# ChenKaiXuSan/Skiing_Analysis_PyTorch

Measured on AMD Instinct MI355X. Metric: 3D-pose frames/sec, 8-view 518px clips, higher is better.
Workload: dtype f16

## Files before the change

### include/skimi.h

```cpp
#ifndef SKIMI_H
#define SKIMI_H

#include <stddef.h>
#include <stdint.h>

#ifdef __cplusplus
extern "C" {
#endif

#define SKIMI_OK 0
#define SKIMI_ERR_ARG (-1)
#define SKIMI_ERR_HIP (-2)
#define SKIMI_ERR_STATE (-3)
#define SKIMI_ERR_WORKSPACE (-4)

#define SKIMI_F32 0
#define SKIMI_BF16 1
#define SKIMI_BF16X3_REC 2
#define SKIMI_FP8MX 3
#define SKIMI_F16 4

#define SKIMI_PREC_BF16 0
#define SKIMI_PREC_BF16X3 1
#define SKIMI_PREC_FP8 2
#define SKIMI_PREC_F16 3

#define SKIMI_ACT_NONE 0
#define SKIMI_ACT_RELU 1
#define SKIMI_ACT_GELU 2
#define SKIMI_ACT_SILU 3
#define SKIMI_ACT_SIGMOID 4

const char* skimi_last_error(void);
int skimi_version(void);
int skimi_sizeof_gemm_desc(void);
int skimi_device_count(void);

int skimi_profile_start(int32_t kind, int64_t min_size);
int skimi_profile_stop(double* total_ms, int64_t* launches, double* flops, double* bytes);

typedef struct skimi_gemm_desc {
    int32_t M, N, K;
    const void* A;
    const void* W;
    int32_t a_dtype, w_dtype;
    int64_t lda, ldw;
    int32_t prec;
    int32_t a_mode;
    int32_t cN, cH, cW, cC, KH, KW, stride, pad, dil, OH, OW;
    const float* bias;
    const float* gamma;
    const void* resid;
    int32_t resid_dtype;
    int64_t ldr;
    int32_t resid_rows_per_batch;
    int64_t resid_batch_stride;
    int64_t resid_row_off;
    int32_t act;
    const void* resid2;
    int64_t ldr2;
    int32_t post_act;
    int32_t out_rows_per_batch;
    int64_t out_batch_stride;
    int64_t out_row_off;
    void* out;
    void* out2;
    int32_t out_dtype;
    int64_t ldo, ldo2;
    int32_t store_mode, ps_s, ps_C;
    void* splitk_scratch;
    uint64_t splitk_scratch_bytes;
    int32_t force_splitk;
    int32_t splitk_scratch_zeroed;
    const void* W_split;
    void* x3_scratch;
    uint64_t x3_scratch_bytes;
    void* out_records;
} skimi_gemm_desc;

int skimi_split_planes(const float* x, int64_t ld, int64_t rows, int32_t C, void* hi, void* lo, void* stream);

int skimi_split_records(const float* x, int64_t ld, int64_t rows, int32_t C, void* records, void* stream);

int skimi_dpt_fold_pack(const float* w_T, const float* b_T, const float* w_rn, int32_t C_in, int32_t C_mid, int32_t C_out,
                        int32_t s, void* w_records, float* beta, void* stream);

int skimi_gemm(const skimi_gemm_desc* d, void* stream);

#define SKIMI_GEMM_PATH_GENERIC 1
#define SKIMI_GEMM_PATH_SPLITK_ORDERED 2
#define SKIMI_GEMM_PATH_SPLITK_ATOMIC 3
#define SKIMI_GEMM_PATH_X3DMA_WIDE 4
#define SKIMI_GEMM_PATH_X3DMA_NARROW 5
#define SKIMI_GEMM_PATH_GEMM256 6
#define SKIMI_GEMM_PATH_CONV_WIN 7
int32_t skimi_gemm_last_path(void);

int skimi_quant_mx(const void* x, int32_t dtype, int64_t ldx, int64_t rows, int32_t K, void* payload, void* scales,
                   void* stream);
int skimi_layernorm_mx(const float* x, int64_t ldx, int64_t rows, int32_t C, const float* gamma, const float* beta,
                       float eps, void* payload, void* scales, void* stream);
int skimi_gemm_fp8(const void* A, const void* A_scales, const void* W, const void* W_scales, int32_t M, int32_t N,
                   int32_t K, const float* bias, int32_t act, const float* gamma, const float* resid, int64_t ldr,
                   void* out, int32_t out_dtype, int64_t ldo, void* out_scales, void* stream);

int skimi_conv3x3_n32_pack(const float* w, void* packed, int32_t C, void* stream);
int skimi_conv3x3_n32(const void* in_hi, const void* in_lo, const void* packed_w, const float* bias, float* out,
                      int32_t F, int32_t H, int32_t W, int32_t C, int32_t relu, void* stream);

int skimi_resample_u8(const uint8_t* in, uint8_t* out, int64_t outer, int32_t n_in, int32_t n_out, int64_t inner,
                      const int32_t* kk, const int32_t* bounds, int32_t ksize, void* stream);
int skimi_u8_hwc_to_f32_chw(const uint8_t* in, int32_t H, int32_t W, float* out, int32_t OH, int32_t OW, int32_t y_off,
                            int32_t x_off, float fill, void* stream);

int skimi_layernorm(const float* x, const float* x2, int64_t ldx, int64_t rows, int32_t C,
                    const float* gamma, const float* beta, float eps,
                    void* out, int32_t out_dtype, int64_t ldo, void* stream);

int skimi_qknorm_rope(void* qkv, int32_t dtype, int64_t tokens, int32_t heads,
                      const float* qn_w, const float* qn_b, const float* kn_w, const float* kn_b,
                      float eps, const int32_t* pos, const float* rope_cos, const float* rope_sin,
                      int32_t rope_npos, void* stream);

int skimi_attention(const void* qkv, void* out, int32_t dtype, int32_t batch, int32_t seq,
                    int32_t heads, int32_t head_dim, void* stream);
int skimi_attention_out(const void* qkv, void* out, int32_t dtype, int32_t out_dtype, int32_t batch, int32_t seq,
                        int32_t heads, int32_t head_dim, void* stream);

int skimi_qknorm_rope_scaled(void* qkv, int32_t dtype, int64_t tokens, int32_t heads,
                             const float* qn_w, const float* qn_b, const float* kn_w, const float* kn_b,
                             float eps, const int32_t* pos, const float* rope_cos, const float* rope_sin,
                             int32_t rope_npos, float q_scale, int32_t* q_scaled, void* stream);
int skimi_attention_ex(const void* qkv, void* out, int32_t dtype, int32_t out_dtype, int32_t batch, int32_t seq,
                       int32_t heads, int32_t head_dim, int32_t q_prescaled, void* x3_scratch,
                       uint64_t x3_scratch_bytes, int32_t* out_records, void* stream);
uint64_t skimi_attention_x3_scratch_bytes(int64_t tokens, int64_t row_elems);

typedef struct skimi_vp3d skimi_vp3d;

skimi_vp3d* skimi_vp3d_create(int32_t joints_in, int32_t in_features, int32_t joints_out,
                              const int32_t* filter_widths, int32_t n_widths,
                              int32_t channels, int32_t causal);
skimi_vp3d* skimi_vp3d_create_ex(int32_t joints_in, int32_t in_features, int32_t joints_out,
                                 const int32_t* filter_widths, int32_t n_widths,
                                 int32_t channels, int32_t causal, int32_t dense);
void skimi_vp3d_destroy(skimi_vp3d*);
int skimi_vp3d_set_weight(skimi_vp3d*, const char* key, const float* host_data, int64_t n);
int skimi_vp3d_finalize(skimi_vp3d*, int32_t prec);
int32_t skimi_vp3d_receptive_field(const skimi_vp3d*);
size_t skimi_vp3d_workspace_bytes(const skimi_vp3d*, int32_t batch, int32_t frames_in);
int skimi_vp3d_forward(skimi_vp3d*, const float* x, float* out, int32_t batch, int32_t frames_in,
                       void* workspace, size_t workspace_bytes, void* stream);

typedef struct skimi_vggt skimi_vggt;

typedef struct skimi_vggt_config {
    int32_t patch_size, embed_dim, depth, num_heads, num_register_tokens;
    int32_t use_dino;
    int32_t dino_depth, dino_heads, dino_img_size;
    int32_t cam_trunk_depth, cam_heads, cam_iters;
    int32_t dpt_features, dpt_out_channels[4], dpt_layers[4];
    int32_t track_features, track_hidden, track_corr_levels, track_corr_radius, track_iters, track_depth,
        track_heads, track_virtual;
    int32_t enable_camera, enable_depth, enable_point, enable_track;
    int32_t prec;
    int32_t head_prec;
} skimi_vggt_config;

skimi_vggt* skimi_vggt_create(const skimi_vggt_config* cfg);
void skimi_vggt_destroy(skimi_vggt*);
int skimi_vggt_set_weight(skimi_vggt*, const char* key, const float* data, int64_t n, int32_t on_device);
int skimi_vggt_finalize(skimi_vggt*);
int skimi_vggt_set_pos_embed(skimi_vggt*, int32_t H, int32_t W, const float* pos_embed, int32_t on_device);
size_t skimi_vggt_workspace_bytes(skimi_vggt*, int32_t B, int32_t S, int32_t H, int32_t W, int32_t n_query);
int skimi_vggt_rope_positions(skimi_vggt*, int32_t frames, int32_t H, int32_t W, int32_t* positions);

typedef struct skimi_vggt_outputs {
    float* pose_enc;
    float* pose_enc_list;
    float* depth;
    float* depth_conf;
    float* world_points;
    float* world_points_conf;
    float* track;
    float* vis;
    float* conf;
    float* tokens_last;
} skimi_vggt_outputs;

int skimi_vggt_forward(skimi_vggt*, const float* images, const float* query_points, int32_t B, int32_t S,
                       int32_t H, int32_t W, int32_t n_query, const skimi_vggt_outputs* out,
                       void* workspace, size_t workspace_bytes, void* stream);

int skimi_pose_to_cameras(const float* pose_enc, int64_t rows, int32_t H, int32_t W, float* extrinsic,
                          float* intrinsic, void* stream);
int skimi_unproject_depth(const float* depth, const float* extrinsic, const float* intrinsic,
                          float* world_points, int32_t frames, int32_t H, int32_t W, void* stream);
int skimi_triangulate_dlt(const float* K, const float* R, const float* t, const float* keypoints,
                          float* joints3d, int64_t steps, int32_t views, int32_t joints, void* stream);

int skimi_triangulate_triage(const float* K, const float* R, const float* t, const float* keypoints, const float* conf,
                             double conf_thr, double err_thresh_px, int64_t steps, int32_t views, int32_t joints,
                             float* joints3d, float* joints3d_clean, double* err, double* depth, uint8_t* keep,
                             double* view_stats, double* report, void* stream);

int skimi_triangulate_robust(const float* K, const float* R, const float* t, const float* keypoints, const float* conf,
                             double conf_thr, double inlier_px, int32_t min_inliers, int32_t refine_iters, int32_t weighted,
                             int64_t steps, int32_t views, int32_t joints, float* joints3d, double* err,
                             uint8_t* inlier_views, double* rms_px, uint8_t* ok, float* joints3d_ok,
                             double* view_inlier_ratio, double* report, void* stream);

size_t skimi_person_workspace_bytes(int64_t maps, int32_t H, int32_t W);
int skimi_person_origin(const float* points, const float* boxes, int64_t maps, int32_t H, int32_t W, int32_t src_h,
                        int32_t src_w, void* workspace, double* stats, void* stream);
int skimi_recenter_cameras(const double* stats, const float* extrinsic, int64_t steps, int32_t views, double* origin_out,
                           float* R_out, float* t_out, void* stream);

size_t skimi_icp_workspace_bytes(int64_t n_src, int64_t n_tgt);
int skimi_estimate_normals(const float* points, int64_t n, double radius, double* normals_out,
                           int32_t* neighbour_count_out, void* ws, size_t ws_bytes, void* stream);
int skimi_icp_correspondences(const float* src, int64_t n_src, const float* tgt, int64_t n_tgt, const double* T4x4,
                              double max_dist, int32_t* tgt_index_out, void* ws, size_t ws_bytes, void* stream);
int skimi_icp_point_to_plane(const float* src, int64_t n_src, const float* tgt, int64_t n_tgt, double max_corr_dist,
                             double normal_radius, int32_t max_iteration, double rel_fitness, double rel_rmse,
                             const double* init4x4, double* T_out, double* fitness_out, double* rmse_out,
                             int32_t* iterations_out, void* ws, size_t ws_bytes, void* stream);

#define SKIMI_BA_POSE_ONLY 0
#define SKIMI_BA_POSE_CAM_T 1
#define SKIMI_BA_FULL 2
#define SKIMI_BA_AUTO 0
#define SKIMI_BA_LDS 1
#define SKIMI_BA_WORKSPACE 2
size_t skimi_ba_workspace_bytes(int64_t T, int32_t C, int32_t J, int32_t modes);
int skimi_bundle_adjust(const double* K, const double* R0, const double* t0, const double* X0, const double* x2d,
                        const double* conf, int64_t T, int32_t C, int32_t J, const int32_t* modes, int32_t n_modes,
                        int32_t num_iters, double lr, double w_reproj, double w_smooth, double w_baseline,
                        double w_bone_length, double w_pose_temporal, int32_t placement, double* R_out, double* t_out,
                        double* X_out, double* history_out, void* ws, size_t ws_bytes, void* stream);

#define SKIMI_RESECT_LINEAR 0
#define SKIMI_RESECT_SOFT_L1 1
size_t skimi_resect_workspace_bytes(int64_t n_points, int32_t views, int64_t group_size);
int skimi_resect_cameras(const double* X, const double* x2d, const double* conf, const double* K, const double* R0,
                         const double* t0, int64_t n_points, int32_t views, int64_t group_size, int32_t loss, double f_scale,
                         double min_conf, int32_t max_evals, double* R, double* t, double* K_out, double* cost0, double* cost,
                         int32_t* n_evals, int32_t* n_used, int32_t* success, double* err, double* stats, void* ws,
                         size_t ws_bytes, void* stream);
int skimi_relative_pose(const double* R, const double* t, int64_t groups, int32_t views, double* R_rel, double* t_rel,
                        void* stream);

#ifdef __cplusplus
}
#endif
#endif
```

### skiing_analysis_pytorch_amd/_lib.py

```python
from __future__ import annotations

import ctypes as C
from pathlib import Path

LIB_PATH = Path(__file__).resolve().parent / "lib" / "libskimi.so"

F32, BF16 = 0, 1
F16 = 4
BF16X3_REC = 2
FP8MX = 3
PREC_BF16, PREC_BF16X3, PREC_FP8 = 0, 1, 2
PREC_F16 = 3
ACT_NONE, ACT_RELU, ACT_GELU, ACT_SILU, ACT_SIGMOID = 0, 1, 2, 3, 4
GEMM_PATH_GENERIC, GEMM_PATH_SPLITK_ORDERED, GEMM_PATH_SPLITK_ATOMIC = 1, 2, 3
GEMM_PATH_X3DMA_WIDE, GEMM_PATH_X3DMA_NARROW, GEMM_PATH_GEMM256, GEMM_PATH_CONV_WIN = 4, 5, 6, 7


class SkimiError(RuntimeError):
    pass


class GemmDesc(C.Structure):

    _fields_ = [
        ("M", C.c_int32), ("N", C.c_int32), ("K", C.c_int32),
        ("A", C.c_void_p), ("W", C.c_void_p),
        ("a_dtype", C.c_int32), ("w_dtype", C.c_int32),
        ("lda", C.c_int64), ("ldw", C.c_int64),
        ("prec", C.c_int32),
        ("a_mode", C.c_int32),
        ("cN", C.c_int32), ("cH", C.c_int32), ("cW", C.c_int32), ("cC", C.c_int32),
        ("KH", C.c_int32), ("KW", C.c_int32), ("stride", C.c_int32), ("pad", C.c_int32),
        ("dil", C.c_int32), ("OH", C.c_int32), ("OW", C.c_int32),
        ("bias", C.c_void_p), ("gamma", C.c_void_p), ("resid", C.c_void_p),
        ("resid_dtype", C.c_int32),
        ("ldr", C.c_int64),
        ("resid_rows_per_batch", C.c_int32),
        ("resid_batch_stride", C.c_int64),
        ("resid_row_off", C.c_int64),
        ("act", C.c_int32),
        ("resid2", C.c_void_p), ("ldr2", C.c_int64), ("post_act", C.c_int32),
        ("out_rows_per_batch", C.c_int32), ("out_batch_stride", C.c_int64), ("out_row_off", C.c_int64),
        ("out", C.c_void_p), ("out2", C.c_void_p),
        ("out_dtype", C.c_int32),
        ("ldo", C.c_int64), ("ldo2", C.c_int64),
        ("store_mode", C.c_int32), ("ps_s", C.c_int32), ("ps_C", C.c_int32),
        ("splitk_scratch", C.c_void_p),
        ("splitk_scratch_bytes", C.c_uint64),
        ("force_splitk", C.c_int32), ("splitk_scratch_zeroed", C.c_int32),
        ("W_split", C.c_void_p), ("x3_scratch", C.c_void_p), ("x3_scratch_bytes", C.c_uint64),
        ("out_records", C.c_void_p),
    ]


_vp = C.c_void_p
_SIGNATURES = {
    "skimi_last_error": (C.c_char_p, []),
    "skimi_version": (C.c_int, []),
    "skimi_sizeof_gemm_desc": (C.c_int, []),
    "skimi_device_count": (C.c_int, []),
    "skimi_profile_start": (C.c_int, [C.c_int32, C.c_int64]),
    "skimi_profile_stop": (C.c_int, [C.POINTER(C.c_double), C.POINTER(C.c_int64), C.POINTER(C.c_double),
                                    C.POINTER(C.c_double)]),
    "skimi_gemm": (C.c_int, [C.POINTER(GemmDesc), _vp]),
    "skimi_gemm_last_path": (C.c_int32, []),
    "skimi_dpt_fold_pack": (C.c_int, [_vp, _vp, _vp, C.c_int32, C.c_int32, C.c_int32, C.c_int32, _vp, _vp, _vp]),
    "skimi_quant_mx": (C.c_int, [_vp, C.c_int32, C.c_int64, C.c_int64, C.c_int32, _vp, _vp, _vp]),
    "skimi_layernorm_mx": (C.c_int, [_vp, C.c_int64, C.c_int64, C.c_int32, _vp, _vp, C.c_float, _vp, _vp, _vp]),
    "skimi_gemm_fp8": (C.c_int, [_vp, _vp, _vp, _vp, C.c_int32, C.c_int32, C.c_int32, _vp, C.c_int32, _vp, _vp, C.c_int64,
                                 _vp, C.c_int32, C.c_int64, _vp, _vp]),
    "skimi_split_planes": (C.c_int, [_vp, C.c_int64, C.c_int64, C.c_int32, _vp, _vp, _vp]),
    "skimi_split_records": (C.c_int, [_vp, C.c_int64, C.c_int64, C.c_int32, _vp, _vp]),
    "skimi_resample_u8": (C.c_int, [_vp, _vp, C.c_int64, C.c_int32, C.c_int32, C.c_int64, _vp, _vp, C.c_int32, _vp]),
    "skimi_u8_hwc_to_f32_chw": (C.c_int, [_vp, C.c_int32, C.c_int32, _vp, C.c_int32, C.c_int32, C.c_int32, C.c_int32,
                                          C.c_float, _vp]),
    "skimi_conv3x3_n32_pack": (C.c_int, [_vp, _vp, C.c_int32, _vp]),
    "skimi_conv3x3_n32": (C.c_int, [_vp, _vp, _vp, _vp, _vp, C.c_int32, C.c_int32, C.c_int32, C.c_int32, C.c_int32, _vp]),
    "skimi_layernorm": (C.c_int, [_vp, _vp, C.c_int64, C.c_int64, C.c_int32, _vp, _vp, C.c_float, _vp,
                                  C.c_int32, C.c_int64, _vp]),
    "skimi_qknorm_rope": (C.c_int, [_vp, C.c_int32, C.c_int64, C.c_int32, _vp, _vp, _vp, _vp, C.c_float,
                                    _vp, _vp, _vp, C.c_int32, _vp]),
    "skimi_attention": (C.c_int, [_vp, _vp, C.c_int32, C.c_int32, C.c_int32, C.c_int32, C.c_int32, _vp]),
    "skimi_attention_out": (C.c_int, [_vp, _vp, C.c_int32, C.c_int32, C.c_int32, C.c_int32, C.c_int32, C.c_int32, _vp]),
    "skimi_qknorm_rope_scaled": (C.c_int, [_vp, C.c_int32, C.c_int64, C.c_int32, _vp, _vp, _vp, _vp, C.c_float,
                                           _vp, _vp, _vp, C.c_int32, C.c_float, C.POINTER(C.c_int32), _vp]),
    "skimi_attention_ex": (C.c_int, [_vp, _vp, C.c_int32, C.c_int32, C.c_int32, C.c_int32, C.c_int32, C.c_int32, C.c_int32,
                                     _vp, C.c_uint64, C.POINTER(C.c_int32), _vp]),
    "skimi_attention_x3_scratch_bytes": (C.c_uint64, [C.c_int64, C.c_int64]),
    "skimi_vp3d_create": (_vp, [C.c_int32, C.c_int32, C.c_int32, C.POINTER(C.c_int32), C.c_int32,
                                C.c_int32, C.c_int32]),
    "skimi_vp3d_create_ex": (_vp, [C.c_int32, C.c_int32, C.c_int32, C.POINTER(C.c_int32), C.c_int32,
                                   C.c_int32, C.c_int32, C.c_int32]),
    "skimi_vp3d_destroy": (None, [_vp]),
    "skimi_vp3d_set_weight": (C.c_int, [_vp, C.c_char_p, _vp, C.c_int64]),
    "skimi_vp3d_finalize": (C.c_int, [_vp, C.c_int32]),
    "skimi_vp3d_receptive_field": (C.c_int32, [_vp]),
    "skimi_vp3d_workspace_bytes": (C.c_size_t, [_vp, C.c_int32, C.c_int32]),
    "skimi_vp3d_forward": (C.c_int, [_vp, _vp, _vp, C.c_int32, C.c_int32, _vp, C.c_size_t, _vp]),
    "skimi_pose_to_cameras": (C.c_int, [_vp, C.c_int64, C.c_int32, C.c_int32, _vp, _vp, _vp]),
    "skimi_unproject_depth": (C.c_int, [_vp, _vp, _vp, _vp, C.c_int32, C.c_int32, C.c_int32, _vp]),
    "skimi_triangulate_dlt": (C.c_int, [_vp, _vp, _vp, _vp, _vp, C.c_int64, C.c_int32, C.c_int32, _vp]),
    "skimi_triangulate_triage": (C.c_int, [_vp, _vp, _vp, _vp, _vp, C.c_double, C.c_double, C.c_int64, C.c_int32, C.c_int32,
                                           _vp, _vp, _vp, _vp, _vp, _vp, _vp, _vp]),
    "skimi_triangulate_robust": (C.c_int, [_vp, _vp, _vp, _vp, _vp, C.c_double, C.c_double, C.c_int32, C.c_int32, C.c_int32,
                                           C.c_int64, C.c_int32, C.c_int32, _vp, _vp, _vp, _vp, _vp, _vp, _vp, _vp, _vp]),
    "skimi_person_workspace_bytes": (C.c_size_t, [C.c_int64, C.c_int32, C.c_int32]),
    "skimi_person_origin": (C.c_int, [_vp, _vp, C.c_int64, C.c_int32, C.c_int32, C.c_int32, C.c_int32, _vp, _vp, _vp]),
    "skimi_recenter_cameras": (C.c_int, [_vp, _vp, C.c_int64, C.c_int32, _vp, _vp, _vp, _vp]),
    "skimi_icp_workspace_bytes": (C.c_size_t, [C.c_int64, C.c_int64]),
    "skimi_estimate_normals": (C.c_int, [_vp, C.c_int64, C.c_double, _vp, _vp, _vp, C.c_size_t, _vp]),
    "skimi_icp_correspondences": (C.c_int, [_vp, C.c_int64, _vp, C.c_int64, C.POINTER(C.c_double), C.c_double, _vp, _vp,
                                            C.c_size_t, _vp]),
    "skimi_icp_point_to_plane": (C.c_int, [_vp, C.c_int64, _vp, C.c_int64, C.c_double, C.c_double, C.c_int32, C.c_double,
                                           C.c_double, C.POINTER(C.c_double), C.POINTER(C.c_double), C.POINTER(C.c_double),
                                           C.POINTER(C.c_double), C.POINTER(C.c_int32), _vp, C.c_size_t, _vp]),
    "skimi_ba_workspace_bytes": (C.c_size_t, [C.c_int64, C.c_int32, C.c_int32, C.c_int32]),
    "skimi_bundle_adjust": (C.c_int, [_vp, _vp, _vp, _vp, _vp, _vp, C.c_int64, C.c_int32, C.c_int32, C.POINTER(C.c_int32),
                                      C.c_int32, C.c_int32, C.c_double, C.c_double, C.c_double, C.c_double, C.c_double,
                                      C.c_double, C.c_int32, _vp, _vp, _vp, _vp, _vp, C.c_size_t, _vp]),
    "skimi_resect_workspace_bytes": (C.c_size_t, [C.c_int64, C.c_int32, C.c_int64]),
    "skimi_resect_cameras": (C.c_int, [_vp, _vp, _vp, _vp, _vp, _vp, C.c_int64, C.c_int32, C.c_int64, C.c_int32, C.c_double,
                                       C.c_double, C.c_int32, _vp, _vp, _vp, _vp, _vp, _vp, _vp, _vp, _vp, _vp, _vp, C.c_size_t,
                                       _vp]),
    "skimi_relative_pose": (C.c_int, [_vp, _vp, C.c_int64, C.c_int32, _vp, _vp, _vp]),
    "skimi_vggt_create": (_vp, [_vp]),
    "skimi_vggt_destroy": (None, [_vp]),
    "skimi_vggt_set_weight": (C.c_int, [_vp, C.c_char_p, _vp, C.c_int64, C.c_int32]),
    "skimi_vggt_finalize": (C.c_int, [_vp]),
    "skimi_vggt_set_pos_embed": (C.c_int, [_vp, C.c_int32, C.c_int32, _vp, C.c_int32]),
    "skimi_vggt_rope_positions": (C.c_int, [_vp, C.c_int32, C.c_int32, C.c_int32, _vp]),
    "skimi_vggt_workspace_bytes": (C.c_size_t, [_vp, C.c_int32, C.c_int32, C.c_int32, C.c_int32, C.c_int32]),
    "skimi_vggt_forward": (C.c_int, [_vp, _vp, _vp, C.c_int32, C.c_int32, C.c_int32, C.c_int32, C.c_int32, _vp,
                                     _vp, C.c_size_t, _vp]),
}

_lib = None


def exported_symbols():
    return sorted(_SIGNATURES)


def lib() -> C.CDLL:
    global _lib
    if _lib is not None:
        return _lib
    if not LIB_PATH.exists():
        raise SkimiError(
            f"{LIB_PATH} not found: build it with `python -m skiing_analysis_pytorch_amd.build` "
            "(or __graft_entry__.build()). There is no fallback path."
        )
    import torch

    handle = C.CDLL(str(LIB_PATH))
    for name, (res, args) in _SIGNATURES.items():
        try:
            fn = getattr(handle, name)
        except AttributeError as e:
            raise SkimiError(f"libskimi.so does not export {name}") from e
        fn.restype = res
        fn.argtypes = args
    if handle.skimi_sizeof_gemm_desc() != C.sizeof(GemmDesc):
        raise SkimiError(f"skimi_gemm_desc is {handle.skimi_sizeof_gemm_desc()} bytes in libskimi.so but "
                         f"{C.sizeof(GemmDesc)} in _lib.py: rebuild the library (python -m skiing_analysis_pytorch_amd.build)")
    _lib = handle
    return _lib


def check(rc: int, what: str = "") -> None:
    if rc != 0:
        msg = lib().skimi_last_error()
        raise SkimiError(f"{what} failed ({rc}): {msg.decode() if msg else ''}")


def ptr(t) -> int | None:
    if t is None:
        return None
    return t.data_ptr()


def current_stream() -> int:
    import torch

    return torch.cuda.current_stream().cuda_stream
```

### skiing_analysis_pytorch_amd/csrc/api.hip

```cpp
#include <stdarg.h>

#include <mutex>
#include <vector>

#include "common.h"
#include "gemm_epilogue.h"
#include "kernels.h"
#include "vggt_kernels.h"

namespace skimi {

static thread_local char g_err[512] = "";

void set_error(const char* fmt, ...) {
    va_list ap;
    va_start(ap, fmt);
    vsnprintf(g_err, sizeof(g_err), fmt, ap);
    va_end(ap);
}

int lds_opt_in(std::atomic<unsigned>& done, const void* kernel, int bytes, const char* what) {
    int dev = 0;
    if (hipGetDevice(&dev) != hipSuccess) {
        set_error("hipGetDevice failed (%s)", what);
// ... 78 lines not shown
        SKIMI_HIP(hipEventSynchronize(e.second));
        float t = 0;
        SKIMI_HIP(hipEventElapsedTime(&t, e.first, e.second));
        ms += t;
    }
    if (total_ms) *total_ms = ms;
    if (launches) *launches = (int64_t)g_prof.ev.size();
    if (flops) *flops = g_prof.flops;
    if (bytes) *bytes = g_prof.bytes;
    for (auto& e : g_prof.ev) g_prof.pool.push_back(e);
    g_prof.ev.clear();
    g_prof.kind = PROF_NONE;
    return SKIMI_OK;
}

int32_t skimi_gemm_last_path(void) { return gemm_last_path(); }

int skimi_gemm(const skimi_gemm_desc* d, void* stream) {
    if (!d) {
        set_gemm_path(0, 0, 0, 0, 0);
        set_error("skimi_gemm: null descriptor");
        return SKIMI_ERR_ARG;
    }
    return gemm_dispatch(d, (hipStream_t)stream, d->splitk_scratch, (size_t)d->splitk_scratch_bytes,
                         d->force_splitk);
}

int skimi_resample_u8(const uint8_t* in, uint8_t* out, int64_t outer, int32_t n_in, int32_t n_out, int64_t inner,
                      const int32_t* kk, const int32_t* bounds, int32_t ksize, void* stream) {
    return resample_u8_launch(in, out, outer, n_in, n_out, inner, kk, bounds, ksize, (hipStream_t)stream);
}

int skimi_u8_hwc_to_f32_chw(const uint8_t* in, int32_t H, int32_t W, float* out, int32_t OH, int32_t OW, int32_t y_off,
                            int32_t x_off, float fill, void* stream) {
    return u8_hwc_to_f32_chw_launch(in, H, W, out, OH, OW, y_off, x_off, fill, (hipStream_t)stream);
}

int skimi_conv3x3_n32_pack(const float* w, void* packed, int32_t C, void* stream) {
    SKIMI_CHECK_ARG(w && packed && C > 0, "skimi_conv3x3_n32_pack: bad arguments");
    return conv_direct_pack_launch(w, (unsigned short*)packed, C, (hipStream_t)stream);
}

int skimi_conv3x3_n32(const void* in_hi, const void* in_lo, const void* packed_w, const float* bias, float* out,
                      int32_t F, int32_t H, int32_t W, int32_t C, int32_t relu, void* stream) {
    return conv_direct_n32_launch((const unsigned short*)in_hi, (const unsigned short*)in_lo,
                                  (const unsigned short*)packed_w, bias, out, F, H, W, C, relu, (hipStream_t)stream);
}

int skimi_split_planes(const float* x, int64_t ld, int64_t rows, int32_t C, void* hi, void* lo, void* stream) {
    SKIMI_CHECK_ARG(x && hi && lo && rows > 0 && C > 0, "skimi_split_planes: bad arguments");
    return split_planes_launch(x, (long)ld, (long)rows, C, hi, lo, (hipStream_t)stream);
}

int skimi_split_records(const float* x, int64_t ld, int64_t rows, int32_t C, void* records, void* stream) {
    SKIMI_CHECK_ARG(x && records && rows > 0 && C > 0, "skimi_split_records: bad arguments");
    return split_records_launch(x, (long)ld, (long)rows, C, records, (hipStream_t)stream);
}

int skimi_dpt_fold_pack(const float* w_T, const float* b_T, const float* w_rn, int32_t C_in, int32_t C_mid, int32_t C_out,
                        int32_t s, void* w_records, float* beta, void* stream) {
    SKIMI_CHECK_ARG(w_T && w_rn && w_records && beta, "skimi_dpt_fold_pack: null buffer");
    SKIMI_CHECK_ARG(s >= 2 && s <= 16 && C_in > 0 && C_in % 32 == 0 && C_mid > 0 && C_out > 0, "skimi_dpt_fold_pack: bad sizes");
    float* tmp = nullptr;
    SKIMI_HIP(hipMalloc((void**)&tmp, (size_t)(s + 2) * (s + 2) * C_out * C_in * 4));
    const int rc = dpt_fold_pack_launch(w_T, b_T, w_rn, C_in, C_mid, C_out, s, tmp, w_records, beta, (hipStream_t)stream);
    const hipError_t e = hipStreamSynchronize((hipStream_t)stream);
    (void)hipFree(tmp);
    if (rc) return rc;
    SKIMI_HIP(e);
    return SKIMI_OK;
}

int skimi_quant_mx(const void* x, int32_t dtype, int64_t ldx, int64_t rows, int32_t K, void* payload, void* scales,
                   void* stream) {
    return quant_mx_launch(x, dtype, (long)ldx, (long)rows, K, payload, scales, (hipStream_t)stream);
}

int skimi_layernorm_mx(const float* x, int64_t ldx, int64_t rows, int32_t C, const float* gamma, const float* beta,
                       float eps, void* payload, void* scales, void* stream) {
    return layernorm_mx_launch(x, ldx, rows, C, gamma, beta, eps, payload, scales, (hipStream_t)stream);
}

int skimi_gemm_fp8(const void* A, const void* A_scales, const void* W, const void* W_scales, int32_t M, int32_t N,
                   int32_t K, const float* bias, int32_t act, const float* gamma, const float* resid, int64_t ldr,
                   void* out, int32_t out_dtype, int64_t ldo, void* out_scales, void* stream) {
    return gemm_fp8_launch(A, A_scales, W, W_scales, M, N, K, bias, act, gamma, resid, (long)ldr, out, out_dtype, (long)ldo,
                           (hipStream_t)stream, out_scales);
}

int skimi_layernorm(const float* x, const float* x2, int64_t ldx, int64_t rows, int32_t C,
                    const float* gamma, const float* beta, float eps, void* out, int32_t out_dtype,
                    int64_t ldo, void* stream) {
    return layernorm_launch(x, x2, ldx, rows, C, gamma, beta, eps, out, out_dtype, ldo,
                            (hipStream_t)stream);
}

int skimi_qknorm_rope(void* qkv, int32_t dtype, int64_t tokens, int32_t heads, const float* qn_w,
                      const float* qn_b, const float* kn_w, const float* kn_b, float eps,
                      const int32_t* pos, const float* rope_cos, const float* rope_sin,
                      int32_t rope_npos, void* stream) {
    return qknorm_rope_launch(qkv, dtype, tokens, heads, qn_w, qn_b, kn_w, kn_b, eps, pos, rope_cos,
                              rope_sin, rope_npos, (hipStream_t)stream);
}

int skimi_attention(const void* qkv, void* out, int32_t dtype, int32_t batch, int32_t seq,
                    int32_t heads, int32_t head_dim, void* stream) {
    return attention_launch(qkv, out, dtype, batch, seq, heads, head_dim, (hipStream_t)stream);
}

int skimi_attention_out(const void* qkv, void* out, int32_t dtype, int32_t out_dtype, int32_t batch, int32_t seq,
                        int32_t heads, int32_t head_dim, void* stream) {
    if (out_dtype == SKIMI_FP8MX) {
        SKIMI_CHECK_ARG(out && batch > 0 && seq > 0 && attention_mx_output_ok(dtype, heads, head_dim),
                        "skimi_attention_out: MXFP8 rows need bf16 q / k / v, head_dim 64 and an even number of heads");
        const size_t Kp = align_up((size_t)heads * head_dim, 128);
        return attention_launch(qkv, nullptr, dtype, batch, seq, heads, head_dim, (hipStream_t)stream, 0, nullptr, 0, nullptr, 0,
                                out, (char*)out + (size_t)batch * seq * Kp);
    }
    SKIMI_CHECK_ARG(out_dtype == dtype || (dtype == SKIMI_BF16 && out_dtype == SKIMI_F16),
                    "skimi_attention_out: out_dtype is dtype, SKIMI_F16 or SKIMI_FP8MX for bf16 q / k / v (got %d -> %d)", dtype, out_dtype);
    return attention_launch(qkv, out, dtype, batch, seq, heads, head_dim, (hipStream_t)stream, 0, nullptr, 0, nullptr,
                            out_dtype == SKIMI_F16 && dtype == SKIMI_BF16);
}

int skimi_qknorm_rope_scaled(void* qkv, int32_t dtype, int64_t tokens, int32_t heads, const float* qn_w,
                             const float* qn_b, const float* kn_w, const float* kn_b, float eps,
                             const int32_t* pos, const float* rope_cos, const float* rope_sin,
                             int32_t rope_npos, float q_scale, int32_t* q_scaled, void* stream) {
    return qknorm_rope_launch(qkv, dtype, tokens, heads, qn_w, qn_b, kn_w, kn_b, eps, pos, rope_cos,
                              rope_sin, rope_npos, (hipStream_t)stream, q_scale, q_scaled);
}

int skimi_attention_ex(const void* qkv, void* out, int32_t dtype, int32_t out_dtype, int32_t batch, int32_t seq,
                       int32_t heads, int32_t head_dim, int32_t q_prescaled, void* x3_scratch,
                       uint64_t x3_scratch_bytes, int32_t* out_records, void* stream) {
    if (out_dtype == SKIMI_FP8MX) {
        if (out_records) *out_records = 0;
        SKIMI_CHECK_ARG(out && batch > 0 && seq > 0 && attention_mx_output_ok(dtype, heads, head_dim),
                        "skimi_attention_ex: MXFP8 rows need bf16 q / k / v, head_dim 64 and an even number of heads");
        const size_t Kp = align_up((size_t)heads * head_dim, 128);
        return attention_launch(qkv, nullptr, dtype, batch, seq, heads, head_dim, (hipStream_t)stream, q_prescaled, nullptr, 0,
                                nullptr, 0, out, (char*)out + (size_t)batch * seq * Kp);
    }
    SKIMI_CHECK_ARG(out_dtype == dtype || (dtype == SKIMI_BF16 && out_dtype == SKIMI_F16),
                    "skimi_attention_ex: out_dtype is dtype, SKIMI_F16 or SKIMI_FP8MX for bf16 q / k / v (got %d -> %d)", dtype, out_dtype);
    return attention_launch(qkv, out, dtype, batch, seq, heads, head_dim, (hipStream_t)stream, q_prescaled, x3_scratch,
                            (size_t)x3_scratch_bytes, out_records, out_dtype == SKIMI_F16 && dtype == SKIMI_BF16);
}

uint64_t skimi_attention_x3_scratch_bytes(int64_t tokens, int64_t row_elems) {
    return (uint64_t)attention_x3_scratch_bytes((long)tokens, (long)row_elems);
}

}
```

### skiing_analysis_pytorch_amd/csrc/attention_bf16.hip

```cpp
#include <stdlib.h>

#include "common.h"
#include "kernels.h"

namespace skimi {

typedef __attribute__((ext_vector_type(4))) short s16x4;
typedef __attribute__((address_space(3))) s16x4 lds_s16x4;
typedef __attribute__((address_space(3))) void lds_void;
typedef __attribute__((address_space(1))) const void gbl_void;

__device__ __forceinline__ bf16x8 pack8(const f32x16& p, int s) {
    bf16x8 r;
#pragma unroll
    for (int j = 0; j < 8; ++j) r[j] = (short)f2bf(p[8 * s + j]);
    return r;
}

template <int dbg>
__global__ __launch_bounds__(256, 4) void attn_bf16_kernel(const AttnArgs a, int nqb) {
    constexpr int KV = 64;
    constexpr int TILE = KV * 64 * 2;
    __shared__ __attribute__((aligned(16))) char smem[4 * TILE];

// ... 20 lines not shown

    bf16x8 qf[4];
    {
        const int q = min(q0 + l31, a.seq_q - 1);
        const unsigned short* qp = Q + (long)q * a.q_row + 8 * lh;
#pragma unroll
        for (int s = 0; s < 4; ++s) qf[s] = *reinterpret_cast<const bf16x8*>(qp + 16 * s);
    }

    const int nkt = (a.seq_k + KV - 1) / KV;
    const bool ragged = (a.seq_k & (KV - 1)) != 0;
    const int srow = lane >> 3, sch = lane & 7;
    auto issue = [&](int buf, int kt) {
        char* kb = smem + buf * 2 * TILE;
        char* vb = kb + TILE;
#pragma unroll
        for (int j = 0; j < 2; ++j) {
            const int row = 8 * (2 * wave + j) + srow;
            const int key = min(kt * KV + row, a.seq_k - 1);
            const int kc = sch ^ ((row >> 1) & 7);
            const int vc = sch ^ (((row >> 1) & 1) << 2);
            __builtin_amdgcn_global_load_lds((gbl_void*)(K + (long)key * a.k_row + kc * 8),
                                             (lds_void*)(kb + (2 * wave + j) * 8 * 128), 16, 0, 0);
            __builtin_amdgcn_global_load_lds((gbl_void*)(V + (long)key * a.v_row + vc * 8),
                                             (lds_void*)(vb + (2 * wave + j) * 8 * 128), 16, 0, 0);
        }
    };

    f32x16 o[2];
#pragma unroll
    for (int i = 0; i < 2; ++i)
#pragma unroll
        for (int r = 0; r < 16; ++r) o[i][r] = 0.f;
    f32x16 lacc = {0.f, 0.f, 0.f, 0.f, 0.f, 0.f, 0.f, 0.f, 0.f, 0.f, 0.f, 0.f, 0.f, 0.f, 0.f, 0.f};
    const bf16x8 ones = {0x3F80, 0x3F80, 0x3F80, 0x3F80, 0x3F80, 0x3F80, 0x3F80, 0x3F80};
    float m = -INFINITY;
    const float c2 = a.scale * 1.44269504088896340736f;

    issue(0, 0);
    __builtin_amdgcn_s_waitcnt(0x0F70);
    __syncthreads();

    for (int kt = 0; kt < nkt; ++kt) {
        const int cur = kt & 1;
        if (kt + 1 < nkt) issue(cur ^ 1, kt + 1);
        const char* kb = smem + cur * 2 * TILE;
        const char* vb = kb + TILE;

        f32x16 s[2];
        const f32x16 zero16 = {0.f, 0.f, 0.f, 0.f, 0.f, 0.f, 0.f, 0.f, 0.f, 0.f, 0.f, 0.f, 0.f, 0.f, 0.f, 0.f};
#pragma unroll
        for (int t = 0; t < 2; ++t) {
            const int row = t * 32 + l31;
#pragma unroll
            for (int ks = 0; ks < 4; ++ks) {
                const bf16x8 kf = (dbg & 1) ? qf[ks] :
                    *reinterpret_cast<const bf16x8*>(kb + row * 128 + (((2 * ks + lh) ^ ((row >> 1) & 7)) << 4));
                s[t] = __builtin_amdgcn_mfma_f32_32x32x16_bf16(kf, qf[ks], ks == 0 ? zero16 : s[t], 0, 0, 0);
            }
        }
        if (ragged && kt == nkt - 1) {
#pragma unroll
            for (int t = 0; t < 2; ++t)
#pragma unroll
                for (int r = 0; r < 16; ++r) {
                    const int key = kt * KV + t * 32 + (r & 3) + 8 * (r >> 2) + 4 * lh;
                    if (key >= a.seq_k) s[t][r] = -INFINITY;
                }
        }
        float mloc = -INFINITY;
#pragma unroll
        for (int t = 0; t < 2; ++t)
#pragma unroll
            for (int r = 0; r < 16; ++r) mloc = fmaxf(mloc, s[t][r]);
        mloc = fmaxf(mloc, __shfl_xor(mloc, 32, 64));
        const float mnew = fmaxf(m, mloc);
        const float nmb = -(mnew * c2);
        if (!__all(mnew == m)) {
            const float alpha = __builtin_amdgcn_exp2f((m - mnew) * c2);
#pragma unroll
            for (int r = 0; r < 16; ++r) {
                o[0][r] *= alpha;
                o[1][r] *= alpha;
                lacc[r] *= alpha;
            }
            m = mnew;
        }
#pragma unroll
        for (int r = 0; r < 16; ++r) {
            if (!(dbg & 4)) {
                s[0][r] = __builtin_amdgcn_exp2f(__builtin_fmaf(s[0][r], c2, nmb));
                s[1][r] = __builtin_amdgcn_exp2f(__builtin_fmaf(s[1][r], c2, nmb));
            }
        }

#pragma unroll
        for (int t = 0; t < 2; ++t) {
#pragma unroll
            for (int ks = 0; ks < 2; ++ks) {
                const bf16x8 pf = pack8(s[t], ks);
                if (!(dbg & 8)) lacc = __builtin_amdgcn_mfma_f32_32x32x16_bf16(ones, pf, lacc, 0, 0, 0);
#pragma unroll
                for (int dt = 0; dt < 2; ++dt) {
                    const int q4 = (lane & 15) >> 2, p4 = lane & 3;
                    const int dcol = dt * 32 + 16 * ((lane >> 4) & 1) + 4 * p4;
                    bf16x8 vf = qf[0];
                    if (!(dbg & 2))
#pragma unroll
                    for (int half = 0; half < 2; ++half) {
                        const int row = t * 32 + 16 * ks + 8 * half + 4 * lh + q4;
                        const int chunk = (dcol >> 3) ^ (((row >> 1) & 1) << 2);
                        const char* addr = vb + row * 128 + (chunk << 4) + ((dcol & 7) << 1);
                        const s16x4 v4 = __builtin_amdgcn_ds_read_tr16_b64_v4i16((lds_s16x4*)addr);
                        vf[4 * half + 0] = v4[0];
                        vf[4 * half + 1] = v4[1];
                        vf[4 * half + 2] = v4[2];
                        vf[4 * half + 3] = v4[3];
                    }
                    o[dt] = __builtin_amdgcn_mfma_f32_32x32x16_bf16(vf, pf, o[dt], 0, 0, 0);
                }
            }
        }

        __builtin_amdgcn_s_waitcnt(0x0F70);
        __syncthreads();
    }

    const float inv = 1.f / lacc[0];
    const int q = q0 + l31;
    if (q < a.seq_q) {
        unsigned short* op = O + (long)q * a.o_row;
#pragma unroll
        for (int dt = 0; dt < 2; ++dt)
#pragma unroll
            for (int g = 0; g < 4; ++g) {
                bf16x4 v;
#pragma unroll
                for (int j = 0; j < 4; ++j) v[j] = (short)f2x16(o[dt][4 * g + j] * inv, a.out_f16 != 0);
                *reinterpret_cast<bf16x4*>(op + dt * 32 + 8 * g + 4 * lh) = v;
            }
    }
}

static int q64_enabled() {
    static const int q64 = getenv("SKIMI_ATTN_Q64") ? atoi(getenv("SKIMI_ATTN_Q64")) : 1;
    return q64;
}

bool attention_mx_output_ok(int dtype, int heads, int head_dim) {
    static const bool dyn = getenv("SKIMI_ENV_DYNAMIC") && atoi(getenv("SKIMI_ENV_DYNAMIC"));
    static int use_mx = -1;
    if (use_mx < 0 || dyn) use_mx = getenv("SKIMI_ATTN_MX") ? atoi(getenv("SKIMI_ATTN_MX")) : 1;
    return use_mx && dtype == SKIMI_BF16 && head_dim == 64 && heads % 2 == 0 && q64_enabled() != 0;
}

int attention_bf16_launch(const AttnArgs& a, hipStream_t st) {
    SKIMI_CHECK_ARG(a.q && a.k && a.v && (a.out || a.out_mx), "skimi_attention: null buffer");
    SKIMI_CHECK_ARG(a.batch > 0 && a.heads > 0 && a.seq_q > 0 && a.seq_k > 0, "skimi_attention: empty shape");
    SKIMI_CHECK_ARG(a.head_dim == 64, "skimi_attention: the bf16 MFMA kernel is head_dim 64 only (got %d)", a.head_dim);
    SKIMI_CHECK_ARG(a.q_row % 8 == 0 && a.k_row % 8 == 0 && a.v_row % 8 == 0 && a.o_row % 4 == 0 &&
                    a.q_head % 8 == 0 && a.k_head % 8 == 0 && a.v_head % 8 == 0 && a.o_head % 4 == 0 &&
                    a.q_batch % 8 == 0 && a.k_batch % 8 == 0 && a.v_batch % 8 == 0 && a.o_batch % 4 == 0,
                    "skimi_attention: bf16 strides must keep 16-B alignment");
    SKIMI_CHECK_ARG((((uintptr_t)a.q | (uintptr_t)a.k | (uintptr_t)a.v) & 15) == 0,
                    "skimi_attention: bf16 q / k / v are loaded in 16-B pieces: the buffer must be 16-B aligned");
    const int nqb = (int)cdiv(a.seq_q, 128);
    const long nblk = (long)nqb * a.heads * a.batch;
    SKIMI_CHECK_ARG(nblk < (1l << 31), "skimi_attention: grid too large");
    const bool prof = prof_armed(PROF_ATTN_BF16, a.seq_k);
    if (prof) prof_before(st);
#ifdef SKIMI_ABLATIONS
    static const int dbg = getenv("SKIMI_ATTN_ABL") ? atoi(getenv("SKIMI_ATTN_ABL")) : 0;
#else
    const int dbg = 0;
#endif
    const int q64 = q64_enabled();
    SKIMI_CHECK_ARG(!a.out_mx || q64 != 0, "skimi_attention: MXFP8 output rows are written by the 64-query kernel only");
    if (q64 != 0) {
        attention_q64_dispatch(a, st);
    } else if (a.q_prescaled) {
        AttnArgs a1 = a;
        a1.scale = 0.69314718055994530942f;
        hipLaunchKernelGGL(attn_bf16_kernel<0>, dim3((unsigned)nblk), dim3(256), 0, st, a1, nqb);
    } else
    switch (dbg) {
#ifdef SKIMI_ABLATIONS
#define SKIMI_ABL_CASE(D) case D: hipLaunchKernelGGL(attn_bf16_kernel<D>, dim3((unsigned)nblk), dim3(256), 0, st, a, nqb); break;
        SKIMI_ABL_CASE(1) SKIMI_ABL_CASE(2) SKIMI_ABL_CASE(3) SKIMI_ABL_CASE(4) SKIMI_ABL_CASE(8) SKIMI_ABL_CASE(12)
        SKIMI_ABL_CASE(15)
#undef SKIMI_ABL_CASE
#endif
        default: hipLaunchKernelGGL(attn_bf16_kernel<0>, dim3((unsigned)nblk), dim3(256), 0, st, a, nqb);
    }
    if (prof) {
        const double bh = (double)a.batch * a.heads;
        prof_after(st, 4.0 * bh * a.seq_q * (double)a.seq_k * 64.0,
                   2.0 * bh * 64.0 * (2.0 * a.seq_q + 2.0 * a.seq_k));
    }
    SKIMI_LAUNCH_CHECK();
    return SKIMI_OK;
}

int attention_launch(const void* qkv, void* out, int dtype, int batch, int seq, int heads, int head_dim,
                     hipStream_t st, int q_prescaled, void* x3_scratch, size_t x3_scratch_bytes, int* out_records, int out_f16,
                     void* out_mx, void* out_mx_scales) {
    SKIMI_CHECK_ARG(qkv && (out || out_mx), "skimi_attention: null buffer");
    SKIMI_CHECK_ARG(!out_mx || (out_mx_scales && attention_mx_output_ok(dtype, heads, head_dim)),
                    "skimi_attention: MXFP8 output needs the 64-query bf16 kernel (head_dim 64, heads even) and a scale buffer");
    const bool want_rec = out_records != nullptr && *out_records != 0;
    if (out_records) *out_records = 0;
    AttnArgs a;
    const long C = (long)heads * head_dim;
    const size_t es = dtype == SKIMI_F32 ? 4 : 2;
    a.q = qkv;
    a.k = (const char*)qkv + C * es;
    a.v = (const char*)qkv + 2 * C * es;
    a.out = out;
    a.q_row = a.k_row = a.v_row = 3 * C;
    a.o_row = C;
    a.q_batch = a.k_batch = a.v_batch = (long)seq * 3 * C;
    a.o_batch = (long)seq * C;
    a.q_head = a.k_head = a.v_head = a.o_head = head_dim;
    a.batch = batch;
    a.heads = heads;
    a.seq_q = a.seq_k = seq;
    a.head_dim = head_dim;
    a.scale = 1.0f / sqrtf((float)head_dim);
    a.q_prescaled = dtype == SKIMI_F32 ? 0 : q_prescaled;
    a.out_f16 = dtype == SKIMI_F32 ? 0 : out_f16;
    if (out_mx) {
        a.out_mx = out_mx;
        a.out_mx_scales = out_mx_scales;
        a.mx_row = (long)align_up((size_t)C, 128);
        a.mx_srow = a.mx_row / 32;
    }
    if (dtype == SKIMI_F32) {
        static const bool dyn = getenv("SKIMI_ENV_DYNAMIC") && atoi(getenv("SKIMI_ENV_DYNAMIC"));
        static int use_x3 = -1;
        if (use_x3 < 0 || dyn) use_x3 = getenv("SKIMI_ATTN_X3") ? atoi(getenv("SKIMI_ATTN_X3")) : 1;
        const long tokens = (long)batch * seq;
        if (use_x3 && head_dim == 64 && x3_scratch && x3_scratch_bytes >= attention_x3_scratch_bytes(tokens, 3 * C)) {
            const bool rec = want_rec && ((uintptr_t)out & 127) == 0;
            if (rec) *out_records = 1;
            return attention_x3_launch(a, tokens, 3 * C, x3_scratch, x3_scratch_bytes, st, rec);
        }
        return attention_f32_launch(a, st);
    }
    return attention_bf16_launch(a, st);
}

}
```

### skiing_analysis_pytorch_amd/csrc/attention_q64.hip

```cpp
#include <stdlib.h>

#include "common.h"
#include "kernels.h"

namespace skimi {

typedef __attribute__((ext_vector_type(4))) short s16x4;
typedef __attribute__((address_space(3))) s16x4 lds_s16x4;
typedef __attribute__((address_space(3))) void lds_void;
typedef __attribute__((address_space(1))) const void gbl_void;
typedef __attribute__((ext_vector_type(2))) float f32x2;

__device__ __forceinline__ float xhalf_max(float x) {
    const auto r = __builtin_amdgcn_permlane32_swap(__float_as_uint(x), __float_as_uint(x), false, false);
    return __builtin_fmaxf(__uint_as_float(r[0]), __uint_as_float(r[1]));
}
__device__ __forceinline__ float xhalf_sum(float x) {
    const auto r = __builtin_amdgcn_permlane32_swap(__float_as_uint(x), __float_as_uint(x), false, false);
    return __uint_as_float(r[0]) + __uint_as_float(r[1]);
}

template <int dbg>
__global__ __launch_bounds__(256, 2) void attn_q64_kernel(const AttnArgs a, int nqb) {
    constexpr int KV = 64;
    constexpr int TILE = KV * 64 * 2;
    __shared__ __attribute__((aligned(16))) char smem[4 * TILE];

    const int tid = threadIdx.x, lane = tid & 63;
    const int wave = __builtin_amdgcn_readfirstlane(tid >> 6);
    const int l31 = lane & 31, lh = lane >> 5;

    int id;
    {
        const int nblk = gridDim.x;
        const int bid = blockIdx.x;
        const int xcd = bid & 7;
        const int q = nblk >> 3, r = nblk & 7;
        id = (xcd < r ? xcd * (q + 1) : r * (q + 1) + (xcd - r) * q) + (bid >> 3);
    }
    const int qb = id % nqb;
    const int bh = id / nqb;
    const int head = bh % a.heads, b = bh / a.heads;
    const int q0 = qb * 256 + wave * 64;

    const unsigned short* Q = (const unsigned short*)a.q + (long)b * a.q_batch + (long)head * a.q_head;
    const unsigned short* K = (const unsigned short*)a.k + (long)b * a.k_batch + (long)head * a.k_head;
    const unsigned short* V = (const unsigned short*)a.v + (long)b * a.v_batch + (long)head * a.v_head;
    unsigned short* O = (unsigned short*)a.out + (long)b * a.o_batch + (long)head * a.o_head;

    bf16x8 qf[2][4];
#pragma unroll
    for (int qi = 0; qi < 2; ++qi) {
        const int q = min(q0 + qi * 32 + l31, a.seq_q - 1);
        const unsigned short* qp = Q + (long)q * a.q_row + 8 * lh;
#pragma unroll
        for (int s = 0; s < 4; ++s) qf[qi][s] = *reinterpret_cast<const bf16x8*>(qp + 16 * s);
    }
    if (!a.q_prescaled) {
        const float c2q = a.scale * 1.44269504088896340736f;
#pragma unroll
        for (int qi = 0; qi < 2; ++qi)
#pragma unroll
            for (int s = 0; s < 4; ++s)
#pragma unroll
                for (int j = 0; j < 8; ++j) qf[qi][s][j] = (short)f2bf(bf2f((unsigned short)qf[qi][s][j]) * c2q);
    }

    const int nkt = (a.seq_k + KV - 1) / KV;
    const bool ragged = (a.seq_k & (KV - 1)) != 0;
    const int srow = lane >> 3, sch = lane & 7;
    auto issue = [&](int buf, int kt) {
        char* kb = smem + buf * 2 * TILE;
        char* vb = kb + TILE;
#pragma unroll
        for (int j = 0; j < 2; ++j) {
            const int row = 8 * (2 * wave + j) + srow;
            const int key = min(kt * KV + row, a.seq_k - 1);
            const int kc = sch ^ ((row >> 1) & 7);
            const int vc = sch ^ (((row >> 1) & 1) << 2);
            __builtin_amdgcn_global_load_lds((gbl_void*)(K + (long)key * a.k_row + kc * 8),
                                             (lds_void*)(kb + (2 * wave + j) * 8 * 128), 16, 0, 0);
            __builtin_amdgcn_global_load_lds((gbl_void*)(V + (long)key * a.v_row + vc * 8),
                                             (lds_void*)(vb + (2 * wave + j) * 8 * 128), 16, 0, 0);
        }
    };

    f32x16 o[2][2];
#pragma unroll
    for (int qi = 0; qi < 2; ++qi)
#pragma unroll
        for (int dt = 0; dt < 2; ++dt)
#pragma unroll
            for (int r = 0; r < 16; ++r) o[qi][dt][r] = 0.f;
    float lsum[2] = {0.f, 0.f};
    float mr[2] = {0.f, 0.f};
    const f32x16 zero16 = {0.f, 0.f, 0.f, 0.f, 0.f, 0.f, 0.f, 0.f, 0.f, 0.f, 0.f, 0.f, 0.f, 0.f, 0.f, 0.f};
    bf16x8 kone = {0, 0, 0, 0, 0, 0, 0, 0};
    if (lh == 0) kone[0] = (short)0x3F80;
    bf16x8 qneg[2] = {{0, 0, 0, 0, 0, 0, 0, 0}, {0, 0, 0, 0, 0, 0, 0, 0}};

    issue(0, 0);
    __builtin_amdgcn_s_waitcnt(0x0F70);
    __syncthreads();

    for (int kt = 0; kt < nkt; ++kt) {
        const int cur = kt & 1;
        const char* kb = smem + cur * 2 * TILE;
        const char* vb = kb + TILE;

        f32x16 s[2][2];
        bf16x8 kf[2][4];
#pragma unroll
        for (int t = 0; t < 2; ++t) {
            const int row = t * 32 + l31;
#pragma unroll
            for (int ks = 0; ks < 4; ++ks)
                kf[t][ks] = *reinterpret_cast<const bf16x8*>(kb + row * 128 + (((2 * ks + lh) ^ ((row >> 1) & 7)) << 4));
        }
        __builtin_amdgcn_sched_barrier(0);
#pragma unroll
        for (int t = 0; t < 2; ++t) {
#pragma unroll
            for (int qi = 0; qi < 2; ++qi)
                s[qi][t] = __builtin_amdgcn_mfma_f32_32x32x16_bf16(kone, qneg[qi], zero16, 0, 0, 0);
#pragma unroll
            for (int ks = 0; ks < 4; ++ks)
#pragma unroll
                for (int qi = 0; qi < 2; ++qi)
                    s[qi][t] = __builtin_amdgcn_mfma_f32_32x32x16_bf16(kf[t][ks], qf[qi][ks], s[qi][t], 0, 0, 0);
        }

        bf16x8 vf[2][2][2];
#pragma unroll
        for (int t = 0; t < 2; ++t)
#pragma unroll
            for (int ks = 0; ks < 2; ++ks)
#pragma unroll
                for (int dt = 0; dt < 2; ++dt) {
                    const int q4 = (lane & 15) >> 2, p4 = lane & 3;
                    const int dcol = dt * 32 + 16 * ((lane >> 4) & 1) + 4 * p4;
#pragma unroll
                    for (int half = 0; half < 2; ++half) {
                        const int row = t * 32 + 16 * ks + 8 * half + 4 * lh + q4;
                        const int chunk = (dcol >> 3) ^ (((row >> 1) & 1) << 2);
                        const char* addr = vb + row * 128 + (chunk << 4) + ((dcol & 7) << 1);
                        const s16x4 v4 = __builtin_amdgcn_ds_read_tr16_b64_v4i16((lds_s16x4*)addr);
                        vf[t][ks][dt][4 * half + 0] = v4[0];
                        vf[t][ks][dt][4 * half + 1] = v4[1];
                        vf[t][ks][dt][4 * half + 2] = v4[2];
                        vf[t][ks][dt][4 * half + 3] = v4[3];
                    }
                }

        __builtin_amdgcn_sched_barrier(0);
        if (kt + 1 < nkt) issue(cur ^ 1, kt + 1);

        if (ragged && kt == nkt - 1) {
#pragma unroll
            for (int qi = 0; qi < 2; ++qi)
#pragma unroll
                for (int t = 0; t < 2; ++t)
#pragma unroll
                    for (int r = 0; r < 16; ++r) {
                        const int key = kt * KV + t * 32 + (r & 3) + 8 * (r >> 2) + 4 * lh;
                        if (key >= a.seq_k) s[qi][t][r] = -INFINITY;
                    }
        }

#pragma unroll
        for (int qi = 0; qi < 2; ++qi) {
            bool redo = kt == 0;
            if (kt != 0) {
                float l0 = 0.f, l1 = 0.f;
#pragma unroll
                for (int t = 0; t < 2; ++t)
#pragma unroll
                    for (int r = 0; r < 16; r += 2) {
                        float v0 = s[qi][t][r], v1 = s[qi][t][r + 1];
                        if (!(dbg & 2)) {
                            v0 = __builtin_amdgcn_exp2f(v0);
                            v1 = __builtin_amdgcn_exp2f(v1);
                        }
                        l0 += v0;
                        l1 += v1;
                        s[qi][t][r] = v0;
                        s[qi][t][r + 1] = v1;
                    }
                const float ts = l0 + l1;
                redo = __any(!(ts < 1.099511627776e12f));
                if (!redo) lsum[qi] += ts;
            }
            if (redo) {
                if (kt != 0) {
#pragma unroll
                    for (int t = 0; t < 2; ++t) {
                        const int row = t * 32 + l31;
                        s[qi][t] = __builtin_amdgcn_mfma_f32_32x32x16_bf16(kone, qneg[qi], zero16, 0, 0, 0);
#pragma unroll
                        for (int ks = 0; ks < 4; ++ks) {
                            const bf16x8 kr = *reinterpret_cast<const bf16x8*>(kb + row * 128 + (((2 * ks + lh) ^ ((row >> 1) & 7)) << 4));
                            s[qi][t] = __builtin_amdgcn_mfma_f32_32x32x16_bf16(kr, qf[qi][ks], s[qi][t], 0, 0, 0);
                        }
                        if (ragged && kt == nkt - 1) {
#pragma unroll
                            for (int r = 0; r < 16; ++r) {
                                const int key = kt * KV + t * 32 + (r & 3) + 8 * (r >> 2) + 4 * lh;
                                if (key >= a.seq_k) s[qi][t][r] = -INFINITY;
                            }
                        }
                    }
                }
                float mloc = -INFINITY;
#pragma unroll
                for (int t = 0; t < 2; ++t)
#pragma unroll
                    for (int r = 0; r < 16; ++r) mloc = __builtin_fmaxf(mloc, s[qi][t][r]);
                mloc = xhalf_max(mloc);
                const float want = mr[qi] + (kt == 0 ? mloc : __builtin_fmaxf(mloc, 0.f));
                const float mnew = bf2f(f2bf(want));
                const float dlt = mnew - mr[qi];
                if (kt != 0) {
                    const float alpha = __builtin_amdgcn_exp2f(-dlt);
#pragma unroll
                    for (int r = 0; r < 16; ++r) {
                        o[qi][0][r] *= alpha;
                        o[qi][1][r] *= alpha;
                    }
                    lsum[qi] *= alpha;
                }
                mr[qi] = mnew;
                qneg[qi][0] = lh == 0 ? (short)f2bf(-mnew) : (short)0;
                float l0 = 0.f, l1 = 0.f;
#pragma unroll
                for (int t = 0; t < 2; ++t)
#pragma unroll
                    for (int r = 0; r < 16; r += 2) {
                        float v0 = s[qi][t][r] - dlt, v1 = s[qi][t][r + 1] - dlt;
                        if (!(dbg & 2)) {
                            v0 = __builtin_amdgcn_exp2f(v0);
                            v1 = __builtin_amdgcn_exp2f(v1);
                        }
                        l0 += v0;
                        l1 += v1;
                        s[qi][t][r] = v0;
                        s[qi][t][r + 1] = v1;
                    }
                lsum[qi] += l0 + l1;
            }

#pragma unroll
            for (int t = 0; t < 2; ++t)
#pragma unroll
                for (int ks = 0; ks < 2; ++ks) {
                    bf16x8 pf;
#pragma unroll
                    for (int j = 0; j < 8; ++j) pf[j] = (short)f2bf(s[qi][t][8 * ks + j]);
#pragma unroll
                    for (int dt = 0; dt < 2; ++dt)
                        o[qi][dt] = __builtin_amdgcn_mfma_f32_32x32x16_bf16(vf[t][ks][dt], pf, o[qi][dt], 0, 0, 0);
                }
        }

        __builtin_amdgcn_s_waitcnt(0x0F70);
        if (!(dbg & 1)) __syncthreads();
    }

#pragma unroll
    for (int qi = 0; qi < 2; ++qi) {
        const float inv = 1.f / xhalf_sum(lsum[qi]);
        const int q = q0 + qi * 32 + l31;
        if (a.out_mx) {
            const long tok = (long)b * a.seq_q + q;
            unsigned char* pq = (unsigned char*)a.out_mx + tok * a.mx_row + head * 64;
            unsigned char* ps = (unsigned char*)a.out_mx_scales + tok * a.mx_srow + head * 2;
            unsigned sb2 = 0;
#pragma unroll
            for (int dt = 0; dt < 2; ++dt) {
                float amax = 0.f;
#pragma unroll
                for (int j = 0; j < 16; ++j) amax = __builtin_fmaxf(amax, __builtin_fabsf(o[qi][dt][j] * inv));
                amax = xhalf_max(amax);
                const unsigned sb = mx_scale_byte(amax);
                const float si = mx_inv_scale(sb);
                sb2 |= sb << (8 * dt);
                if (q < a.seq_q) {
#pragma unroll
                    for (int g = 0; g < 4; ++g)
                        *reinterpret_cast<int*>(pq + dt * 32 + 8 * g + 4 * lh) =
                            mx_pack4(o[qi][dt][4 * g] * inv, o[qi][dt][4 * g + 1] * inv, o[qi][dt][4 * g + 2] * inv,
                                     o[qi][dt][4 * g + 3] * inv, si);
                }
            }
            if (q < a.seq_q && lh == 0) *reinterpret_cast<unsigned short*>(ps) = (unsigned short)sb2;
            continue;
        }
        if (q < a.seq_q) {
            unsigned short* op = O + (long)q * a.o_row;
#pragma unroll
            for (int dt = 0; dt < 2; ++dt)
#pragma unroll
                for (int g = 0; g < 4; ++g) {
                    bf16x4 v;
#pragma unroll
                    for (int j = 0; j < 4; ++j) v[j] = (short)f2x16(o[qi][dt][4 * g + j] * inv, a.out_f16 != 0);
                    *reinterpret_cast<bf16x4*>(op + dt * 32 + 8 * g + 4 * lh) = v;
                }
        }
    }
}

void attention_q64_dispatch(const AttnArgs& a, hipStream_t st) {
    const int nqb = (int)cdiv(a.seq_q, 256);
    const long nblk = (long)nqb * a.heads * a.batch;
#ifdef SKIMI_ABLATIONS
    static const int dbg = getenv("SKIMI_ATTN_ABL") ? atoi(getenv("SKIMI_ATTN_ABL")) : 0;
#else
    const int dbg = 0;
#endif
    static const size_t pad = getenv("SKIMI_ATTN_LDSPAD") ? (size_t)atol(getenv("SKIMI_ATTN_LDSPAD")) : 0;
    if (pad) {
        static bool once = false;
        if (!once) {
            (void)hipFuncSetAttribute(reinterpret_cast<const void*>(attn_q64_kernel<0>), hipFuncAttributeMaxDynamicSharedMemorySize, (int)pad);
            once = true;
        }
        hipLaunchKernelGGL(attn_q64_kernel<0>, dim3((unsigned)nblk), dim3(256), pad, st, a, nqb);
        return;
    }
    switch (dbg) {
#ifdef SKIMI_ABLATIONS
        case 1: hipLaunchKernelGGL(attn_q64_kernel<1>, dim3((unsigned)nblk), dim3(256), 0, st, a, nqb); break;
        case 2: hipLaunchKernelGGL(attn_q64_kernel<2>, dim3((unsigned)nblk), dim3(256), 0, st, a, nqb); break;
        case 3: hipLaunchKernelGGL(attn_q64_kernel<3>, dim3((unsigned)nblk), dim3(256), 0, st, a, nqb); break;
#endif
        default: hipLaunchKernelGGL(attn_q64_kernel<0>, dim3((unsigned)nblk), dim3(256), 0, st, a, nqb);
    }
}

}
```

### skiing_analysis_pytorch_amd/csrc/kernels.h

```cpp
#pragma once
#include "common.h"

namespace skimi {

int gemm_dispatch(const skimi_gemm_desc* d, hipStream_t st, void* scratch, size_t scratch_bytes,
                  int force_splitk);

int layernorm_launch(const float* x, const float* x2, int64_t ldx, int64_t rows, int C,
                     const float* gamma, const float* beta, float eps, void* out, int out_dtype,
                     int64_t ldo, hipStream_t st, int64_t grp_rows = 0, int64_t grp_stride = 0,
                     int64_t grp_off = 0);

int qknorm_rope_launch(void* qkv, int dtype, int64_t tokens, int heads, const float* qn_w,
                       const float* qn_b, const float* kn_w, const float* kn_b, float eps,
                       const int32_t* pos, const float* rope_cos, const float* rope_sin, int rope_npos,
                       hipStream_t st, float q_scale = 1.f, int* q_scaled = nullptr);

struct AttnArgs {
    const void* q;
    const void* k;
    const void* v;
    void* out;
    long q_row, k_row, v_row, o_row;
    long q_batch, k_batch, v_batch, o_batch;
    long q_head, k_head, v_head, o_head;
    int batch, heads, seq_q, seq_k, head_dim;
    float scale;
    int batch_inner = 0;
    long q_batch2 = 0, k_batch2 = 0, v_batch2 = 0, o_batch2 = 0;
    int q_prescaled = 0;
    int out_f16 = 0;
    void* out_mx = nullptr;
    void* out_mx_scales = nullptr;
    long mx_row = 0, mx_srow = 0;
};
bool attention_mx_output_ok(int dtype, int heads, int head_dim);
int attention_f32_launch(const AttnArgs& a, hipStream_t st);
int attention_bf16_launch(const AttnArgs& a, hipStream_t st);
int resample_u8_launch(const unsigned char* in, unsigned char* out, long outer, int n_in, int n_out, long inner,
                       const int* kk, const int* bounds, int ksize, hipStream_t st);
int u8_hwc_to_f32_chw_launch(const unsigned char* in, int H, int W, float* out, int OH, int OW, int y_off, int x_off,
                             float fill, hipStream_t st);
int conv_direct_pack_launch(const float* w, unsigned short* out, int Cin, hipStream_t st);
int conv_direct_n32_launch(const unsigned short* in_hi, const unsigned short* in_lo, const unsigned short* w_packed,
                           const float* bias, float* out, int F, int H, int W, int C, int relu, hipStream_t st,
                           long px_stride = 0);
void attention_q64_dispatch(const AttnArgs& a, hipStream_t st);
int attention_launch(const void* qkv, void* out, int dtype, int batch, int seq, int heads, int head_dim,
                     hipStream_t st, int q_prescaled = 0, void* x3_scratch = nullptr, size_t x3_scratch_bytes = 0,
                     int* out_records = nullptr,
                     int out_f16 = 0,
                     void* out_mx = nullptr, void* out_mx_scales = nullptr);
size_t attention_x3_scratch_bytes(long tokens, long row_elems);
int attention_x3_launch(const AttnArgs& a, long tokens, long row_elems, void* scratch, size_t scratch_bytes, hipStream_t st,
                        bool out_records = false);

int vp3d_im2col_launch(const float* x, float* a0, int B, int L, int Cin, int k, int Kpad, hipStream_t st);

int quant_mx_launch(const void* x, int dtype, long ldx, long rows, int K, void* q, void* scales, hipStream_t st);
int gemm_fp8_launch(const void* A, const void* As, const void* W, const void* Ws, int M, int N, int K, const float* bias, int act,
                    const float* gamma, const float* resid, long ldr, void* out, int out_dtype, long ldo, hipStream_t st,
                    void* out_scales = nullptr);
bool gemm_fp8_mx_output_ok(int M, int N);
int layernorm_mx_launch(const float* x, int64_t ldx, int64_t rows, int C, const float* gamma, const float* beta, float eps,
                        void* payload, void* scales, hipStream_t st);

int vp3d_expand_launch(const float* x, const float* w, int ldw, const float* bias, float* out_f32, void* out_rec, int B, int Lin,
                       int Cin, int taps, int C, hipStream_t st);
int vp3d_expand_mfma_launch(const float* x, const void* wfrag, int Kpad, const float* bias, float* out_f32, void* out_rec, int B,
                            int Lin, int Cin, int taps, int C, hipStream_t st);
int vp3d_mm_launch(const void* wrec, int Npad, const void* xrec, const float* bias, const float* resid, int resid_L,
                   int resid_off, float* out_f32, int ldo, void* out_rec, int B, int Lin, int C, int taps, int dil, int N,
                   int relu, hipStream_t st);
bool vp3d_window_enabled();
int vp3d_win_launch(const void* wrec, int Npad, const void* xrec, const float* bias, float* out_f32, int ldo, void* out_rec,
                    int B, int Lin, int C, int taps, int N, hipStream_t st);

}
```

### skiing_analysis_pytorch_amd/csrc/rowops.hip

```cpp
#include <algorithm>

#include "common.h"
#include "kernels.h"

namespace skimi {

template <int MAXV>
__global__ __launch_bounds__(256) void layernorm_kernel(const float* __restrict__ x,
                                                        const float* __restrict__ x2, long ldx, long rows,
                                                        int C, const float* __restrict__ gamma,
                                                        const float* __restrict__ beta, float eps, void* out,
                                                        int out_dtype, long ldo, long grp_rows,
                                                        long grp_stride, long grp_off) {
    const int lane = threadIdx.x & 63;
    const long orow = (long)blockIdx.x * 4 + (threadIdx.x >> 6);
    if (orow >= rows) return;
    const long row = grp_rows > 0 ? (orow / grp_rows) * grp_stride + grp_off + orow % grp_rows : orow;
    const int half = C >> 1;
    float v[MAXV];
    float s = 0.f;
#pragma unroll
    for (int i = 0; i < MAXV; ++i) {
        const int c = lane + 64 * i;
        float t = 0.f;
// ... 142 lines not shown
int layernorm_mx_launch(const float* x, int64_t ldx, int64_t rows, int C, const float* gamma, const float* beta, float eps,
                        void* payload, void* scales, hipStream_t st) {
    SKIMI_CHECK_ARG(x && payload && scales && rows > 0, "layernorm_mx: bad arguments");
    SKIMI_CHECK_ARG(C % 256 == 0 && ldx % 4 == 0 && ((uintptr_t)x & 15) == 0 && ((uintptr_t)payload & 3) == 0,
                    "layernorm_mx: C must be a multiple of 256 and the rows 16-byte aligned");
    dim3 grid((unsigned)cdiv(rows, 4)), block(256);
#define LNM_GO(V) hipLaunchKernelGGL(layernorm_vec_kernel<V>, grid, block, 0, st, x, (const float*)nullptr, (long)ldx, (long)rows, gamma, beta, eps, payload, (int)SKIMI_FP8MX, (long)C, 0L, 0L, 0L, (unsigned char*)scales)
    switch (C / 256) {
        case 1: LNM_GO(1); break;
        case 2: LNM_GO(2); break;
        case 3: LNM_GO(3); break;
        case 4: LNM_GO(4); break;
        case 6: LNM_GO(6); break;
        case 8: LNM_GO(8); break;
        default: set_error("layernorm_mx: C = %d not supported", C); return SKIMI_ERR_ARG;
    }
#undef LNM_GO
    SKIMI_LAUNCH_CHECK();
    return SKIMI_OK;
}

template <typename T>
__global__ __launch_bounds__(256) void qknorm_rope_kernel(T* __restrict__ qkv, long tokens, int heads,
                                                          const float* __restrict__ qn_w,
                                                          const float* __restrict__ qn_b,
                                                          const float* __restrict__ kn_w,
                                                          const float* __restrict__ kn_b, float eps,
                                                          const int* __restrict__ pos,
                                                          const float* __restrict__ rcos,
                                                          const float* __restrict__ rsin, int npos) {
    const int lane = threadIdx.x & 63;
    const long vec = (long)blockIdx.x * 4 + (threadIdx.x >> 6);
    const long total = tokens * 2 * heads;
    if (vec >= total) return;
    const long tok = vec / (2 * heads);
    const int rem = (int)(vec - tok * 2 * heads);
    const int which = rem / heads;
    const int h = rem - which * heads;
    T* p = qkv + ((tok * 3 + which) * heads + h) * 64;
    float t;
    if (sizeof(T) == 4) t = ((const float*)p)[lane];
    else t = bf2f(((const unsigned short*)p)[lane]);
    const float* w = which ? kn_w : qn_w;
    const float* b = which ? kn_b : qn_b;
    if (w != nullptr) {
        const float mean = wave_sum(t) * (1.f / 64.f);
        const float d = t - mean;
        const float var = wave_sum(d * d) * (1.f / 64.f);
        t = d * rsqrtf(var + eps) * w[lane] + (b ? b[lane] : 0.f);
    }
    if (pos != nullptr) {
        const int sect = lane >> 5;
        const int d = lane & 31;
        int pp = pos[tok * 2 + sect];
        pp = min(max(pp, 0), npos - 1);
        const float c = rcos[pp * 16 + (d & 15)];
        const float s = rsin[pp * 16 + (d & 15)];
        const float other = __shfl_xor(t, 16, 64);
        const float rot = (d < 16) ? -other : other;
        t = t * c + rot * s;
    }
    if (sizeof(T) == 4) ((float*)p)[lane] = t;
    else ((unsigned short*)p)[lane] = f2bf(t);
}

template <typename T>
__global__ __launch_bounds__(256) void qknorm_rope_vec_kernel(T* __restrict__ qkv, long tokens, int heads,
                                                              const float* __restrict__ qn_w,
                                                              const float* __restrict__ qn_b,
                                                              const float* __restrict__ kn_w,
                                                              const float* __restrict__ kn_b, float eps,
                                                              const int* __restrict__ pos,
                                                              const float* __restrict__ rcos,
                                                              const float* __restrict__ rsin, int npos) {
    const long gid = (long)blockIdx.x * 256 + threadIdx.x;
    const long vec = gid >> 3;
    const int sub = (int)(gid & 7);
    const long total = tokens * 2 * heads;
    const bool live = vec < total;
    const long vv = live ? vec : total - 1;
    const long tok = vv / (2 * heads);
    const int rem = (int)(vv - tok * 2 * heads);
    const int which = rem / heads;
    const int h = rem - which * heads;
    T* p = qkv + ((tok * 3 + which) * heads + h) * 64 + 8 * sub;
    float t[8];
    if (sizeof(T) == 4) {
        const float4 a = *reinterpret_cast<const float4*>(p), b = *reinterpret_cast<const float4*>((const float*)p + 4);
        t[0] = a.x; t[1] = a.y; t[2] = a.z; t[3] = a.w; t[4] = b.x; t[5] = b.y; t[6] = b.z; t[7] = b.w;
    } else {
        const bf16x8 a = *reinterpret_cast<const bf16x8*>(p);
#pragma unroll
        for (int j = 0; j < 8; ++j) t[j] = bf2f((unsigned short)a[j]);
    }
    const float* w = which ? kn_w : qn_w;
    const float* b = which ? kn_b : qn_b;
    if (w != nullptr) {
        float s = 0.f;
#pragma unroll
        for (int j = 0; j < 8; ++j) s += t[j];
        s += __shfl_xor(s, 1, 64); s += __shfl_xor(s, 2, 64); s += __shfl_xor(s, 4, 64);
        const float mean = s * (1.f / 64.f);
        float q = 0.f;
#pragma unroll
        for (int j = 0; j < 8; ++j) { t[j] -= mean; q += t[j] * t[j]; }
        q += __shfl_xor(q, 1, 64); q += __shfl_xor(q, 2, 64); q += __shfl_xor(q, 4, 64);
        const float rstd = rsqrtf(q * (1.f / 64.f) + eps);
#pragma unroll
        for (int j = 0; j < 8; ++j) t[j] = t[j] * rstd * w[8 * sub + j] + (b ? b[8 * sub + j] : 0.f);
    }
    if (pos != nullptr) {
        const int sect = sub >> 2;
        const int d0 = (8 * sub) & 31;
        int pp = pos[tok * 2 + sect];
        pp = min(max(pp, 0), npos - 1);
        const float* ct = rcos + pp * 16 + (d0 & 15);
        const float* st = rsin + pp * 16 + (d0 & 15);
        const bool lower = d0 < 16;
#pragma unroll
        for (int j = 0; j < 8; ++j) {
            const float other = __shfl_xor(t[j], 2, 64);
            const float rot = lower ? -other : other;
            t[j] = t[j] * ct[j] + rot * st[j];
        }
    }
    if (!live) return;
    if (sizeof(T) == 4) {
        *reinterpret_cast<float4*>(p) = make_float4(t[0], t[1], t[2], t[3]);
        *reinterpret_cast<float4*>((float*)p + 4) = make_float4(t[4], t[5], t[6], t[7]);
    } else {
        bf16x8 o;
#pragma unroll
        for (int j = 0; j < 8; ++j) o[j] = (short)f2bf(t[j]);
        *reinterpret_cast<bf16x8*>(p) = o;
    }
}

__device__ __forceinline__ float dpp_xor1(float v) {
    return __int_as_float(__builtin_amdgcn_update_dpp(0, __float_as_int(v), 0xB1, 0xF, 0xF, true));
}
__device__ __forceinline__ float dpp_xor2(float v) {
    return __int_as_float(__builtin_amdgcn_update_dpp(0, __float_as_int(v), 0x4E, 0xF, 0xF, true));
}
__device__ __forceinline__ float dpp_mirror8(float v) {
    return __int_as_float(__builtin_amdgcn_update_dpp(0, __float_as_int(v), 0x141, 0xF, 0xF, true));
}
__device__ __forceinline__ float sum8(float s) {
    s += dpp_xor1(s);
    s += dpp_xor2(s);
    s += dpp_mirror8(s);
    return s;
}

__global__ __launch_bounds__(256) void qknorm_rope_bf16_kernel(unsigned short* __restrict__ qkv, long tokens, int heads,
                                                               const float* __restrict__ qn_w,
                                                               const float* __restrict__ qn_b,
                                                               const float* __restrict__ kn_w,
                                                               const float* __restrict__ kn_b, float eps,
                                                               const int* __restrict__ pos,
                                                               const float* __restrict__ rcos,
                                                               const float* __restrict__ rsin, int npos, float q_scale) {
    extern __shared__ __attribute__((aligned(16))) float tab[];
    for (int i = threadIdx.x; i < npos * 16; i += 256) {
        tab[i] = rcos[i];
        tab[npos * 16 + i] = rsin[i];
    }
    __syncthreads();
    const int sub = threadIdx.x & 7;
    float w[2][8], b[2][8];
#pragma unroll
    for (int j = 0; j < 8; ++j) {
        w[0][j] = qn_w[8 * sub + j]; b[0][j] = qn_b ? qn_b[8 * sub + j] : 0.f;
        w[1][j] = kn_w[8 * sub + j]; b[1][j] = kn_b ? kn_b[8 * sub + j] : 0.f;
    }
    const int sect = sub >> 2;
    const int d0 = (8 * sub) & 15;
    const bool lower = ((8 * sub) & 31) < 16;
    const long total = tokens * heads;
    const long step = (long)gridDim.x * 32;
    const long trips = (total + step - 1) / step;
    long idx = (long)blockIdx.x * 32 + (threadIdx.x >> 3);
    for (long it = 0; it < trips; ++it, idx += step) {
        const bool live = idx < total;
        const long ii = live ? idx : total - 1;
        const long tok = ii / heads;
        const int h = (int)(ii - tok * heads);
        unsigned short* pq = qkv + ((tok * 3) * heads + h) * 64 + 8 * sub;
        unsigned short* pk = pq + (long)heads * 64;
        const bf16x8 raw[2] = {*reinterpret_cast<const bf16x8*>(pq), *reinterpret_cast<const bf16x8*>(pk)};
        int pp = pos[tok * 2 + sect];
        pp = min(max(pp, 0), npos - 1);
        const float4 c0 = *reinterpret_cast<const float4*>(&tab[pp * 16 + d0]);
        const float4 c1 = *reinterpret_cast<const float4*>(&tab[pp * 16 + d0 + 4]);
        const float4 s0 = *reinterpret_cast<const float4*>(&tab[npos * 16 + pp * 16 + d0]);
        const float4 s1 = *reinterpret_cast<const float4*>(&tab[npos * 16 + pp * 16 + d0 + 4]);
        const float ct[8] = {c0.x, c0.y, c0.z, c0.w, c1.x, c1.y, c1.z, c1.w};
        const float st[8] = {s0.x, s0.y, s0.z, s0.w, s1.x, s1.y, s1.z, s1.w};
        bf16x8 outv[2];
#pragma unroll
        for (int z = 0; z < 2; ++z) {
            float t[8];
#pragma unroll
            for (int j = 0; j < 8; ++j) t[j] = bf2f((unsigned short)raw[z][j]);
            float s = 0.f;
#pragma unroll
            for (int j = 0; j < 8; ++j) s += t[j];
            const float mean = sum8(s) * (1.f / 64.f);
            float q = 0.f;
#pragma unroll
            for (int j = 0; j < 8; ++j) { t[j] -= mean; q += t[j] * t[j]; }
            const float rstd = rsqrtf(sum8(q) * (1.f / 64.f) + eps);
#pragma unroll
            for (int j = 0; j < 8; ++j) t[j] = t[j] * rstd * w[z][j] + b[z][j];
#pragma unroll
            for (int j = 0; j < 8; ++j) {
                const float other = dpp_xor2(t[j]);
                const float rot = lower ? -other : other;
                const float r = t[j] * ct[j] + rot * st[j];
                outv[z][j] = (short)f2bf(z == 0 ? r * q_scale : r);
            }
        }
        if (live) {
            *reinterpret_cast<bf16x8*>(pq) = outv[0];
            *reinterpret_cast<bf16x8*>(pk) = outv[1];
        }
    }
}

int qknorm_rope_launch(void* qkv, int dtype, int64_t tokens, int heads, const float* qn_w, const float* qn_b,
                       const float* kn_w, const float* kn_b, float eps, const int32_t* pos,
                       const float* rope_cos, const float* rope_sin, int rope_npos, hipStream_t st, float q_scale,
                       int* q_scaled) {
    SKIMI_CHECK_ARG(qkv && tokens > 0 && heads > 0, "skimi_qknorm_rope: bad arguments");
    if (q_scaled) *q_scaled = 0;
    SKIMI_CHECK_ARG(pos == nullptr || (rope_cos && rope_sin && rope_npos > 0), "skimi_qknorm_rope: pos without tables");
    if (((uintptr_t)qkv & 15) == 0 && dtype == SKIMI_BF16 && qn_w && kn_w && pos && rope_npos * 128 <= 48 * 1024) {
        const long total = tokens * heads;
        const unsigned blocks = (unsigned)std::min<long>(cdiv(total, 32), 256 * 8);
        hipLaunchKernelGGL(qknorm_rope_bf16_kernel, dim3(blocks), dim3(256), (size_t)rope_npos * 128, st,
                           (unsigned short*)qkv, (long)tokens, heads, qn_w, qn_b, kn_w, kn_b, eps, pos, rope_cos, rope_sin,
                           rope_npos, q_scaled ? q_scale : 1.f);
        if (q_scaled) *q_scaled = 1;
        SKIMI_LAUNCH_CHECK();
        return SKIMI_OK;
    }
    if (((uintptr_t)qkv & 15) == 0) {
        const long threads = tokens * 2 * heads * 8;
        dim3 g((unsigned)cdiv(threads, 256)), blk(256);
        if (dtype == SKIMI_F32)
            hipLaunchKernelGGL(qknorm_rope_vec_kernel<float>, g, blk, 0, st, (float*)qkv, (long)tokens, heads, qn_w, qn_b,
                               kn_w, kn_b, eps, pos, rope_cos, rope_sin, rope_npos);
        else
            hipLaunchKernelGGL(qknorm_rope_vec_kernel<unsigned short>, g, blk, 0, st, (unsigned short*)qkv, (long)tokens,
                               heads, qn_w, qn_b, kn_w, kn_b, eps, pos, rope_cos, rope_sin, rope_npos);
        SKIMI_LAUNCH_CHECK();
        return SKIMI_OK;
    }
    const long total = tokens * 2 * heads;
    dim3 grid((unsigned)cdiv(total, 4)), block(256);
    if (dtype == SKIMI_F32)
        hipLaunchKernelGGL(qknorm_rope_kernel<float>, grid, block, 0, st, (float*)qkv, (long)tokens, heads, qn_w,
                           qn_b, kn_w, kn_b, eps, pos, rope_cos, rope_sin, rope_npos);
    else
        hipLaunchKernelGGL(qknorm_rope_kernel<unsigned short>, grid, block, 0, st, (unsigned short*)qkv,
                           (long)tokens, heads, qn_w, qn_b, kn_w, kn_b, eps, pos, rope_cos, rope_sin, rope_npos);
    SKIMI_LAUNCH_CHECK();
    return SKIMI_OK;
}

__global__ __launch_bounds__(256) void vp3d_im2col_kernel(const float* __restrict__ x, float* __restrict__ a0,
                                                          int B, int L, int Cin, int k, int Kpad) {
    const int Lout = L - k + 1;
    const long total = (long)B * Lout * Kpad;
    for (long i = (long)blockIdx.x * 256 + threadIdx.x; i < total; i += (long)gridDim.x * 256) {
        const int c = (int)(i % Kpad);
        const long r = i / Kpad;
        const int b = (int)(r / Lout);
        const int t = (int)(r - (long)b * Lout);
        a0[i] = (c < k * Cin) ? x[((long)b * L + t) * Cin + c] : 0.f;
    }
}

int vp3d_im2col_launch(const float* x, float* a0, int B, int L, int Cin, int k, int Kpad, hipStream_t st) {
    const long total = (long)B * (L - k + 1) * Kpad;
    int blocks = (int)std::min<long>(cdiv(total, 256), 1024);
    hipLaunchKernelGGL(vp3d_im2col_kernel, dim3(blocks), dim3(256), 0, st, x, a0, B, L, Cin, k, Kpad);
    SKIMI_LAUNCH_CHECK();
    return SKIMI_OK;
}

}
```

### skiing_analysis_pytorch_amd/csrc/vggt.hip

```cpp
#include <math.h>
#include <string.h>

#include <map>
#include <memory>
#include <string>
#include <tuple>
#include <atomic>
#include <mutex>
#include <vector>

#include <stdlib.h>

#include "common.h"
#include "gemm_epilogue.h"
#include "kernels.h"
#include "track_kernels.h"
#include "vggt_kernels.h"

using namespace skimi;

namespace {

struct Lin {
    void* w = nullptr;
    int wdt = SKIMI_F32;
    float* b = nullptr;
    int N = 0, K = 0;
    int prec = SKIMI_PREC_BF16X3;
    void* w_split = nullptr;
    void* wq = nullptr;
    void* wq_scales = nullptr;
};
struct LNw { float* g = nullptr; float* b = nullptr; };
struct BlockW {
    LNw n1, n2;
    Lin qkv, proj, fc1, fc2;
    float *ls1 = nullptr, *ls2 = nullptr;
    float *qn_w = nullptr, *qn_b = nullptr, *kn_w = nullptr, *kn_b = nullptr;
};
struct ConvW { Lin lin; int k = 1, stride = 1, pad = 0, cin = 0; int kmode = 1; };
struct FusionW { Lin out_conv; ConvW r1c1, r1c2, r2c1, r2c2; bool has_r1 = false; };
struct DptW {
    LNw norm;
    Lin proj[4];
    Lin rs0, rs1;
    Lin fold[2];
    ConvW rs3;
    ConvW rn[4];
    FusionW ref[4];
    ConvW oc1, oc2a;
    float *oc2b_w = nullptr, *oc2b_b = nullptr;
    unsigned short* oc2a_direct = nullptr;
    int n_out = 0, features = 0, oc[4] = {0, 0, 0, 0};
    bool feature_only = false, pos_embed = true;
    bool out_f32 = false;
    const LNw* out_ln = nullptr;
    int down_ratio = 1;
};
struct CamW {
    std::vector<BlockW> trunk;
    LNw token_norm, trunk_norm;
    float* empty16 = nullptr;
    Lin embed_pose, poseLN, fc1, fc2;
};

struct Arena {
    char* base = nullptr;
    size_t off = 0, peak = 0, cap = 0;
    bool dry = false, overflow = false;
    void* alloc(size_t bytes) {
        off = align_up(off, 256);
        void* p = dry ? (void*)(uintptr_t)(0x1000 + off) : (void*)(base + off);
        off += bytes;
        if (off > peak) peak = off;
        if (!dry && off > cap) overflow = true;
        return p;
    }
    size_t mark() const { return off; }
    void release(size_t m) { off = m; }
};

struct UvTab { int w, h, C; float* tx; float* ty; };

struct ShapeTabs {
    int frames = 0;
    int* pos = nullptr;
    float *rope_cos = nullptr, *rope_sin = nullptr;
    int rope_npos = 0;
    const float* dino_pos = nullptr;
    std::vector<UvTab> uv;
    std::vector<void*> owned;
    ~ShapeTabs() {
        for (void* p : owned) (void)hipFree(p);
    }
};

#define TRACK_PART 1
#include "track_impl.inc"
#undef TRACK_PART

}

struct skimi_vggt {
    skimi_vggt_config cfg;
    std::map<std::string, std::pair<float*, int64_t>> raw;
    std::vector<void*> owned;
    bool finalized = false;
    bool dpt_fold = true;
    Lin patch_proj;
    int patch_kp = 0;
    float* dino_pos = nullptr;
    std::map<std::pair<int, int>, float*> dino_pos_alt;
    float* dino_special = nullptr;
    float* agg_special = nullptr;
    std::vector<BlockW> dino, frame, global;
    LNw dino_norm;
    CamW cam;
    DptW depth, point, trackf;
    TrackW track;
    std::mutex prep_mu;
    std::map<std::pair<int, int>, std::vector<std::unique_ptr<ShapeTabs>>> tabs;
};

namespace {

struct Packer {
    skimi_vggt* h;
    int rc = SKIMI_OK;
    hipStream_t st = nullptr;

    float* raw(const std::string& key, int64_t n) {
        if (rc) return nullptr;
        auto it = h->raw.find(key);
        if (it == h->raw.end()) {
            set_error("skimi_vggt_finalize: missing weight '%s'", key.c_str());
            rc = SKIMI_ERR_STATE;
            return nullptr;
        }
        if (it->second.second != n) {
            set_error("skimi_vggt_finalize: weight '%s' has %ld elements, expected %ld", key.c_str(),
                      (long)it->second.second, (long)n);
            rc = SKIMI_ERR_STATE;
            return nullptr;
        }
        return it->second.first;
    }
    void* dmalloc(size_t bytes) {
        if (rc) return nullptr;
        void* p = nullptr;
        if (hipMalloc(&p, bytes) != hipSuccess) {
            set_error("skimi_vggt_finalize: hipMalloc(%zu) failed", bytes);
            rc = SKIMI_ERR_HIP;
            return nullptr;
        }
        h->owned.push_back(p);
        return p;
    }
    float* keep(const std::string& key, int64_t n) {
        float* src = raw(key, n);
        if (!src) return nullptr;
        float* dst = (float*)dmalloc(n * 4);
        if (dst && hipMemcpyAsync(dst, src, n * 4, hipMemcpyDeviceToDevice, st) != hipSuccess) rc = SKIMI_ERR_HIP;
        return dst;
    }
    LNw ln(const std::string& p, int C) { return LNw{keep(p + ".weight", C), keep(p + ".bias", C)}; }

    Lin pack_matrix(float* src, int N, int K, int prec) {
        Lin L;
        L.N = N;
        L.K = (int)align_up((size_t)K, 8);
        L.prec = prec;
        if (rc) return L;
        float* m = src;
        if (L.K != K) {
            m = (float*)dmalloc((size_t)N * L.K * 4);
            if (m && (rc = pad_cols_launch(src, m, N, K, L.K, st))) return L;
        }
        if (prec == SKIMI_PREC_BF16 || prec == SKIMI_PREC_F16) {
            void* b = dmalloc((size_t)N * L.K * 2);
            if (b) rc = prec == SKIMI_PREC_F16 ? f32_to_f16_launch(m, b, (long)N * L.K, st) : f32_to_bf16_launch(m, b, (long)N * L.K, st);
            L.w = b;
            L.wdt = prec == SKIMI_PREC_F16 ? SKIMI_F16 : SKIMI_BF16;
        } else {
            if (m == src) {
                m = (float*)dmalloc((size_t)N * L.K * 4);
                if (m && hipMemcpyAsync(m, src, (size_t)N * L.K * 4, hipMemcpyDeviceToDevice, st) != hipSuccess)
                    rc = SKIMI_ERR_HIP;
            }
            L.w = m;
            L.wdt = SKIMI_F32;
        }
        return L;
    }
    Lin linear(const std::string& p, int N, int K, int prec, bool bias = true) {
        Lin L = pack_matrix(raw(p + ".weight", (int64_t)N * K), N, K, prec);
        if (bias) L.b = keep(p + ".bias", N);
        return L;
    }
    Lin linear_named(const std::string& wkey, const std::string& bkey, int N, int K, int prec) {
        Lin L = pack_matrix(raw(wkey, (int64_t)N * K), N, K, prec);
        L.b = keep(bkey, N);
        return L;
    }
    void add_records(Lin& L) {
        const size_t n = (size_t)L.N * ((L.K + 31) / 32 * 32);
        L.w_split = dmalloc(n * 4);
        if (L.w_split) rc = split_records_launch((const float*)L.w, L.K, L.N, L.K, L.w_split, st);
    }
    ConvW conv(const std::string& p, int Co, int Ci, int k, int stride, int pad, int prec, bool bias) {
        ConvW c;
        c.k = k; c.stride = stride; c.pad = pad; c.cin = Ci;
        float* src = raw(p + ".weight", (int64_t)Co * Ci * k * k);
        if (rc) return c;
        float* perm = src;
        float* tmp = nullptr;
        if (k > 1) {
            static const int force_tap_major = getenv("SKIMI_CONV_TAP_MAJOR") ? atoi(getenv("SKIMI_CONV_TAP_MAJOR")) : 0;
            c.kmode = (prec == SKIMI_PREC_BF16X3 && Ci % 32 == 0 && !force_tap_major) ? 2 : 1;
            if (hipMalloc((void**)&tmp, (size_t)Co * Ci * k * k * 4) != hipSuccess) { rc = SKIMI_ERR_HIP; return c; }
            if ((rc = permute_conv_launch(src, tmp, Co, Ci, k, k, st, c.kmode == 2))) return c;
            perm = tmp;
        }
        c.lin = pack_matrix(perm, Co, Ci * k * k, prec);
        if (!rc && prec == SKIMI_PREC_BF16X3 && Ci % 32 == 0 && ((k == 3 && Co >= 96) || (k == 1 && Co >= 512)))
            add_records(c.lin);
        if (tmp) { (void)hipStreamSynchronize(st); (void)hipFree(tmp); }
        if (bias) c.lin.b = keep(p + ".bias", Co);
        return c;
    }
    Lin convT(const std::string& p, int C, int s, int prec) {
        Lin L;
        float* src = raw(p + ".weight", (int64_t)C * C * s * s);
        float* bsrc = raw(p + ".bias", C);
        if (rc) return L;
        float* tmp = nullptr;
        if (hipMalloc((void**)&tmp, (size_t)C * C * s * s * 4) != hipSuccess) { rc = SKIMI_ERR_HIP; return L; }
        if ((rc = permute_convT_launch(src, tmp, C, C, s, st))) return L;
        L = pack_matrix(tmp, s * s * C, C, prec);
        if (!rc && prec == SKIMI_PREC_BF16X3 && C % 32 == 0) add_records(L);
        (void)hipStreamSynchronize(st);
        (void)hipFree(tmp);
        L.b = (float*)dmalloc((size_t)s * s * C * 4);
// ... 17 lines not shown
        (void)hipStreamSynchronize(st);
        (void)hipFree(tmp);
        return L;
    }
    void add_fp8(Lin& L, const std::string& p, int N, int K) {
        if (rc) return;
        const size_t Kp = align_up((size_t)K, 128);
        L.wq = dmalloc((size_t)N * Kp);
        L.wq_scales = dmalloc((size_t)N * (Kp / 32));
        if (L.wq && L.wq_scales) rc = quant_mx_launch(raw(p + ".weight", (int64_t)N * K), SKIMI_F32, K, N, K, L.wq, L.wq_scales, st);
    }
    BlockW block(const std::string& p, int C, int hidden, bool qk_norm, int hd, int prec_in) {
        BlockW b;
        const bool fp8 = prec_in == SKIMI_PREC_FP8 && C % 32 == 0 && hidden % 32 == 0;
        const int prec = prec_in == SKIMI_PREC_FP8 ? SKIMI_PREC_BF16 : prec_in;
        b.n1 = ln(p + ".norm1", C);
        b.n2 = ln(p + ".norm2", C);
        b.qkv = linear(p + ".attn.qkv", 3 * C, C, prec);
        b.proj = linear(p + ".attn.proj", C, C, prec);
        b.fc1 = linear(p + ".mlp.fc1", hidden, C, prec);
        b.fc2 = linear(p + ".mlp.fc2", C, hidden, prec);
        if (!rc && prec == SKIMI_PREC_BF16X3 && C % 32 == 0 && hidden % 32 == 0) {
            add_records(b.qkv);
            add_records(b.proj);
            add_records(b.fc1);
            add_records(b.fc2);
        }
        if (fp8) {
            add_fp8(b.qkv, p + ".attn.qkv", 3 * C, C);
            if (!(getenv("SKIMI_FP8_PROJ") && atoi(getenv("SKIMI_FP8_PROJ")) == 0)) add_fp8(b.proj, p + ".attn.proj", C, C);
            add_fp8(b.fc1, p + ".mlp.fc1", hidden, C);
            add_fp8(b.fc2, p + ".mlp.fc2", C, hidden);
        }
        b.ls1 = keep(p + ".ls1.gamma", C);
        b.ls2 = keep(p + ".ls2.gamma", C);
        if (qk_norm) {
            b.qn_w = keep(p + ".attn.q_norm.weight", hd);
            b.qn_b = keep(p + ".attn.q_norm.bias", hd);
            b.kn_w = keep(p + ".attn.k_norm.weight", hd);
            b.kn_b = keep(p + ".attn.k_norm.bias", hd);
        }
        return b;
    }
    DptW dpt(const std::string& p, int D, int features, const int* oc, int n_out, bool feature_only, int prec) {
        DptW d;
        d.features = features;
        d.n_out = n_out;
        d.feature_only = feature_only;
        for (int i = 0; i < 4; ++i) d.oc[i] = oc[i];
        d.norm = ln(p + ".norm", D);
        for (int i = 0; i < 4; ++i) {
            d.proj[i] = linear(p + ".projects." + std::to_string(i), oc[i], D, prec);
            if (!rc && prec == SKIMI_PREC_BF16X3 && oc[i] >= 512 && D % 32 == 0) add_records(d.proj[i]);
        }
        d.rs0 = convT(p + ".resize_layers.0", oc[0], 4, prec);
        d.rs1 = convT(p + ".resize_layers.1", oc[1], 2, prec);
        d.rs3 = conv(p + ".resize_layers.3", oc[3], oc[3], 3, 2, 1, prec, true);
        for (int i = 0; i < 4; ++i)
            d.rn[i] = conv(p + ".scratch.layer" + std::to_string(i + 1) + "_rn", features, oc[i], 3, 1, 1, prec, false);
        if (h->dpt_fold && prec == SKIMI_PREC_BF16X3 && features % 32 == 0 && features > 128)
            for (int i = 0; i < 2; ++i)
                if (oc[i] % 32 == 0)
                    d.fold[i] = conv_fold(p + ".resize_layers." + std::to_string(i), p + ".scratch.layer" + std::to_string(i + 1) + "_rn",
                                          oc[i], features, i == 0 ? 4 : 2);
        for (int r = 0; r < 4; ++r) {
            const std::string rp = p + ".scratch.refinenet" + std::to_string(r + 1);
            FusionW& f = d.ref[r];
            f.out_conv = linear(rp + ".out_conv", features, features, prec);
            if (!rc && prec == SKIMI_PREC_BF16X3 && features % 32 == 0) add_records(f.out_conv);
            f.has_r1 = r != 3;
            if (f.has_r1) {
                f.r1c1 = conv(rp + ".resConfUnit1.conv1", features, features, 3, 1, 1, prec, true);
                f.r1c2 = conv(rp + ".resConfUnit1.conv2", features, features, 3, 1, 1, prec, true);
            }
            f.r2c1 = conv(rp + ".resConfUnit2.conv1", features, features, 3, 1, 1, prec, true);
            f.r2c2 = conv(rp + ".resConfUnit2.conv2", features, features, 3, 1, 1, prec, true);
        }
        if (feature_only) {
            d.oc1 = conv(p + ".scratch.output_conv1", features, features, 3, 1, 1, prec, true);
        } else {
            d.oc1 = conv(p + ".scratch.output_conv1", features / 2, features, 3, 1, 1, prec, true);
            d.oc2a = conv(p + ".scratch.output_conv2.0", 32, features / 2, 3, 1, 1, prec, true);
            if (!rc && prec == SKIMI_PREC_BF16X3 && (features / 2) % 32 == 0) {
                const int Ci = features / 2;
                float* src = raw(p + ".scratch.output_conv2.0.weight", (int64_t)32 * Ci * 9);
                d.oc2a_direct = (unsigned short*)dmalloc((size_t)32 * Ci * 9 * 2 * 2);
                if (!rc && d.oc2a_direct) rc = conv_direct_pack_launch(src, d.oc2a_direct, Ci, st);
                if (!rc && hipStreamSynchronize(st) != hipSuccess) rc = SKIMI_ERR_HIP;
            }
            d.oc2b_w = keep(p + ".scratch.output_conv2.2.weight", (int64_t)n_out * 32);
            d.oc2b_b = keep(p + ".scratch.output_conv2.2.bias", n_out);
        }
        return d;
    }
};

struct Ctx {
    skimi_vggt* h;
    hipStream_t st;
    const ShapeTabs* tabs = nullptr;
    Arena ar;
    int rc = SKIMI_OK;
    void* slab = nullptr;
    size_t slab_bytes = 0;

    bool dry() const { return ar.dry; }
    static int act_dt(int prec) { return prec == SKIMI_PREC_BF16X3 ? SKIMI_F32 : prec == SKIMI_PREC_F16 ? SKIMI_F16 : SKIMI_BF16; }
    static size_t esz(int dt) { return dt == SKIMI_F32 ? 4 : 2; }

    void gemm(skimi_gemm_desc& d) {
        const size_t mk = ar.mark();
        if (d.W_split != nullptr && d.a_dtype != SKIMI_BF16X3_REC) {
            d.x3_scratch_bytes = gemm_x3dma_scratch_bytes(&d);
            d.x3_scratch = ar.alloc(d.x3_scratch_bytes);
        }
        if (!rc && !dry()) rc = gemm_dispatch(&d, st, slab, slab_bytes, 0);
        ar.release(mk);
    }
    skimi_gemm_desc desc(const Lin& L, const void* A, int a_dt, long lda, int M, void* out, int out_dt, long ldo) {
        skimi_gemm_desc d;
        memset(&d, 0, sizeof d);
        d.M = M; d.N = L.N; d.K = L.K;
        d.A = A; d.a_dtype = a_dt; d.lda = lda;
        d.W = L.w; d.w_dtype = L.wdt; d.ldw = L.K;
        d.prec = L.prec;
        d.splitk_scratch_zeroed = 1;
        d.W_split = L.w_split;
        d.bias = L.b;
        d.out = out; d.out_dtype = out_dt; d.ldo = ldo;
        return d;
    }
    void conv_geom(skimi_gemm_desc& d, const ConvW& c, int N, int H, int W, int OH, int OW) {
        if (c.k == 1 && c.stride == 1) return;
        d.a_mode = c.kmode;
        d.cN = N; d.cH = H; d.cW = W; d.cC = c.cin; d.KH = c.k; d.KW = c.k;
        d.stride = c.stride; d.pad = c.pad; d.dil = 1; d.OH = OH; d.OW = OW;
    }
    void ln(const float* x, const float* x2, long ldx, long rows, int C, const LNw& w, float eps, void* out, int odt,
            long grp_rows = 0, long grp_stride = 0, long grp_off = 0) {
        if (rc || dry()) return;
        rc = layernorm_launch(x, x2, ldx, rows, C, w.g, w.b, eps, out, odt, C, st, grp_rows, grp_stride, grp_off);
    }
    void copy(void* dst, const void* src, size_t bytes) {
        if (rc || dry()) return;
        if (hipMemcpyAsync(dst, src, bytes, hipMemcpyDeviceToDevice, st) != hipSuccess) {
            set_error("hipMemcpyAsync failed");
            rc = SKIMI_ERR_HIP;
        }
    }
};

struct BlockBufs { void* xn; void* qkv; void* ao; void* hid; void* q8 = nullptr; void* q8s = nullptr; };

void run_block(Ctx& c, const BlockW& w, float* x, int batch, int seq, int C, int heads, float eps, bool rope,
               const BlockBufs& b) {
    const int M = batch * seq;
    const int prec = w.qkv.prec;
    const int adt = Ctx::act_dt(prec);
    const int qdt = adt == SKIMI_F16 ? SKIMI_BF16 : adt;
    const int hidden = w.fc1.N;
    const bool fp8 = w.qkv.wq != nullptr && b.q8 != nullptr;
    const bool ln_mx = fp8 && C % 256 == 0;
    const bool hid_mx = fp8 && gemm_fp8_mx_output_ok(M, hidden);
    const bool ao_mx = fp8 && w.proj.wq != nullptr && attention_mx_output_ok(qdt, heads, C / heads);
    auto as_records = [&](skimi_gemm_desc d, void* rec, size_t rec_bytes) {
        d.A = rec; d.a_dtype = SKIMI_BF16X3_REC;
        d.x3_scratch = (char*)rec + rec_bytes; d.x3_scratch_bytes = 256;
        return d;
    };
    const bool x3 = adt == SKIMI_F32 && C % 256 == 0;
    auto d_qkv = c.desc(w.qkv, b.xn, adt, C, M, b.qkv, qdt, 3 * C);
    bool rec_qkv = false;
    if (x3) {
        const auto q = as_records(d_qkv, b.xn, (size_t)M * C * 4);
        if ((rec_qkv = gemm_x3dma_eligible(&q))) d_qkv = q;
    }
    if (ln_mx) {
        if (!c.rc && !c.dry()) c.rc = layernorm_mx_launch(x, C, M, C, w.n1.g, w.n1.b, eps, b.q8, b.q8s, c.st);
    } else {
        c.ln(x, nullptr, C, M, C, w.n1, eps, b.xn, rec_qkv ? SKIMI_BF16X3_REC : adt);
    }
    if (fp8) {
        if (!ln_mx && !c.rc && !c.dry()) c.rc = quant_mx_launch(b.xn, SKIMI_BF16, C, M, C, b.q8, b.q8s, c.st);
        if (!c.rc && !c.dry())
            c.rc = gemm_fp8_launch(b.q8, b.q8s, w.qkv.wq, w.qkv.wq_scales, M, 3 * C, C, w.qkv.b, SKIMI_ACT_NONE, nullptr, nullptr, 0,
                                   b.qkv, SKIMI_BF16, 3 * C, c.st);
    } else {
        c.gemm(d_qkv);
    }
    int q_scaled = 0;
    if (!c.rc && !c.dry() && (w.qn_w || rope)) {
        const float q_scale = (1.0f / sqrtf((float)(C / heads))) * 1.44269504088896340736f;
        c.rc = qknorm_rope_launch(b.qkv, qdt, M, heads, w.qn_w, w.qn_b, w.kn_w, w.kn_b, 1e-5f, rope ? c.tabs->pos : nullptr,
                                  c.tabs->rope_cos, c.tabs->rope_sin, c.tabs->rope_npos, c.st, q_scale,
                                  qdt == SKIMI_BF16 && C / heads == 64 ? &q_scaled : nullptr);
    }
    auto d_proj = c.desc(w.proj, b.ao, adt, C, M, x, SKIMI_F32, C);
    d_proj.gamma = w.ls1; d_proj.resid = x; d_proj.ldr = C;
    int ao_rec = 0;
    if (x3 && C / heads == 64) {
        const auto q = as_records(d_proj, b.ao, (size_t)M * C * 4);
        ao_rec = gemm_x3dma_eligible(&q) ? 1 : 0;
    }
    if (!c.rc && !c.dry())
        c.rc = attention_launch(b.qkv, b.ao, qdt, batch, seq, heads, C / heads, c.st, q_scaled, adt == SKIMI_F32 ? b.hid : nullptr,
                                adt == SKIMI_F32 ? (size_t)M * hidden * 4 : 0, &ao_rec, adt == SKIMI_F16,
                                ao_mx ? b.q8 : nullptr, ao_mx ? b.q8s : nullptr);
    if (ao_rec && !c.dry()) d_proj = as_records(d_proj, b.ao, (size_t)M * C * 4);
    if (fp8 && w.proj.wq) {
        if (!ao_mx && !c.rc && !c.dry()) c.rc = quant_mx_launch(b.ao, SKIMI_BF16, C, M, C, b.q8, b.q8s, c.st);
        if (!c.rc && !c.dry())
            c.rc = gemm_fp8_launch(b.q8, b.q8s, w.proj.wq, w.proj.wq_scales, M, C, C, w.proj.b, SKIMI_ACT_NONE, w.ls1, x, C, x,
                                   SKIMI_F32, C, c.st);
    } else {
        c.gemm(d_proj);
    }
    auto d_fc1 = c.desc(w.fc1, b.xn, adt, C, M, b.hid, adt, hidden);
    d_fc1.act = SKIMI_ACT_GELU;
    auto d_fc2 = c.desc(w.fc2, b.hid, adt, hidden, M, x, SKIMI_F32, C);
    d_fc2.gamma = w.ls2; d_fc2.resid = x; d_fc2.ldr = C;
    bool rec_fc1 = false;
    if (x3) {
        const auto q1 = as_records(d_fc1, b.xn, (size_t)M * C * 4);
        if ((rec_fc1 = gemm_x3dma_eligible(&q1))) d_fc1 = q1;
        const auto q2 = as_records(d_fc2, b.hid, (size_t)M * hidden * 4);
        if (hidden % 32 == 0 && gemm_x3dma_eligible(&q2)) {
            d_fc2 = q2;
            d_fc1.out = nullptr;
            d_fc1.out_records = b.hid;
        }
    }
    if (ln_mx) {
        if (!c.rc && !c.dry()) c.rc = layernorm_mx_launch(x, C, M, C, w.n2.g, w.n2.b, eps, b.q8, b.q8s, c.st);
    } else {
        c.ln(x, nullptr, C, M, C, w.n2, eps, b.xn, rec_fc1 ? SKIMI_BF16X3_REC : adt);
    }
    if (fp8) {
        if (!ln_mx && !c.rc && !c.dry()) c.rc = quant_mx_launch(b.xn, SKIMI_BF16, C, M, C, b.q8, b.q8s, c.st);
        unsigned char* hq = (unsigned char*)b.hid;
        unsigned char* hs = hq + (size_t)M * hidden;
        if (hid_mx) {
            if (!c.rc && !c.dry())
                c.rc = gemm_fp8_launch(b.q8, b.q8s, w.fc1.wq, w.fc1.wq_scales, M, hidden, C, w.fc1.b, SKIMI_ACT_GELU, nullptr, nullptr, 0,
                                       hq, SKIMI_FP8MX, hidden, c.st, hs);
        } else {
            if (!c.rc && !c.dry())
                c.rc = gemm_fp8_launch(b.q8, b.q8s, w.fc1.wq, w.fc1.wq_scales, M, hidden, C, w.fc1.b, SKIMI_ACT_GELU, nullptr, nullptr, 0,
                                       b.hid, SKIMI_BF16, hidden, c.st);
            if (!c.rc && !c.dry()) c.rc = quant_mx_launch(b.hid, SKIMI_BF16, hidden, M, hidden, b.q8, b.q8s, c.st);
            hq = (unsigned char*)b.q8;
            hs = (unsigned char*)b.q8s;
        }
        if (!c.rc && !c.dry())
            c.rc = gemm_fp8_launch(hq, hs, w.fc2.wq, w.fc2.wq_scales, M, C, hidden, w.fc2.b, SKIMI_ACT_NONE, w.ls2, x, C, x,
                                   SKIMI_F32, C, c.st);
        return;
    }
    c.gemm(d_fc1);
    c.gemm(d_fc2);
}

const UvTab* find_uv(const ShapeTabs* h, int w, int hh, int C) {
    if (!h) return nullptr;
    for (const auto& t : h->uv)
        if (t.w == w && t.h == hh && t.C == C) return &t;
    return nullptr;
}

bool dpt_fused_ln(const DptW& w, int f2, int udt) {
    static const bool off = getenv("SKIMI_TRACK_LN_FUSED") && !atoi(getenv("SKIMI_TRACK_LN_FUSED"));
    return !off && w.feature_only && w.out_ln != nullptr && w.out_ln->g != nullptr && w.out_ln->b != nullptr && f2 == 128 && udt == SKIMI_F32;
}

void* run_dpt(Ctx& c, const DptW& w, float* const* sf, float* const* sg, int F, int P, int nsp, int ph, int pw, int C,
              int H, int W, float* pts, float* conf, int act_mode) {
    const int prec = w.proj[0].prec;
    const int adt = Ctx::act_dt(prec);
    const size_t es = Ctx::esz(adt);
    const int D = 2 * C, np = ph * pw, feat = w.features;
    const size_t mk = c.ar.mark();
    int hh[4] = {ph * 4, ph * 2, ph, (ph - 1) / 2 + 1};
    int ww[4] = {pw * 4, pw * 2, pw, (pw - 1) / 2 + 1};
    void* rn[4];
    for (int i = 0; i < 4; ++i) rn[i] = c.ar.alloc((size_t)F * hh[i] * ww[i] * feat * es);
    auto rec_bytes = [&](int lvl) { return (size_t)F * hh[lvl] * ww[lvl] * feat * 4 + 256; };
    auto takes_records = [&](const Lin& L, const ConvW* cw, int lvl) {
        if (adt != SKIMI_F32 || feat % 32 != 0 || L.w_split == nullptr) return false;
        char* fake = (char*)(uintptr_t)0x10000000;
        auto d = c.desc(L, fake, SKIMI_BF16X3_REC, feat, F * hh[lvl] * ww[lvl], fake, adt, L.N);
        if (cw) c.conv_geom(d, *cw, F, hh[lvl], ww[lvl], hh[lvl], ww[lvl]);
        d.x3_scratch = fake + rec_bytes(lvl) - 256;
        d.x3_scratch_bytes = 256;
        return gemm_x3dma_eligible(&d);
    };
    bool use_rec[4];
    char* rn_rec[4] = {nullptr, nullptr, nullptr, nullptr};
    for (int i = 0; i < 4; ++i) {
        use_rec[i] = takes_records(w.ref[i].r2c1.lin, &w.ref[i].r2c1, i);
        if (use_rec[i]) rn_rec[i] = (char*)c.ar.alloc(rec_bytes(i));
    }
    {
        const size_t mk2 = c.ar.mark();
        void* lnb = c.ar.alloc((size_t)F * np * D * es);
        void* lnb_rec = adt == SKIMI_F32 ? c.ar.alloc((size_t)F * np * D * 4 + 256) : nullptr;
        for (int i = 0; i < 4; ++i) {
            const size_t mk3 = c.ar.mark();
            void* t0 = c.ar.alloc((size_t)F * np * w.oc[i] * es);
            {
                auto d = c.desc(w.proj[i], lnb, adt, D, F * np, t0, adt, w.oc[i]);
                bool rec_in = false;
                if (adt == SKIMI_F32 && D % 256 == 0 && w.proj[i].w_split != nullptr) {
                    auto q = d;
                    q.a_dtype = SKIMI_BF16X3_REC;
                    q.x3_scratch = (char*)lnb_rec + (size_t)F * np * D * 4;
                    q.x3_scratch_bytes = 256;
                    q.A = lnb_rec;
                    rec_in = gemm_x3dma_eligible(&q);
                    if (rec_in) d = q;
                }
                c.ln(sf[i], sg[i], C, (long)F * np, D, w.norm, 1e-5f, rec_in ? lnb_rec : lnb, rec_in ? SKIMI_BF16X3_REC : adt, np, P, nsp);
                c.gemm(d);
            }
            if (i < 2 && adt == SKIMI_F32 && w.fold[i].w_split != nullptr) {
                const size_t t0_bytes = (size_t)F * np * w.oc[i] * 4;
                char* fake = (char*)(uintptr_t)0x10000000;
                auto d = c.desc(w.fold[i], fake, SKIMI_BF16X3_REC, w.oc[i], F * np, fake, adt, feat);
                d.a_mode = 3; d.store_mode = 2; d.ps_s = i == 0 ? 4 : 2; d.ps_C = feat;
                d.cN = F; d.cH = ph; d.cW = pw; d.cC = w.oc[i];
                d.x3_scratch = fake + t0_bytes; d.x3_scratch_bytes = 256;
                d.act = SKIMI_ACT_RELU;
                if (gemm_x3dma_eligible(&d)) {
                    char* t0_rec = (char*)c.ar.alloc(t0_bytes + 256);
                    const UvTab* t = w.pos_embed ? find_uv(c.tabs, pw, ph, w.oc[i]) : nullptr;
                    if (w.pos_embed && !t && !c.rc && !c.dry()) { set_error("uv table missing"); c.rc = SKIMI_ERR_STATE; }
                    if (!c.rc && !c.dry())
                        c.rc = add_uv_pos_records_launch((const float*)t0, t ? t->tx : nullptr, t ? t->ty : nullptr, F, ph, pw, w.oc[i],
                                                         t0_rec, c.st);
                    d.A = t0_rec;
                    d.x3_scratch = t0_rec + t0_bytes;
                    d.out = rn[i];
                    d.out_records = rn_rec[i];
                    c.gemm(d);
                    c.ar.release(mk3);
                    continue;
                }
            }
            if (w.pos_embed && !c.rc && !c.dry()) {
                const UvTab* t = find_uv(c.tabs, pw, ph, w.oc[i]);
                if (!t) { set_error("uv table missing"); c.rc = SKIMI_ERR_STATE; }
                else c.rc = add_uv_pos_launch(t0, adt, t->tx, t->ty, F, ph, pw, w.oc[i], c.st);
            }
            void* t1 = t0;
            if (i == 0 || i == 1) {
                const int s = i == 0 ? 4 : 2;
                const Lin& L = i == 0 ? w.rs0 : w.rs1;
                t1 = c.ar.alloc((size_t)F * hh[i] * ww[i] * w.oc[i] * es);
                auto d = c.desc(L, t0, adt, w.oc[i], F * np, t1, adt, w.oc[i]);
                d.store_mode = 1; d.ps_s = s; d.ps_C = w.oc[i];
                d.cN = F; d.cH = ph; d.cW = pw;
                c.gemm(d);
            } else if (i == 3) {
                t1 = c.ar.alloc((size_t)F * hh[i] * ww[i] * w.oc[i] * es);
                auto d = c.desc(w.rs3.lin, t0, adt, w.oc[i], F * hh[i] * ww[i], t1, adt, w.oc[i]);
                c.conv_geom(d, w.rs3, F, ph, pw, hh[i], ww[i]);
                c.gemm(d);
            }
            {
                auto d = c.desc(w.rn[i].lin, t1, adt, w.oc[i], F * hh[i] * ww[i], rn[i], adt, feat);
                c.conv_geom(d, w.rn[i], F, hh[i], ww[i], hh[i], ww[i]);
                d.act = SKIMI_ACT_RELU;
                d.out_records = rn_rec[i];
                c.gemm(d);
            }
            c.ar.release(mk3);
        }
        c.ar.release(mk2);
    }
    void* prev = nullptr;
    char* prev_rec = nullptr;
    for (int r = 3; r >= 0; --r) {
        const FusionW& f = w.ref[r];
        const int h0 = hh[r], w0 = ww[r];
        const int M = F * h0 * w0;
        const size_t bytes = (size_t)M * feat * es;
        const bool recs = use_rec[r];
        auto conv_in = [&](const ConvW& cw, const void* in_f32, char* in_rec, void* out_f32, char* out_rec) {
            auto d = c.desc(cw.lin, recs ? (const void*)in_rec : in_f32, recs ? SKIMI_BF16X3_REC : adt, feat, M, out_f32, adt, feat);
            c.conv_geom(d, cw, F, h0, w0, h0, w0);
            if (recs) {
                d.x3_scratch = in_rec + rec_bytes(r) - 256;
                d.x3_scratch_bytes = 256;
            }
            d.out_records = out_rec;
            return d;
        };
        void* cur;
        char* cur_rec = nullptr;
        void* tmp = recs ? nullptr : c.ar.alloc(bytes);
        char* tmp_rec = recs ? (char*)c.ar.alloc(rec_bytes(r)) : nullptr;
        if (f.has_r1) {
            cur = c.ar.alloc(bytes);
            if (recs) cur_rec = (char*)c.ar.alloc(rec_bytes(r));
            auto d1 = conv_in(f.r1c1, rn[r], rn_rec[r], tmp, tmp_rec);
            d1.act = SKIMI_ACT_RELU;
            c.gemm(d1);
            auto d2 = conv_in(f.r1c2, tmp, tmp_rec, cur, cur_rec);
            d2.resid = rn[r]; d2.ldr = feat; d2.resid_dtype = adt;
            d2.resid2 = prev; d2.ldr2 = feat;
            d2.post_act = SKIMI_ACT_RELU;
            c.gemm(d2);
        } else {
            cur = rn[r];
            cur_rec = rn_rec[r];
        }
        const bool u_recs = recs && takes_records(f.out_conv, nullptr, r);
        void* u = u_recs ? nullptr : c.ar.alloc(bytes);
        char* u_rec = u_recs ? (char*)c.ar.alloc(rec_bytes(r)) : nullptr;
        {
            auto d1 = conv_in(f.r2c1, cur, cur_rec, tmp, tmp_rec);
            d1.act = SKIMI_ACT_RELU;
            c.gemm(d1);
            auto d2 = conv_in(f.r2c2, tmp, tmp_rec, u, u_rec);
            d2.resid = cur; d2.ldr = feat; d2.resid_dtype = adt;
            c.gemm(d2);
        }
        const int h1 = r > 0 ? hh[r - 1] : 2 * h0, w1 = r > 0 ? ww[r - 1] : 2 * w0;
        void* olow = c.ar.alloc(bytes);
        {
            auto d = c.desc(f.out_conv, u_recs ? (const void*)u_rec : u, u_recs ? SKIMI_BF16X3_REC : adt, feat, M, olow, adt, feat);
            if (u_recs) {
                d.x3_scratch = u_rec + rec_bytes(r) - 256;
                d.x3_scratch_bytes = 256;
            }
            c.gemm(d);
        }
        if (r == 0 && adt == SKIMI_F32 && w.oc1.lin.w_split != nullptr && feat % 32 == 0) {
            const size_t rec_bytes = (size_t)F * h1 * w1 * feat * 4;
            const size_t mk_rec = c.ar.mark();
            char* rec = (char*)c.ar.alloc(rec_bytes + 256);
            auto d = c.desc(w.oc1.lin, rec, SKIMI_BF16X3_REC, feat, F * h1 * w1, nullptr, adt, w.feature_only ? feat : feat / 2);
            c.conv_geom(d, w.oc1, F, h1, w1, h1, w1);
            d.x3_scratch = rec + rec_bytes;
            d.x3_scratch_bytes = 256;
            d.out = rec;
            if (gemm_x3dma_eligible(&d)) {
                prev_rec = rec;
                if (!c.rc && !c.dry())
                    c.rc = bilinear_ac_planes_launch((const float*)olow, (unsigned short*)rec, F, h0, w0, h1, w1, feat, c.st,
                                                     nullptr, nullptr, 1, rec + rec_bytes);
                prev = nullptr;
                hh[r] = h1; ww[r] = w1;
                continue;
            }
            c.ar.release(mk_rec);
        }
        void* o = c.ar.alloc((size_t)F * h1 * w1 * feat * es);
        if (!c.rc && !c.dry()) c.rc = bilinear_ac_launch(olow, o, adt, F, h0, w0, h1, w1, feat, c.st);
        prev = o;
        hh[r] = h1; ww[r] = w1;
    }
    const int h1 = hh[0], w1 = ww[0];
    const int f2 = w.feature_only ? feat : feat / 2;
    void* c1 = c.ar.alloc((size_t)F * h1 * w1 * f2 * es);
    if (prev_rec != nullptr) {
        auto d = c.desc(w.oc1.lin, prev_rec, SKIMI_BF16X3_REC, feat, F * h1 * w1, c1, adt, f2);
        c.conv_geom(d, w.oc1, F, h1, w1, h1, w1);
        d.x3_scratch = prev_rec + (size_t)F * h1 * w1 * feat * 4;
        d.x3_scratch_bytes = 256;
        if (!c.rc && !c.dry()) c.rc = gemm_dispatch(&d, c.st, c.slab, c.slab_bytes, 0);
    } else {
        auto d = c.desc(w.oc1.lin, prev, adt, feat, F * h1 * w1, c1, adt, f2);
        c.conv_geom(d, w.oc1, F, h1, w1, h1, w1);
        c.gemm(d);
    }
    const int Ho = ph * c.h->cfg.patch_size / w.down_ratio, Wo = pw * c.h->cfg.patch_size / w.down_ratio;
    const UvTab* uvt = w.pos_embed ? find_uv(c.tabs, Wo, Ho, f2) : nullptr;
    if (w.pos_embed && !uvt && !c.rc && !c.dry()) { set_error("uv table missing"); c.rc = SKIMI_ERR_STATE; }
    static const int no_direct = getenv("SKIMI_CONV_DIRECT") ? !atoi(getenv("SKIMI_CONV_DIRECT")) : 0;
    const bool direct = !w.feature_only && w.oc2a_direct != nullptr && adt == SKIMI_F32 && !no_direct;
    void* c2 = nullptr;
    if (direct) {
        const size_t pe = (size_t)F * Ho * Wo * f2;
        unsigned short* rec = (unsigned short*)c.ar.alloc(pe * 4);
        c2 = c.ar.alloc((size_t)F * Ho * Wo * 32 * es);
        if (!c.rc && !c.dry())
            c.rc = bilinear_ac_planes_launch((const float*)c1, rec, F, h1, w1, Ho, Wo, f2, c.st, uvt ? uvt->tx : nullptr,
                                             uvt ? uvt->ty : nullptr);
        if (!c.rc && !c.dry())
            c.rc = conv_direct_n32_launch(rec, rec + f2, w.oc2a_direct, w.oc2a.lin.b, (float*)c2, F, Ho, Wo, f2, 1, c.st,
                                          2L * f2);
    } else {
        const int udt = (w.feature_only && w.out_f32) ? SKIMI_F32 : adt;
        void* c1u = c.ar.alloc((size_t)F * Ho * Wo * f2 * Ctx::esz(udt));
        if (!c.rc && !c.dry())
            c.rc = dpt_fused_ln(w, f2, udt)
                       ? bilinear_ac_launch(c1, c1u, adt, F, h1, w1, Ho, Wo, f2, c.st, uvt ? uvt->tx : nullptr, uvt ? uvt->ty : nullptr, udt,
                                            w.out_ln->g, w.out_ln->b, 1e-5f)
                       : bilinear_ac_launch(c1, c1u, adt, F, h1, w1, Ho, Wo, f2, c.st, uvt ? uvt->tx : nullptr, uvt ? uvt->ty : nullptr, udt);
        if (w.feature_only) return c1u;
        c2 = c.ar.alloc((size_t)F * Ho * Wo * 32 * es);
        auto d = c.desc(w.oc2a.lin, c1u, adt, f2, F * Ho * Wo, c2, adt, 32);
        c.conv_geom(d, w.oc2a, F, Ho, Wo, Ho, Wo);
        d.act = SKIMI_ACT_RELU;
        c.gemm(d);
    }
    if (!c.rc && !c.dry())
        c.rc = dpt_out_launch(c2, adt, w.oc2b_w, w.oc2b_b, w.n_out, pts, conf, (long)F * Ho * Wo, act_mode, c.st);
    c.ar.release(mk);
    (void)H; (void)W;
    return nullptr;
}

#define TRACK_PART 2
#include "track_impl.inc"
#undef TRACK_PART

void run_camera(Ctx& c, const CamW& w, const float* sf, const float* sg, int B, int S, int P, int C, float* out_list,
                float* out_last) {
    const skimi_vggt_config& cfg = c.h->cfg;
    const int R = B * S, D = 2 * C;
    const size_t mk = c.ar.mark();
    float* pose_tokens = (float*)c.ar.alloc((size_t)R * D * 4);
    float* xn = (float*)c.ar.alloc((size_t)R * D * 4);
    float* xc = (float*)c.ar.alloc((size_t)R * D * 4);
    float* e = (float*)c.ar.alloc((size_t)R * D * 4);
    float* mod = (float*)c.ar.alloc((size_t)R * 3 * D * 4);
    float* pred16 = (float*)c.ar.alloc((size_t)R * 16 * 4);
    float* t2 = (float*)c.ar.alloc((size_t)R * (D / 2) * 4);
    float* delta = (float*)c.ar.alloc((size_t)R * 9 * 4);
    BlockBufs bb;
    bb.xn = c.ar.alloc((size_t)R * D * 4 + 256);
    bb.qkv = c.ar.alloc((size_t)R * 3 * D * 4);
    bb.ao = c.ar.alloc((size_t)R * D * 4 + 256);
    bb.hid = c.ar.alloc((size_t)R * 4 * D * 4 + 256);
    c.ln(sf, sg, (long)P * C, R, D, w.token_norm, 1e-5f, pose_tokens, SKIMI_F32);
    LNw none;
    for (int it = 0; it < cfg.cam_iters; ++it) {
        if (it == 0 && !c.rc && !c.dry()) c.rc = tile_vec_launch(w.empty16, pred16, 16, R, c.st);
        {
            auto d = c.desc(w.embed_pose, pred16, SKIMI_F32, 16, R, e, SKIMI_F32, D);
            d.act = SKIMI_ACT_SILU;
            c.gemm(d);
        }
        {
            auto d = c.desc(w.poseLN, e, SKIMI_F32, D, R, mod, SKIMI_F32, 3 * D);
            c.gemm(d);
        }
        c.ln(pose_tokens, nullptr, D, R, D, none, 1e-6f, xn, SKIMI_F32);
        if (!c.rc && !c.dry()) c.rc = adaln_launch(xn, pose_tokens, mod, xc, R, D, c.st);
        for (const BlockW& b : w.trunk) run_block(c, b, xc, B, S, D, cfg.cam_heads, 1e-5f, false, bb);
        c.ln(xc, nullptr, D, R, D, w.trunk_norm, 1e-5f, xn, SKIMI_F32);
        {
            auto d = c.desc(w.fc1, xn, SKIMI_F32, D, R, t2, SKIMI_F32, D / 2);
            d.act = SKIMI_ACT_GELU;
            c.gemm(d);
        }
        {
            auto d = c.desc(w.fc2, t2, SKIMI_F32, D / 2, R, delta, SKIMI_F32, 9);
            c.gemm(d);
        }
        float* dst = out_list ? out_list + (size_t)it * R * 9 : (it == cfg.cam_iters - 1 ? out_last : xn );
        if (!c.rc && !c.dry()) c.rc = pose_update_launch(delta, pred16, dst, R, it == 0, c.st);
        if (it == cfg.cam_iters - 1 && out_list && out_last) c.copy(out_last, dst, (size_t)R * 9 * 4);
    }
    c.ar.release(mk);
}

int prepare(skimi_vggt* h, int F, int S, int H, int W, const ShapeTabs** out) {
    auto& entries = h->tabs[std::make_pair(H, W)];
    int largest = 0;
    for (const auto& e : entries) {
        if (e->frames >= F) {
            *out = e.get();
            return SKIMI_OK;
        }
        largest = std::max(largest, e->frames);
    }
    const ShapeTabs* first = entries.empty() ? nullptr : entries.front().get();
    const int cap = std::max(F, 2 * largest);
    (void)S;
    std::unique_ptr<ShapeTabs> tabs(new ShapeTabs());
    ShapeTabs* t_ = tabs.get();
    t_->frames = cap;
    const skimi_vggt_config& cfg = h->cfg;
    const int p = cfg.patch_size, ph = H / p, pw = W / p, nsp = 1 + cfg.num_register_tokens, P = nsp + ph * pw;
    auto up = [&](const void* src, size_t bytes, void** dst) -> int {
        SKIMI_HIP(hipMalloc(dst, bytes));
        t_->owned.push_back(*dst);
        SKIMI_HIP(hipMemcpy(*dst, src, bytes, hipMemcpyHostToDevice));
        return SKIMI_OK;
    };
    int rc;
    if (cfg.use_dino) {
        const bool native = H == W && H == cfg.dino_img_size;
        t_->dino_pos = native ? h->dino_pos : h->dino_pos_alt.at({H, W});
    }
    std::vector<int> pos((size_t)cap * P * 2, 0);
    for (int f = 0; f < cap; ++f)
        for (int y = 0; y < ph; ++y)
            for (int x = 0; x < pw; ++x) {
                const size_t i = ((size_t)f * P + nsp + (size_t)y * pw + x) * 2;
                pos[i] = y + 1;
                pos[i + 1] = x + 1;
            }
    if ((rc = up(pos.data(), pos.size() * 4, (void**)&t_->pos))) return rc;
    if (first) {
        t_->rope_cos = first->rope_cos; t_->rope_sin = first->rope_sin; t_->rope_npos = first->rope_npos;
        t_->uv = first->uv;
        *out = t_;
        entries.push_back(std::move(tabs));
        return SKIMI_OK;
    }
    const int npos = std::max(ph, pw) + 1;
    std::vector<float> cs((size_t)npos * 16), sn((size_t)npos * 16);
    for (int i = 0; i < 16; ++i) {
        const float expo = (float)(2 * i) / 32.0f;
        const float inv = 1.0f / powf(100.0f, expo);
        for (int q = 0; q < npos; ++q) {
            const float a = (float)q * inv;
            cs[(size_t)q * 16 + i] = cosf(a);
            sn[(size_t)q * 16 + i] = sinf(a);
        }
    }
    if ((rc = up(cs.data(), cs.size() * 4, (void**)&t_->rope_cos))) return rc;
    if ((rc = up(sn.data(), sn.size() * 4, (void**)&t_->rope_sin))) return rc;
    t_->rope_npos = npos;
    auto add_uv = [&](int w, int hh, int C) -> int {
        if (find_uv(t_, w, hh, C)) return SKIMI_OK;
        const double aspect = (double)W / (double)H;
        const double diag = sqrt(aspect * aspect + 1.0);
        const double sx = aspect / diag, sy = 1.0 / diag;
        const int half = C / 2, quarter = C / 4;
        std::vector<float> tx((size_t)w * half), ty((size_t)hh * half);
        auto fill = [&](std::vector<float>& tab, int n, double span) {
            const float lo = (float)(-span * (n - 1) / n), hi = (float)(span * (n - 1) / n);
            const float step = n > 1 ? (hi - lo) / (float)(n - 1) : 0.f;
            for (int i = 0; i < n; ++i) {
                const float pv = i < n / 2 ? lo + step * (float)i : hi - step * (float)(n - 1 - i);
                for (int j = 0; j < quarter; ++j) {
                    const double omega = 1.0 / pow(100.0, (double)j / (double)quarter);
                    const double a = (double)pv * omega;
                    tab[(size_t)i * half + j] = (float)sin(a) * 0.1f;
                    tab[(size_t)i * half + quarter + j] = (float)cos(a) * 0.1f;
                }
            }
        };
        fill(tx, w, sx);
        fill(ty, hh, sy);
        UvTab t{w, hh, C, nullptr, nullptr};
        int r2;
        if ((r2 = up(tx.data(), tx.size() * 4, (void**)&t.tx))) return r2;
        if ((r2 = up(ty.data(), ty.size() * 4, (void**)&t.ty))) return r2;
        t_->uv.push_back(t);
        return SKIMI_OK;
    };
    if (cfg.enable_depth || cfg.enable_point) {
        for (int i = 0; i < 4; ++i)
            if ((rc = add_uv(pw, ph, cfg.dpt_out_channels[i]))) return rc;
        if ((rc = add_uv(pw * p, ph * p, cfg.dpt_features / 2))) return rc;
    }
    *out = t_;
    entries.push_back(std::move(tabs));
    return SKIMI_OK;
}

int forward_impl(skimi_vggt* h, Ctx& c, const float* images, const float* query, int B, int S, int H, int W, int nq,
                 const skimi_vggt_outputs* out) {
    const skimi_vggt_config& cfg = h->cfg;
    const int p = cfg.patch_size, C = cfg.embed_dim, ph = H / p, pw = W / p, np = ph * pw;
    const int nsp = 1 + cfg.num_register_tokens, P = nsp + np, F = B * S, M = F * P;
    const int prec = cfg.prec, adt = Ctx::act_dt(prec);
    const size_t es = Ctx::esz(adt);

    c.slab_bytes = std::max<size_t>((size_t)F * 6 * C * 4 * 4 * 4, 4u << 20);
    c.slab = c.ar.alloc(c.slab_bytes);
    if (!c.dry() && hipMemsetAsync(c.slab, 0, c.slab_bytes, c.st) != hipSuccess) c.rc = SKIMI_ERR_HIP;

    float* x = (float*)c.ar.alloc((size_t)M * C * 4);
    std::vector<int> keep;
    auto want = [&](int l) { for (int k : keep) if (k == l) return; keep.push_back(l); };
    const bool run_depth = cfg.enable_depth && out && (out->depth || out->depth_conf);
    const bool run_point = cfg.enable_point && out && (out->world_points || out->world_points_conf);
    const bool run_cam = cfg.enable_camera && out && (out->pose_enc || out->pose_enc_list);
    const bool do_track = cfg.enable_track && out && out->track && query && nq > 0;
    if (run_depth || run_point || do_track) for (int i = 0; i < 4; ++i) want(cfg.dpt_layers[i]);
    if (run_cam || (out && out->tokens_last)) want(cfg.depth - 1);
    std::map<int, std::pair<float*, float*>> saved;
    for (int l : keep) {
        float* a = (float*)c.ar.alloc((size_t)M * C * 4);
        float* b = (float*)c.ar.alloc((size_t)M * C * 4);
        saved[l] = {a, b};
    }
    {
        const size_t mk = c.ar.mark();
        BlockBufs bb;
        bb.xn = c.ar.alloc((size_t)M * C * es + 256);
        bb.qkv = c.ar.alloc((size_t)M * 3 * C * es);
        bb.ao = c.ar.alloc((size_t)M * C * es + 256);
        bb.hid = c.ar.alloc((size_t)M * 4 * C * es + 256);
        if (cfg.prec == SKIMI_PREC_FP8) {
            const size_t kp = align_up((size_t)4 * C, 128);
            bb.q8 = c.ar.alloc((size_t)M * kp);
            bb.q8s = c.ar.alloc((size_t)M * (kp / 32));
        }
        void* pa = c.ar.alloc((size_t)F * np * h->patch_kp * es);
        if (!c.rc && !c.dry()) c.rc = patch_gather_launch(images, pa, adt, F, H, W, p, h->patch_kp, c.st);
        {
            auto d = c.desc(h->patch_proj, pa, adt, h->patch_kp, F * np, x, SKIMI_F32, C);
            d.out_rows_per_batch = np; d.out_batch_stride = P; d.out_row_off = nsp;
            if (cfg.use_dino) {
                const bool native = H == W && H == cfg.dino_img_size;
                (void)native;
                d.resid = c.tabs ? c.tabs->dino_pos : h->dino_pos; d.ldr = C;
                d.resid_rows_per_batch = np; d.resid_batch_stride = 0; d.resid_row_off = 1;
            }
            c.gemm(d);
        }
        if (cfg.use_dino) {
            if (!c.rc && !c.dry()) c.rc = special_tokens_launch(x, h->dino_special, F, S, P, nsp, C, c.st);
            for (const BlockW& b : h->dino) run_block(c, b, x, F, P, C, cfg.dino_heads, 1e-6f, false, bb);
            c.ln(x, nullptr, C, M, C, h->dino_norm, 1e-6f, x, SKIMI_F32);
        }
        if (!c.rc && !c.dry()) c.rc = special_tokens_launch(x, h->agg_special, F, S, P, nsp, C, c.st);
        for (int i = 0; i < cfg.depth && !c.rc; ++i) {
            run_block(c, h->frame[i], x, F, P, C, cfg.num_heads, 1e-5f, true, bb);
            auto it = saved.find(i);
            if (it != saved.end()) c.copy(it->second.first, x, (size_t)M * C * 4);
            run_block(c, h->global[i], x, B, S * P, C, cfg.num_heads, 1e-5f, true, bb);
            if (it != saved.end()) c.copy(it->second.second, x, (size_t)M * C * 4);
        }
        c.ar.release(mk);
    }
    if (out && out->tokens_last && !c.rc && !c.dry()) {
        auto& sv = saved[cfg.depth - 1];
        if (hipMemcpy2DAsync(out->tokens_last, (size_t)2 * C * 4, sv.first, (size_t)C * 4, (size_t)C * 4, M,
                             hipMemcpyDeviceToDevice, c.st) != hipSuccess ||
            hipMemcpy2DAsync(out->tokens_last + C, (size_t)2 * C * 4, sv.second, (size_t)C * 4, (size_t)C * 4, M,
                             hipMemcpyDeviceToDevice, c.st) != hipSuccess) {
            set_error("hipMemcpy2DAsync failed");
            c.rc = SKIMI_ERR_HIP;
        }
    }
    if (run_cam) {
        auto& sv = saved[cfg.depth - 1];
        run_camera(c, h->cam, sv.first, sv.second, B, S, P, C, out->pose_enc_list, out->pose_enc);
    }
    float* sf[4];
    float* sg[4];
    if (run_depth || run_point || do_track)
        for (int i = 0; i < 4; ++i) {
            sf[i] = saved[cfg.dpt_layers[i]].first;
            sg[i] = saved[cfg.dpt_layers[i]].second;
        }
    if (run_depth) {
        float* pts = out->depth ? out->depth : (float*)c.ar.alloc((size_t)F * H * W * 4);
        float* cf = out->depth_conf ? out->depth_conf : (float*)c.ar.alloc((size_t)F * H * W * 4);
        run_dpt(c, h->depth, sf, sg, F, P, nsp, ph, pw, C, H, W, pts, cf, 0);
    }
    if (run_point) {
        float* pts = out->world_points ? out->world_points : (float*)c.ar.alloc((size_t)F * H * W * 3 * 4);
        float* cf = out->world_points_conf ? out->world_points_conf : (float*)c.ar.alloc((size_t)F * H * W * 4);
        run_dpt(c, h->point, sf, sg, F, P, nsp, ph, pw, C, H, W, pts, cf, 1);
    }
    if (do_track) run_track(c, sf, sg, B, S, P, nsp, ph, pw, C, H, W, query, nq, out->track, out->vis, out->conf);
    return c.rc;
}

}

extern "C" {

skimi_vggt* skimi_vggt_create(const skimi_vggt_config* cfg) {
    if (!cfg) { set_error("skimi_vggt_create: null config"); return nullptr; }
    if (cfg->embed_dim <= 0 || cfg->num_heads <= 0 || cfg->embed_dim / cfg->num_heads != 64 ||
        cfg->embed_dim % cfg->num_heads != 0) {
        set_error("skimi_vggt_create: embed_dim / num_heads must be 64");
        return nullptr;
    }
    if (cfg->use_dino && cfg->embed_dim / cfg->dino_heads != 64) {
        set_error("skimi_vggt_create: DINOv2 head_dim must be 64");
        return nullptr;
    }
    if (cfg->patch_size <= 0 || cfg->depth <= 0 || cfg->num_register_tokens < 0) {
        set_error("skimi_vggt_create: bad sizes");
        return nullptr;
    }
    for (int i = 0; i < 4; ++i)
        if (cfg->dpt_layers[i] < 0 || cfg->dpt_layers[i] >= cfg->depth) {
            set_error("skimi_vggt_create: dpt_layers[%d] = %d outside [0, depth)", i, cfg->dpt_layers[i]);
            return nullptr;
        }
    if (cfg->prec < SKIMI_PREC_BF16 || cfg->prec > SKIMI_PREC_F16) {
        set_error("skimi_vggt_create: prec %d is not one of SKIMI_PREC_BF16 / BF16X3 / FP8 / F16", cfg->prec);
        return nullptr;
    }
    if (cfg->head_prec != SKIMI_PREC_BF16 && cfg->head_prec != SKIMI_PREC_BF16X3 && cfg->head_prec != SKIMI_PREC_F16) {
        set_error("skimi_vggt_create: head_prec %d: the depth / point heads run in SKIMI_PREC_BF16X3 (the reference's fp32) or, as a "
                  "faster, less accurate option, on SKIMI_PREC_F16 / SKIMI_PREC_BF16 operands", cfg->head_prec);
        return nullptr;
    }
    skimi_vggt* h = new skimi_vggt();
    h->cfg = *cfg;
    h->dpt_fold = !(getenv("SKIMI_DPT_FOLD") && atoi(getenv("SKIMI_DPT_FOLD")) == 0);
    return h;
}

void skimi_vggt_destroy(skimi_vggt* h) {
    if (!h) return;
    for (auto& kv : h->raw) (void)hipFree(kv.second.first);
    for (void* p : h->owned) (void)hipFree(p);
    h->tabs.clear();
    for (auto& kv : h->dino_pos_alt) (void)hipFree(kv.second);
    delete h;
}

int skimi_vggt_set_weight(skimi_vggt* h, const char* key, const float* data, int64_t n, int32_t on_device) {
    SKIMI_CHECK_ARG(h && key && data && n > 0, "skimi_vggt_set_weight: bad arguments");
    float* d = nullptr;
    SKIMI_HIP(hipMalloc((void**)&d, (size_t)n * 4));
    hipError_t e = hipMemcpy(d, data, (size_t)n * 4, on_device ? hipMemcpyDeviceToDevice : hipMemcpyHostToDevice);
    if (e != hipSuccess) {
        (void)hipFree(d);
        set_error("skimi_vggt_set_weight: copy failed: %s", hipGetErrorString(e));
        return SKIMI_ERR_HIP;
    }
    auto it = h->raw.find(key);
    if (it != h->raw.end()) (void)hipFree(it->second.first);
    h->raw[key] = {d, n};
    h->finalized = false;
    return SKIMI_OK;
}

int skimi_vggt_set_pos_embed(skimi_vggt* h, int32_t H, int32_t W, const float* pos_embed, int32_t on_device) {
    SKIMI_CHECK_ARG(h && pos_embed && h->cfg.use_dino, "skimi_vggt_set_pos_embed: needs a DINOv2 model and a table");
    const int p = h->cfg.patch_size;
    SKIMI_CHECK_ARG(H > 0 && W > 0 && H % p == 0 && W % p == 0, "skimi_vggt_set_pos_embed: bad size %dx%d", H, W);
    const size_t n = ((size_t)(H / p) * (W / p) + 1) * h->cfg.embed_dim;
    float* d = nullptr;
    SKIMI_HIP(hipMalloc((void**)&d, n * 4));
    hipError_t e = hipMemcpy(d, pos_embed, n * 4, on_device ? hipMemcpyDeviceToDevice : hipMemcpyHostToDevice);
    if (e != hipSuccess) {
        (void)hipFree(d);
        set_error("skimi_vggt_set_pos_embed: copy failed: %s", hipGetErrorString(e));
        return SKIMI_ERR_HIP;
    }
    std::lock_guard<std::mutex> lk(h->prep_mu);
    auto it = h->dino_pos_alt.find({H, W});
    if (it != h->dino_pos_alt.end()) {
        e = hipMemcpy(it->second, d, n * 4, hipMemcpyDeviceToDevice);
        (void)hipFree(d);
        if (e != hipSuccess) {
            set_error("skimi_vggt_set_pos_embed: copy failed: %s", hipGetErrorString(e));
            return SKIMI_ERR_HIP;
        }
        return SKIMI_OK;
    }
    h->dino_pos_alt[{H, W}] = d;
    return SKIMI_OK;
}

int skimi_vggt_finalize(skimi_vggt* h) {
    SKIMI_CHECK_ARG(h, "skimi_vggt_finalize: null handle");
    const skimi_vggt_config& cfg = h->cfg;
    for (void* p : h->owned) (void)hipFree(p);
    h->owned.clear();
    Packer pk{h};
    const int C = cfg.embed_dim, p = cfg.patch_size, R = cfg.num_register_tokens, nsp = 1 + R;
    const int hidden = 4 * C, D = 2 * C;
    const std::string A = "aggregator";
    const int kraw = 3 * p * p;
    const std::string pe = cfg.use_dino ? A + ".patch_embed.patch_embed.proj" : A + ".patch_embed.proj";
    h->patch_proj = pk.linear(pe, C, kraw, cfg.prec == SKIMI_PREC_FP8 ? SKIMI_PREC_BF16 : cfg.prec);
    h->patch_kp = h->patch_proj.K;
    if (cfg.use_dino) {
        const std::string d = A + ".patch_embed";
        const int g = cfg.dino_img_size / p, np0 = g * g;
        h->dino_pos = pk.keep(d + ".pos_embed", (int64_t)(np0 + 1) * C);
        float* cls = pk.raw(d + ".cls_token", C);
        float* reg = R ? pk.raw(d + ".register_tokens", (int64_t)R * C) : nullptr;
        (void)pk.raw(d + ".mask_token", C);
        h->dino_special = (float*)pk.dmalloc((size_t)2 * nsp * C * 4);
// ... 139 lines not shown
```

### skiing_analysis_pytorch_amd/ops.py

```python
from __future__ import annotations

import ctypes as C
from typing import NamedTuple, Optional

import torch

from . import _lib
from ._lib import ACT_NONE, BF16, F16, F32, PREC_BF16, PREC_BF16X3, GemmDesc, check, lib, ptr


def _dt(t: torch.Tensor) -> int:
    if t.dtype == torch.float32:
        return F32
    if t.dtype == torch.bfloat16:
        return BF16
    if t.dtype == torch.float16:
        return F16
    raise TypeError(f"unsupported dtype {t.dtype}")


def _require_cuda(*ts):
    for t in ts:
        if t is not None and not t.is_cuda:
            raise _lib.SkimiError("libskimi ops need device (HBM) tensors; got a CPU tensor")
# ... 14 lines not shown
    d.W, d.w_dtype = ptr(w), _dt(w)
    if a_records is not None:
        _require_cuda(a_records)
        d.A, d.a_dtype = ptr(a_records), _lib.BF16X3_REC
        d.lda = lda if lda is not None else (conv["C"] if conv is not None else K)
    else:
        _require_cuda(a)
        d.A, d.a_dtype = ptr(a), _dt(a)
        d.lda = lda if lda is not None else a.stride(-2) if a.dim() >= 2 else a.shape[-1]
    dev = w.device
    d.ldw = w.stride(0)
    d.prec = prec
    if conv is not None:
        d.a_mode = 2 if conv.get("slice_major") else 1
        d.cN, d.cH, d.cW, d.cC = conv["N"], conv["H"], conv["W"], conv["C"]
        d.KH, d.KW, d.stride, d.pad, d.dil = conv["KH"], conv["KW"], conv["stride"], conv["pad"], conv["dil"]
        d.OH, d.OW = conv["OH"], conv["OW"]
        d.M = d.cN * d.OH * d.OW
    else:
        d.M = M if M is not None else a.shape[0]
    if records_only:
        assert out is None and out_records is not None and pixel_shuffle is None
        d.out_dtype = _lib.F32
    elif pixel_shuffle is not None:
        s, cout, n_img, h, w_ = pixel_shuffle
        d.store_mode, d.ps_s, d.ps_C = 1, s, cout
        d.cN, d.cH, d.cW = n_img, h, w_
        if out is None:
            out = torch.empty((n_img, h * s, w_ * s, cout), dtype=out_dtype, device=dev)
        d.ldo = out.stride(-2)
    else:
        if out is None:
            out = torch.empty((d.M, N), dtype=out_dtype, device=dev)
        d.ldo = out.stride(-2)
    if not records_only:
        d.out, d.out_dtype = ptr(out), _dt(out)
    if out2 is not None:
        if out is None or (out2.dtype == torch.float32) == (out.dtype == torch.float32) or \
                (out.dtype == torch.float32 and out2.dtype != torch.bfloat16):
            raise _lib.SkimiError("gemm: out2 is the other dtype of out (bf16 next to fp32, fp32 next to 16-bit)")
        d.out2, d.ldo2 = ptr(out2), out2.stride(-2)
    if out_map is not None:
        d.out_rows_per_batch, d.out_batch_stride, d.out_row_off = out_map
    d.bias, d.gamma, d.resid = ptr(bias), ptr(gamma), ptr(resid)
    if resid is not None:
        d.ldr = resid.stride(-2)
        d.resid_dtype = _dt(resid)
    if resid2 is not None:
        d.resid2, d.ldr2 = ptr(resid2), resid2.stride(-2)
        d.resid_dtype = _dt(resid2)
    if resid_map is not None:
        d.resid_rows_per_batch, d.resid_batch_stride, d.resid_row_off = resid_map
    d.act = act
    d.post_act = post_act
    if splitk_scratch is not None:
        d.splitk_scratch = ptr(splitk_scratch)
        d.splitk_scratch_bytes = splitk_scratch.numel() * splitk_scratch.element_size()
    d.force_splitk = force_splitk
    d.splitk_scratch_zeroed = int(splitk_zeroed)
    if w_split is not None:
        d.W_split = ptr(w_split)
        if a_records is not None:
            d.x3_scratch = ptr(a_records) + a_records.numel() * 2 - 256
            d.x3_scratch_bytes = 256
        else:
            d.x3_scratch = ptr(x3_scratch)
            d.x3_scratch_bytes = x3_scratch.numel() * x3_scratch.element_size()
    if out_records is not None:
        _require_cuda(out_records)
        d.out_records = ptr(out_records)
    check(lib().skimi_gemm(C.byref(d), _lib.current_stream()), "skimi_gemm")
    return out


class GemmPath(NamedTuple):
    family: Optional[str]
    tile: Optional[str]
    loop: Optional[str]
    mfma: Optional[int]
    epi: int
    splitk: int
    raw: int


_PATH_FAMILY = {1: "generic", 2: "splitk_ordered", 3: "splitk_atomic", 4: "x3dma_wide", 5: "x3dma_narrow",
                6: "gemm256", 7: "conv_win"}
_PATH_TILE = {1: "64x64", 2: "128x64", 3: "128x128"}
_PATH_LOOP = {1: "two_phase_256", 2: "two_phase_192", 3: "ping_pong", 4: "single_stream"}


def gemm_last_path() -> GemmPath:
    v = int(lib().skimi_gemm_last_path())
    fam = _PATH_FAMILY.get(v & 15)
    sub = (v >> 4) & 15
    generic = fam in ("generic", "splitk_ordered", "splitk_atomic")
    return GemmPath(family=fam, tile=_PATH_TILE.get(sub) if generic else None,
                    loop=_PATH_LOOP.get(sub) if fam == "gemm256" else None,
                    mfma={1: 16, 2: 32}.get((v >> 8) & 15), epi=(v >> 12) & 15, splitk=(v >> 16) & 255, raw=v)


def layernorm(x, gamma=None, beta=None, eps=1e-5, *, x2=None, out_dtype=torch.float32):
    _require_cuda(x, x2, gamma, beta)
    rows = x.numel() // x.shape[-1]
    Cc = x.shape[-1] * (2 if x2 is not None else 1)
    out = torch.empty((*x.shape[:-1], Cc), dtype=out_dtype, device=x.device)
    check(lib().skimi_layernorm(ptr(x), ptr(x2), x.stride(-2), rows, Cc, ptr(gamma), ptr(beta), eps, ptr(out),
                                _dt(out), Cc, _lib.current_stream()), "skimi_layernorm")
    return out


def qknorm_rope_(qkv, heads, qn_w=None, qn_b=None, kn_w=None, kn_b=None, eps=1e-5, pos=None, rope_cos=None,
                 rope_sin=None, *, q_scale=None):
    _require_cuda(qkv, pos, rope_cos, rope_sin)
    tokens = qkv.numel() // (3 * heads * 64)
    npos = rope_cos.shape[0] if rope_cos is not None else 0
    if q_scale is not None:
        flag = C.c_int32(0)
        check(lib().skimi_qknorm_rope_scaled(ptr(qkv), _dt(qkv), tokens, heads, ptr(qn_w), ptr(qn_b), ptr(kn_w), ptr(kn_b),
                                             eps, ptr(pos), ptr(rope_cos), ptr(rope_sin), npos, q_scale, C.byref(flag),
                                             _lib.current_stream()), "skimi_qknorm_rope_scaled")
        return qkv, bool(flag.value)
    check(lib().skimi_qknorm_rope(ptr(qkv), _dt(qkv), tokens, heads, ptr(qn_w), ptr(qn_b), ptr(kn_w), ptr(kn_b),
                                  eps, ptr(pos), ptr(rope_cos), ptr(rope_sin), npos, _lib.current_stream()),
          "skimi_qknorm_rope")
    return qkv


def attention_x3_scratch_bytes(tokens, row_elems):
    return int(lib().skimi_attention_x3_scratch_bytes(tokens, row_elems))


def attention(qkv, batch, seq, heads, head_dim, out_dtype=None, *, q_prescaled=0, x3_scratch=None, out_records=False,
              out=None):
    _require_cuda(qkv)
    if q_prescaled or x3_scratch is not None or out_records or out is not None:
        return _attention_ex(qkv, batch, seq, heads, head_dim, out_dtype, q_prescaled, x3_scratch, out_records, out)
    if isinstance(out_dtype, str):
        assert out_dtype == "fp8mx", out_dtype
        rows, Kp = batch * seq, (heads * head_dim + 127) // 128 * 128
        buf = torch.zeros(rows * (Kp + Kp // 32), dtype=torch.uint8, device=qkv.device)
        check(lib().skimi_attention_out(ptr(qkv), ptr(buf), _dt(qkv), _lib.FP8MX, batch, seq, heads, head_dim,
                                        _lib.current_stream()), "skimi_attention_out")
        return buf[:rows * Kp].view(rows, Kp), buf[rows * Kp:].view(rows, Kp // 32)
    out = torch.empty((batch * seq, heads * head_dim), dtype=out_dtype or qkv.dtype, device=qkv.device)
    if out_dtype is None or out_dtype == qkv.dtype:
        check(lib().skimi_attention(ptr(qkv), ptr(out), _dt(qkv), batch, seq, heads, head_dim, _lib.current_stream()),
              "skimi_attention")
    else:
        check(lib().skimi_attention_out(ptr(qkv), ptr(out), _dt(qkv), _dt(out), batch, seq, heads, head_dim,
                                        _lib.current_stream()), "skimi_attention_out")
    return out


def _attention_ex(qkv, batch, seq, heads, head_dim, out_dtype, q_prescaled, x3_scratch, out_records, out):
    _require_cuda(x3_scratch, out)
    rows, Cc = batch * seq, heads * head_dim
    flag = C.c_int32(1 if out_records else 0)
    sc_bytes = x3_scratch.numel() * x3_scratch.element_size() if x3_scratch is not None else 0
    mx = isinstance(out_dtype, str)
    if mx:
        assert out_dtype == "fp8mx", out_dtype
        odt, Kp = _lib.FP8MX, (Cc + 127) // 128 * 128
        need = rows * (Kp + Kp // 32)
        if out is None:
            out = torch.zeros(need, dtype=torch.uint8, device=qkv.device)
    else:
        odt = {torch.float32: F32, torch.bfloat16: BF16, torch.float16: F16}[out_dtype or qkv.dtype]
        need = rows * Cc * (4 if odt == F32 else 2) + (256 if out_records else 0)
        if out is None:
            out = records_buffer(rows, Cc, qkv.device) if out_records else \
                torch.empty((rows, Cc), dtype=out_dtype or qkv.dtype, device=qkv.device)
    assert out.numel() * out.element_size() >= need, "attention: `out` is too small"
    check(lib().skimi_attention_ex(ptr(qkv), ptr(out), _dt(qkv), odt, batch, seq, heads, head_dim, int(q_prescaled),
                                   ptr(x3_scratch), sc_bytes, C.byref(flag), _lib.current_stream()), "skimi_attention_ex")
    if mx:
        buf = out.view(torch.uint8).reshape(-1)
        return buf[:rows * Kp].view(rows, Kp), buf[rows * Kp:need].view(rows, Kp // 32)
    return (out, bool(flag.value)) if out_records else out


def conv3x3_n32(x, w, bias=None, relu=False):
    _require_cuda(x, w, bias)
    F_, H, W_, Cc = x.shape
    assert w.shape == (32, Cc, 3, 3) and Cc % 32 == 0
    planes = split_planes(x.reshape(-1, Cc).contiguous())
    packed = torch.empty(2 * 32 * Cc * 9, dtype=torch.bfloat16, device=x.device)
    st = _lib.current_stream()
    check(lib().skimi_conv3x3_n32_pack(ptr(w.contiguous()), ptr(packed), Cc, st), "skimi_conv3x3_n32_pack")
    out = torch.empty((F_, H, W_, 32), dtype=torch.float32, device=x.device)
    check(lib().skimi_conv3x3_n32(ptr(planes[0]), ptr(planes[1]), ptr(packed), ptr(bias), ptr(out), F_, H, W_, Cc,
                                  1 if relu else 0, st), "skimi_conv3x3_n32")
    return out


def split_records(x):
    _require_cuda(x)
    rows, Cc = x.shape
    out = torch.empty((rows, (Cc + 31) // 32, 2, 32), dtype=torch.bfloat16, device=x.device)
    check(lib().skimi_split_records(ptr(x), x.stride(0), rows, Cc, ptr(out), _lib.current_stream()), "skimi_split_records")
    return out


def records_buffer(rows, Cc, device="cuda"):
    return torch.empty(rows * ((Cc + 31) // 32) * 64 + 128, dtype=torch.bfloat16, device=device)


def x3_scratch_numel(rows, Cc):
    return rows * ((Cc + 31) // 32 * 32) + 64


def dpt_fold_pack(w_T, b_T, w_rn):
    _require_cuda(w_T, b_T, w_rn)
    Ci, Cm, s, s2 = w_T.shape
    Co = w_rn.shape[0]
    assert s == s2 and w_rn.shape == (Co, Cm, 3, 3)
    rec = torch.empty((s + 2) * (s + 2) * Co * Ci * 2, dtype=torch.bfloat16, device=w_T.device)
    beta = torch.empty((9, Co), dtype=torch.float32, device=w_T.device)
    check(lib().skimi_dpt_fold_pack(ptr(w_T.contiguous()), ptr(b_T.contiguous()) if b_T is not None else None, ptr(w_rn.contiguous()),
                                    Ci, Cm, Co, s, ptr(rec), ptr(beta), _lib.current_stream()), "skimi_dpt_fold_pack")
    return rec, beta


def convT_conv3x3_folded(x, w_records, beta, s, Co, *, act=ACT_NONE, out=None, out_records=None, records_only=False,
                         a_records=None):
    _require_cuda(w_records, beta, out, out_records, a_records)
    F_, h, w_, Ci = x if a_records is not None else x.shape
    nrec = F_ * h * w_ * Ci * 2
    ar = a_records
    if ar is None:
        _require_cuda(x)
        ar = records_buffer(F_ * h * w_, Ci, device=x.device)
        ar[:nrec] = split_records(x.reshape(-1, Ci).contiguous()).reshape(-1)
        ar[nrec:] = 0
    d = GemmDesc()
    d.M, d.N, d.K = F_ * h * w_, Co, 4 * Ci
    d.A, d.a_dtype, d.lda = ptr(ar), _lib.BF16X3_REC, Ci
    d.W, d.w_dtype, d.ldw = ptr(w_records), _lib.F32, 4 * Ci
    d.W_split = ptr(w_records)
    d.x3_scratch, d.x3_scratch_bytes = ptr(ar) + nrec * 2, 256
    d.prec = PREC_BF16X3
    d.a_mode, d.store_mode, d.ps_s, d.ps_C = 3, 2, s, Co
    d.cN, d.cH, d.cW, d.cC = F_, h, w_, Ci
    d.bias, d.act = ptr(beta), act
    d.out_dtype = _lib.F32
    if not records_only:
        if out is None:
            out = torch.empty((F_, h * s, w_ * s, Co), dtype=torch.float32, device=w_records.device)
        d.out = ptr(out)
    d.ldo = Co
    if out_records is not None:
        d.out_records = ptr(out_records)
    check(lib().skimi_gemm(C.byref(d), _lib.current_stream()), "skimi_gemm")
    return out


def split_planes(x):
    _require_cuda(x)
    rows, Cc = x.shape
    out = torch.empty((2, rows, Cc), dtype=torch.bfloat16, device=x.device)
    check(lib().skimi_split_planes(ptr(x), x.stride(0), rows, Cc, ptr(out[0]), ptr(out[1]), _lib.current_stream()),
          "skimi_split_planes")
    return out


def quant_mx(x: torch.Tensor):
    _require_cuda(x)
    x = x.contiguous()
    rows, K = x.shape
    Kp = (K + 127) // 128 * 128
    q = torch.empty((rows, Kp), dtype=torch.uint8, device=x.device)
    s = torch.empty((rows, Kp // 32), dtype=torch.uint8, device=x.device)
    check(lib().skimi_quant_mx(ptr(x), _dt(x), x.stride(0), rows, K, ptr(q), ptr(s), _lib.current_stream()), "skimi_quant_mx")
    return q, s


def layernorm_mx(x, gamma, beta, eps=1e-5):
    _require_cuda(x, gamma, beta)
    rows, Cc = x.shape
    q = torch.empty((rows, Cc), dtype=torch.uint8, device=x.device)
    s = torch.empty((rows, Cc // 32), dtype=torch.uint8, device=x.device)
    check(lib().skimi_layernorm_mx(ptr(x), x.stride(0), rows, Cc, ptr(gamma), ptr(beta), eps, ptr(q), ptr(s),
                                   _lib.current_stream()), "skimi_layernorm_mx")
    return q, s


def gemm_fp8(a_q, a_s, w_q, w_s, K, *, bias=None, act=ACT_NONE, gamma=None, resid=None, out=None, out_dtype=torch.float32,
             out_mx=False):
    _require_cuda(a_q, a_s, w_q, w_s, bias, gamma, resid, out)
    M, N = a_q.shape[0], w_q.shape[0]
    Kp = (K + 127) // 128 * 128
    for t, cols, what in ((a_q, Kp, "a_q"), (w_q, Kp, "w_q"), (a_s, Kp // 32, "a_s"), (w_s, Kp // 32, "w_s")):
        if t.dtype != torch.uint8 or t.dim() != 2 or t.shape[1] != cols or not t.is_contiguous():
            raise _lib.SkimiError(f"gemm_fp8: {what} must be a contiguous uint8 [rows, {cols}] array for K = {K} "
                                  f"(got {tuple(t.shape)} {t.dtype}); operands come from quant_mx")
    if a_s.shape[0] != M or w_s.shape[0] != N:
        raise _lib.SkimiError("gemm_fp8: scale rows do not match the payload rows")
    if out_mx:
        q = torch.empty((M, N), dtype=torch.uint8, device=a_q.device)
        sc = torch.empty((M, N // 32), dtype=torch.uint8, device=a_q.device)
        check(lib().skimi_gemm_fp8(ptr(a_q), ptr(a_s), ptr(w_q), ptr(w_s), M, N, K, ptr(bias), act, None, None, 0, ptr(q),
                                   _lib.FP8MX, N, ptr(sc), _lib.current_stream()), "skimi_gemm_fp8")
        return q, sc
    if out is None:
        out = torch.empty((M, N), dtype=out_dtype, device=a_q.device)
    check(lib().skimi_gemm_fp8(ptr(a_q), ptr(a_s), ptr(w_q), ptr(w_s), M, N, K, ptr(bias), act, ptr(gamma), ptr(resid),
                               resid.stride(0) if resid is not None else 0, ptr(out), _dt(out), out.stride(0), None,
# ... 3 lines not shown
```

Baseline: 17.91.

## Fuse Q norm and RoPE into attention Q load, add tail handling and in-place kept blocks

Moves the per-head LayerNorm and RoPE of Q into the 64-query attention kernel's Q load, driven by a per-layer precomputed QPrep block, so the separate qknorm/rope pass only has to process K. It also adds a tail mode in which the last partial query block spreads 32 queries per wave and skips inactive waves. Blocks that are saved for the output now run out of place straight into the saved buffers instead of being copied afterwards. The cost is extra register pressure and per-lane loads of the norm and RoPE tables inside the attention kernel, plus more complex control flow in the hot loop.

```diff
diff --git a/include/skimi.h b/include/skimi.h
--- a/include/skimi.h
+++ b/include/skimi.h
@@ -136,6 +136,12 @@
                        uint64_t x3_scratch_bytes, int32_t* out_records, void* stream);
 uint64_t skimi_attention_x3_scratch_bytes(int64_t tokens, int64_t row_elems);
 
+uint64_t skimi_attention_qprep_bytes(void);
+int skimi_qknorm_rope_attention(void* qkv, void* out, int32_t out_dtype, int32_t batch, int32_t seq, int32_t heads,
+                                const float* qn_w, const float* qn_b, const float* kn_w, const float* kn_b,
+                                float eps, const int32_t* pos, const float* rope_cos, const float* rope_sin,
+                                int32_t rope_npos, float q_scale, void* qprep_block, int32_t* fused, void* stream);
+
 typedef struct skimi_vp3d skimi_vp3d;
 
 skimi_vp3d* skimi_vp3d_create(int32_t joints_in, int32_t in_features, int32_t joints_out,
diff --git a/skiing_analysis_pytorch_amd/_lib.py b/skiing_analysis_pytorch_amd/_lib.py
--- a/skiing_analysis_pytorch_amd/_lib.py
+++ b/skiing_analysis_pytorch_amd/_lib.py
@@ -87,6 +87,9 @@
     "skimi_attention_ex": (C.c_int, [_vp, _vp, C.c_int32, C.c_int32, C.c_int32, C.c_int32, C.c_int32, C.c_int32, C.c_int32,
                                      _vp, C.c_uint64, C.POINTER(C.c_int32), _vp]),
     "skimi_attention_x3_scratch_bytes": (C.c_uint64, [C.c_int64, C.c_int64]),
+    "skimi_attention_qprep_bytes": (C.c_uint64, []),
+    "skimi_qknorm_rope_attention": (C.c_int, [_vp, _vp, C.c_int32, C.c_int32, C.c_int32, C.c_int32, _vp, _vp, _vp, _vp, C.c_float,
+                                              _vp, _vp, _vp, C.c_int32, C.c_float, _vp, C.POINTER(C.c_int32), _vp]),
     "skimi_vp3d_create": (_vp, [C.c_int32, C.c_int32, C.c_int32, C.POINTER(C.c_int32), C.c_int32,
                                 C.c_int32, C.c_int32]),
     "skimi_vp3d_create_ex": (_vp, [C.c_int32, C.c_int32, C.c_int32, C.POINTER(C.c_int32), C.c_int32,
diff --git a/skiing_analysis_pytorch_amd/csrc/api.hip b/skiing_analysis_pytorch_amd/csrc/api.hip
--- a/skiing_analysis_pytorch_amd/csrc/api.hip
+++ b/skiing_analysis_pytorch_amd/csrc/api.hip
@@ -254,4 +254,28 @@
     return (uint64_t)attention_x3_scratch_bytes((long)tokens, (long)row_elems);
 }
 
-}
+uint64_t skimi_attention_qprep_bytes(void) { return sizeof(QPrep); }
+
+int skimi_qknorm_rope_attention(void* qkv, void* out, int32_t out_dtype, int32_t batch, int32_t seq, int32_t heads,
+                                const float* qn_w, const float* qn_b, const float* kn_w, const float* kn_b, float eps,
+                                const int32_t* pos, const float* rope_cos, const float* rope_sin, int32_t rope_npos,
+                                float q_scale, void* qprep_block, int32_t* fused, void* stream) {
+    if (fused) *fused = 0;
+    SKIMI_CHECK_ARG(qkv && out && qn_w && kn_w && pos && rope_cos && rope_sin && batch > 0 && seq > 0 && heads > 0,
+                    "skimi_qknorm_rope_attention: null argument or empty shape");
+    SKIMI_CHECK_ARG(out_dtype == SKIMI_BF16 || out_dtype == SKIMI_F16, "skimi_qknorm_rope_attention: out_dtype is SKIMI_BF16 or SKIMI_F16");
+    SKIMI_CHECK_ARG(qprep_block && ((uintptr_t)qprep_block & 15) == 0, "skimi_qknorm_rope_attention: qprep_block must be a 16-byte aligned device buffer");
+    hipStream_t st = (hipStream_t)stream;
+    const int64_t tokens = (int64_t)batch * seq;
+    int q_scaled = 0, k_only = attention_qprep_ok(SKIMI_BF16, 64);
+    int rc = qknorm_rope_launch(qkv, SKIMI_BF16, tokens, heads, qn_w, qn_b, kn_w, kn_b, eps, pos, rope_cos, rope_sin, rope_npos, st,
+                                q_scale, &q_scaled, &k_only);
+    if (rc) return rc;
+    QPrep* blk = (QPrep*)qprep_block;
+    if (k_only && (rc = qprep_fill_launch(blk, qn_w, qn_b, eps, q_scale, pos, rope_cos, rope_sin, rope_npos, st))) return rc;
+    if (fused) *fused = k_only;
+    return attention_launch(qkv, out, SKIMI_BF16, batch, seq, heads, 64, st, q_scaled, nullptr, 0, nullptr, out_dtype == SKIMI_F16,
+                            nullptr, nullptr, k_only ? blk : nullptr);
+}
+
+}
diff --git a/skiing_analysis_pytorch_amd/csrc/attention_bf16.hip b/skiing_analysis_pytorch_amd/csrc/attention_bf16.hip
--- a/skiing_analysis_pytorch_amd/csrc/attention_bf16.hip
+++ b/skiing_analysis_pytorch_amd/csrc/attention_bf16.hip
@@ -196,6 +196,13 @@
     static int use_mx = -1;
     if (use_mx < 0 || dyn) use_mx = getenv("SKIMI_ATTN_MX") ? atoi(getenv("SKIMI_ATTN_MX")) : 1;
     return use_mx && dtype == SKIMI_BF16 && head_dim == 64 && heads % 2 == 0 && q64_enabled() != 0;
+}
+
+bool attention_qprep_ok(int dtype, int head_dim) {
+    static const bool dyn = getenv("SKIMI_ENV_DYNAMIC") && atoi(getenv("SKIMI_ENV_DYNAMIC"));
+    static int use = -1;
+    if (use < 0 || dyn) use = getenv("SKIMI_ATTN_QPREP") ? atoi(getenv("SKIMI_ATTN_QPREP")) : 1;
+    return use && dtype == SKIMI_BF16 && head_dim == 64 && q64_enabled() != 0;
 }
 
 int attention_bf16_launch(const AttnArgs& a, hipStream_t st) {
@@ -220,6 +227,8 @@
 #endif
     const int q64 = q64_enabled();
     SKIMI_CHECK_ARG(!a.out_mx || q64 != 0, "skimi_attention: MXFP8 output rows are written by the 64-query kernel only");
+    SKIMI_CHECK_ARG(!a.q_prep || (q64 != 0 && a.q_batch == (long)a.seq_q * a.q_row),
+                    "skimi_attention: q's norm and RoPE in the Q load need the 64-query kernel and packed q rows");
     if (q64 != 0) {
         attention_q64_dispatch(a, st);
     } else if (a.q_prescaled) {
@@ -247,8 +256,9 @@
 
 int attention_launch(const void* qkv, void* out, int dtype, int batch, int seq, int heads, int head_dim,
                      hipStream_t st, int q_prescaled, void* x3_scratch, size_t x3_scratch_bytes, int* out_records, int out_f16,
-                     void* out_mx, void* out_mx_scales) {
+                     void* out_mx, void* out_mx_scales, const QPrep* q_prep) {
     SKIMI_CHECK_ARG(qkv && (out || out_mx), "skimi_attention: null buffer");
+    SKIMI_CHECK_ARG(!q_prep || attention_qprep_ok(dtype, head_dim), "skimi_attention: q_prep needs bf16 q / k / v, head_dim 64 and the 64-query kernel");
     SKIMI_CHECK_ARG(!out_mx || (out_mx_scales && attention_mx_output_ok(dtype, heads, head_dim)),
                     "skimi_attention: MXFP8 output needs the 64-query bf16 kernel (head_dim 64, heads even) and a scale buffer");
     const bool want_rec = out_records != nullptr && *out_records != 0;
@@ -272,6 +282,7 @@
     a.scale = 1.0f / sqrtf((float)head_dim);
     a.q_prescaled = dtype == SKIMI_F32 ? 0 : q_prescaled;
     a.out_f16 = dtype == SKIMI_F32 ? 0 : out_f16;
+    a.q_prep = q_prep;
     if (out_mx) {
         a.out_mx = out_mx;
         a.out_mx_scales = out_mx_scales;
diff --git a/skiing_analysis_pytorch_amd/csrc/attention_q64.hip b/skiing_analysis_pytorch_amd/csrc/attention_q64.hip
--- a/skiing_analysis_pytorch_amd/csrc/attention_q64.hip
+++ b/skiing_analysis_pytorch_amd/csrc/attention_q64.hip
@@ -21,7 +21,7 @@
 }
 
 template <int dbg>
-__global__ __launch_bounds__(256, 2) void attn_q64_kernel(const AttnArgs a, int nqb) {
+__global__ __launch_bounds__(256, 2) void attn_q64_kernel(const AttnArgs a, int nqb, int tail) {
     constexpr int KV = 64;
     constexpr int TILE = KV * 64 * 2;
     __shared__ __attribute__((aligned(16))) char smem[4 * TILE];
@@ -41,7 +41,9 @@
     const int qb = id % nqb;
     const int bh = id / nqb;
     const int head = bh % a.heads, b = bh / a.heads;
-    const int q0 = qb * 256 + wave * 64;
+    const bool two = !(tail && a.seq_q - qb * 256 <= 128);
+    const int q0 = qb * 256 + wave * (two ? 64 : 32);
+    const bool live = two || q0 < a.seq_q;
 
     const unsigned short* Q = (const unsigned short*)a.q + (long)b * a.q_batch + (long)head * a.q_head;
     const unsigned short* K = (const unsigned short*)a.k + (long)b * a.k_batch + (long)head * a.k_head;
@@ -56,7 +58,64 @@
 #pragma unroll
         for (int s = 0; s < 4; ++s) qf[qi][s] = *reinterpret_cast<const bf16x8*>(qp + 16 * s);
     }
-    if (!a.q_prescaled) {
+    if (a.q_prep) {
+        const QPrep* __restrict__ P = a.q_prep;
+#pragma unroll
+        for (int qi = 0; qi < 2; ++qi) {
+            if (qi == 1 && !two) break;
+            const int q = min(q0 + qi * 32 + l31, a.seq_q - 1);
+            const long tok = (long)b * a.seq_q + q;
+            float t[4][8];
+            float sum = 0.f;
+#pragma unroll
+            for (int s = 0; s < 4; ++s)
+#pragma unroll
+                for (int j = 0; j < 8; ++j) {
+                    t[s][j] = bf2f((unsigned short)qf[qi][s][j]);
+                    sum += t[s][j];
+                }
+            const float mean = xhalf_sum(sum) * (1.f / 64.f);
+            float sq = 0.f;
+#pragma unroll
+            for (int s = 0; s < 4; ++s)
+#pragma unroll
+                for (int j = 0; j < 8; ++j) {
+                    t[s][j] -= mean;
+                    sq += t[s][j] * t[s][j];
+                }
+            const float rstd = rsqrtf(xhalf_sum(sq) * (1.f / 64.f) + P->eps);
+#pragma unroll
+            for (int s = 0; s < 4; ++s) {
+                const float4 w0 = *reinterpret_cast<const float4*>(&P->qn_w[16 * s + 8 * lh]);
+                const float4 w1 = *reinterpret_cast<const float4*>(&P->qn_w[16 * s + 8 * lh + 4]);
+                const float4 b0 = *reinterpret_cast<const float4*>(&P->qn_b[16 * s + 8 * lh]);
+                const float4 b1 = *reinterpret_cast<const float4*>(&P->qn_b[16 * s + 8 * lh + 4]);
+                const float w[8] = {w0.x, w0.y, w0.z, w0.w, w1.x, w1.y, w1.z, w1.w};
+                const float bb[8] = {b0.x, b0.y, b0.z, b0.w, b1.x, b1.y, b1.z, b1.w};
+#pragma unroll
+                for (int j = 0; j < 8; ++j) t[s][j] = t[s][j] * rstd * w[j] + bb[j];
+            }
+            const float q_scale = P->q_scale;
+#pragma unroll
+            for (int sect = 0; sect < 2; ++sect) {
+                const int pp = min(max(P->pos[tok * 2 + sect], 0), P->npos - 1);
+                const float* ct = P->rope_cos + pp * 16 + 8 * lh;
+                const float* st = P->rope_sin + pp * 16 + 8 * lh;
+                const float4 c0 = *reinterpret_cast<const float4*>(ct), c1 = *reinterpret_cast<const float4*>(ct + 4);
+                const float4 s0 = *reinterpret_cast<const float4*>(st), s1 = *reinterpret_cast<const float4*>(st + 4);
+                const float cs[8] = {c0.x, c0.y, c0.z, c0.w, c1.x, c1.y, c1.z, c1.w};
+                const float sn[8] = {s0.x, s0.y, s0.z, s0.w, s1.x, s1.y, s1.z, s1.w};
+#pragma unroll
+                for (int j = 0; j < 8; ++j) {
+                    const float lo = t[2 * sect][j], hi = t[2 * sect + 1][j];
+                    const float rlo = lo * cs[j] + (-hi) * sn[j];
+                    const float rhi = hi * cs[j] + lo * sn[j];
+                    qf[qi][2 * sect][j] = (short)f2bf(rlo * q_scale);
+                    qf[qi][2 * sect + 1][j] = (short)f2bf(rhi * q_scale);
+                }
+            }
+        }
+    } else if (!a.q_prescaled) {
         const float c2q = a.scale * 1.44269504088896340736f;
 #pragma unroll
         for (int qi = 0; qi < 2; ++qi)
@@ -100,7 +159,7 @@
     bf16x8 qneg[2] = {{0, 0, 0, 0, 0, 0, 0, 0}, {0, 0, 0, 0, 0, 0, 0, 0}};
 
     issue(0, 0);
-    __builtin_amdgcn_s_waitcnt(0x0F70);
+    __builtin_amdgcn_s_waitcnt(0x0070);
     __syncthreads();
 
     for (int kt = 0; kt < nkt; ++kt) {
@@ -110,6 +169,8 @@
 
         f32x16 s[2][2];
         bf16x8 kf[2][4];
+        bf16x8 vf[2][2][2];
+        if (live) {
 #pragma unroll
         for (int t = 0; t < 2; ++t) {
             const int row = t * 32 + l31;
@@ -122,15 +183,14 @@
         for (int t = 0; t < 2; ++t) {
 #pragma unroll
             for (int qi = 0; qi < 2; ++qi)
-                s[qi][t] = __builtin_amdgcn_mfma_f32_32x32x16_bf16(kone, qneg[qi], zero16, 0, 0, 0);
+                if (qi == 0 || two) s[qi][t] = __builtin_amdgcn_mfma_f32_32x32x16_bf16(kone, qneg[qi], zero16, 0, 0, 0);
 #pragma unroll
             for (int ks = 0; ks < 4; ++ks)
 #pragma unroll
                 for (int qi = 0; qi < 2; ++qi)
-                    s[qi][t] = __builtin_amdgcn_mfma_f32_32x32x16_bf16(kf[t][ks], qf[qi][ks], s[qi][t], 0, 0, 0);
-        }
-
-        bf16x8 vf[2][2][2];
+                    if (qi == 0 || two) s[qi][t] = __builtin_amdgcn_mfma_f32_32x32x16_bf16(kf[t][ks], qf[qi][ks], s[qi][t], 0, 0, 0);
+        }
+
 #pragma unroll
         for (int t = 0; t < 2; ++t)
 #pragma unroll
@@ -152,9 +212,12 @@
                     }
                 }
 
+        }
+
         __builtin_amdgcn_sched_barrier(0);
         if (kt + 1 < nkt) issue(cur ^ 1, kt + 1);
 
+        if (live) {
         if (ragged && kt == nkt - 1) {
 #pragma unroll
             for (int qi = 0; qi < 2; ++qi)
@@ -169,6 +232,7 @@
 
 #pragma unroll
         for (int qi = 0; qi < 2; ++qi) {
+            if (qi == 1 && !two) break;
             bool redo = kt == 0;
             if (kt != 0) {
                 float l0 = 0.f, l1 = 0.f;
@@ -261,12 +325,15 @@
                 }
         }
 
+        }
+
         __builtin_amdgcn_s_waitcnt(0x0F70);
         if (!(dbg & 1)) __syncthreads();
     }
 
 #pragma unroll
     for (int qi = 0; qi < 2; ++qi) {
+        if (qi == 1 && !two) break;
         const float inv = 1.f / xhalf_sum(lsum[qi]);
         const int q = q0 + qi * 32 + l31;
         if (a.out_mx) {
@@ -317,6 +384,9 @@
 #else
     const int dbg = 0;
 #endif
+    static const bool dyn = getenv("SKIMI_ENV_DYNAMIC") && atoi(getenv("SKIMI_ENV_DYNAMIC"));
+    static int tail = -1;
+    if (tail < 0 || dyn) tail = getenv("SKIMI_ATTN_TAIL") ? atoi(getenv("SKIMI_ATTN_TAIL")) != 0 : 1;
     static const size_t pad = getenv("SKIMI_ATTN_LDSPAD") ? (size_t)atol(getenv("SKIMI_ATTN_LDSPAD")) : 0;
     if (pad) {
         static bool once = false;
@@ -324,16 +394,16 @@
             (void)hipFuncSetAttribute(reinterpret_cast<const void*>(attn_q64_kernel<0>), hipFuncAttributeMaxDynamicSharedMemorySize, (int)pad);
             once = true;
         }
-        hipLaunchKernelGGL(attn_q64_kernel<0>, dim3((unsigned)nblk), dim3(256), pad, st, a, nqb);
+        hipLaunchKernelGGL(attn_q64_kernel<0>, dim3((unsigned)nblk), dim3(256), pad, st, a, nqb, tail);
         return;
     }
     switch (dbg) {
 #ifdef SKIMI_ABLATIONS
-        case 1: hipLaunchKernelGGL(attn_q64_kernel<1>, dim3((unsigned)nblk), dim3(256), 0, st, a, nqb); break;
-        case 2: hipLaunchKernelGGL(attn_q64_kernel<2>, dim3((unsigned)nblk), dim3(256), 0, st, a, nqb); break;
-        case 3: hipLaunchKernelGGL(attn_q64_kernel<3>, dim3((unsigned)nblk), dim3(256), 0, st, a, nqb); break;
+        case 1: hipLaunchKernelGGL(attn_q64_kernel<1>, dim3((unsigned)nblk), dim3(256), 0, st, a, nqb, tail); break;
+        case 2: hipLaunchKernelGGL(attn_q64_kernel<2>, dim3((unsigned)nblk), dim3(256), 0, st, a, nqb, tail); break;
+        case 3: hipLaunchKernelGGL(attn_q64_kernel<3>, dim3((unsigned)nblk), dim3(256), 0, st, a, nqb, tail); break;
 #endif
-        default: hipLaunchKernelGGL(attn_q64_kernel<0>, dim3((unsigned)nblk), dim3(256), 0, st, a, nqb);
+        default: hipLaunchKernelGGL(attn_q64_kernel<0>, dim3((unsigned)nblk), dim3(256), 0, st, a, nqb, tail);
     }
 }
 
diff --git a/skiing_analysis_pytorch_amd/csrc/kernels.h b/skiing_analysis_pytorch_amd/csrc/kernels.h
--- a/skiing_analysis_pytorch_amd/csrc/kernels.h
+++ b/skiing_analysis_pytorch_amd/csrc/kernels.h
@@ -14,7 +14,19 @@
 int qknorm_rope_launch(void* qkv, int dtype, int64_t tokens, int heads, const float* qn_w,
                        const float* qn_b, const float* kn_w, const float* kn_b, float eps,
                        const int32_t* pos, const float* rope_cos, const float* rope_sin, int rope_npos,
-                       hipStream_t st, float q_scale = 1.f, int* q_scaled = nullptr);
+                       hipStream_t st, float q_scale = 1.f, int* q_scaled = nullptr, int* k_only = nullptr);
+
+struct alignas(16) QPrep {
+    float qn_w[64], qn_b[64];
+    float eps, q_scale;
+    const int32_t* pos;
+    const float* rope_cos;
+    const float* rope_sin;
+    int32_t npos;
+};
+int qprep_fill_launch(QPrep* block, const float* qn_w, const float* qn_b, float eps, float q_scale, const int32_t* pos,
+                      const float* rope_cos, const float* rope_sin, int npos, hipStream_t st);
+bool attention_qprep_ok(int dtype, int head_dim);
 
 struct AttnArgs {
     const void* q;
@@ -33,6 +45,7 @@
     void* out_mx = nullptr;
     void* out_mx_scales = nullptr;
     long mx_row = 0, mx_srow = 0;
+    const QPrep* q_prep = nullptr;
 };
 bool attention_mx_output_ok(int dtype, int heads, int head_dim);
 int attention_f32_launch(const AttnArgs& a, hipStream_t st);
@@ -50,7 +63,8 @@
                      hipStream_t st, int q_prescaled = 0, void* x3_scratch = nullptr, size_t x3_scratch_bytes = 0,
                      int* out_records = nullptr,
                      int out_f16 = 0,
-                     void* out_mx = nullptr, void* out_mx_scales = nullptr);
+                     void* out_mx = nullptr, void* out_mx_scales = nullptr,
+                     const QPrep* q_prep = nullptr);
 size_t attention_x3_scratch_bytes(long tokens, long row_elems);
 int attention_x3_launch(const AttnArgs& a, long tokens, long row_elems, void* scratch, size_t scratch_bytes, hipStream_t st,
                         bool out_records = false);
diff --git a/skiing_analysis_pytorch_amd/csrc/rowops.hip b/skiing_analysis_pytorch_amd/csrc/rowops.hip
--- a/skiing_analysis_pytorch_amd/csrc/rowops.hip
+++ b/skiing_analysis_pytorch_amd/csrc/rowops.hip
@@ -318,6 +318,7 @@
     return s;
 }
 
+template <bool QK>
 __global__ __launch_bounds__(256) void qknorm_rope_bf16_kernel(unsigned short* __restrict__ qkv, long tokens, int heads,
                                                                const float* __restrict__ qn_w,
                                                                const float* __restrict__ qn_b,
@@ -336,7 +337,7 @@
     float w[2][8], b[2][8];
 #pragma unroll
     for (int j = 0; j < 8; ++j) {
-        w[0][j] = qn_w[8 * sub + j]; b[0][j] = qn_b ? qn_b[8 * sub + j] : 0.f;
+        w[0][j] = QK ? qn_w[8 * sub + j] : 0.f; b[0][j] = QK && qn_b ? qn_b[8 * sub + j] : 0.f;
         w[1][j] = kn_w[8 * sub + j]; b[1][j] = kn_b ? kn_b[8 * sub + j] : 0.f;
     }
     const int sect = sub >> 2;
@@ -353,7 +354,8 @@
         const int h = (int)(ii - tok * heads);
         unsigned short* pq = qkv + ((tok * 3) * heads + h) * 64 + 8 * sub;
         unsigned short* pk = pq + (long)heads * 64;
-        const bf16x8 raw[2] = {*reinterpret_cast<const bf16x8*>(pq), *reinterpret_cast<const bf16x8*>(pk)};
+        const bf16x8 raw[2] = {QK ? *reinterpret_cast<const bf16x8*>(pq) : bf16x8{0, 0, 0, 0, 0, 0, 0, 0},
+                               *reinterpret_cast<const bf16x8*>(pk)};
         int pp = pos[tok * 2 + sect];
         pp = min(max(pp, 0), npos - 1);
         const float4 c0 = *reinterpret_cast<const float4*>(&tab[pp * 16 + d0]);
@@ -364,7 +366,7 @@
         const float st[8] = {s0.x, s0.y, s0.z, s0.w, s1.x, s1.y, s1.z, s1.w};
         bf16x8 outv[2];
 #pragma unroll
-        for (int z = 0; z < 2; ++z) {
+        for (int z = QK ? 0 : 1; z < 2; ++z) {
             float t[8];
 #pragma unroll
             for (int j = 0; j < 8; ++j) t[j] = bf2f((unsigned short)raw[z][j]);
@@ -387,7 +389,7 @@
             }
         }
         if (live) {
-            *reinterpret_cast<bf16x8*>(pq) = outv[0];
+            if (QK) *reinterpret_cast<bf16x8*>(pq) = outv[0];
             *reinterpret_cast<bf16x8*>(pk) = outv[1];
         }
     }
@@ -396,14 +398,24 @@
 int qknorm_rope_launch(void* qkv, int dtype, int64_t tokens, int heads, const float* qn_w, const float* qn_b,
                        const float* kn_w, const float* kn_b, float eps, const int32_t* pos,
                        const float* rope_cos, const float* rope_sin, int rope_npos, hipStream_t st, float q_scale,
-                       int* q_scaled) {
+                       int* q_scaled, int* k_only) {
     SKIMI_CHECK_ARG(qkv && tokens > 0 && heads > 0, "skimi_qknorm_rope: bad arguments");
     if (q_scaled) *q_scaled = 0;
+    const bool want_k_only = k_only != nullptr && *k_only != 0;
+    if (k_only) *k_only = 0;
     SKIMI_CHECK_ARG(pos == nullptr || (rope_cos && rope_sin && rope_npos > 0), "skimi_qknorm_rope: pos without tables");
     if (((uintptr_t)qkv & 15) == 0 && dtype == SKIMI_BF16 && qn_w && kn_w && pos && rope_npos * 128 <= 48 * 1024) {
         const long total = tokens * heads;
         const unsigned blocks = (unsigned)std::min<long>(cdiv(total, 32), 256 * 8);
-        hipLaunchKernelGGL(qknorm_rope_bf16_kernel, dim3(blocks), dim3(256), (size_t)rope_npos * 128, st,
+        if (want_k_only) {
+            hipLaunchKernelGGL(qknorm_rope_bf16_kernel<false>, dim3(blocks), dim3(256), (size_t)rope_npos * 128, st,
+                               (unsigned short*)qkv, (long)tokens, heads, qn_w, qn_b, kn_w, kn_b, eps, pos, rope_cos, rope_sin,
+                               rope_npos, 1.f);
+            *k_only = 1;
+            SKIMI_LAUNCH_CHECK();
+            return SKIMI_OK;
+        }
+        hipLaunchKernelGGL(qknorm_rope_bf16_kernel<true>, dim3(blocks), dim3(256), (size_t)rope_npos * 128, st,
                            (unsigned short*)qkv, (long)tokens, heads, qn_w, qn_b, kn_w, kn_b, eps, pos, rope_cos, rope_sin,
                            rope_npos, q_scaled ? q_scale : 1.f);
         if (q_scaled) *q_scaled = 1;
@@ -434,6 +446,31 @@
     return SKIMI_OK;
 }
 
+__global__ __launch_bounds__(64) void qprep_fill_kernel(QPrep* __restrict__ blk, const float* __restrict__ qn_w,
+                                                        const float* __restrict__ qn_b, float eps, float q_scale,
+                                                        const int* __restrict__ pos, const float* __restrict__ rcos,
+                                                        const float* __restrict__ rsin, int npos) {
+    const int i = threadIdx.x;
+    blk->qn_w[i] = qn_w[i];
+    blk->qn_b[i] = qn_b ? qn_b[i] : 0.f;
+    if (i == 0) {
+        blk->eps = eps;
+        blk->q_scale = q_scale;
+        blk->pos = pos;
+        blk->rope_cos = rcos;
+        blk->rope_sin = rsin;
+        blk->npos = npos;
+    }
+}
+
+int qprep_fill_launch(QPrep* block, const float* qn_w, const float* qn_b, float eps, float q_scale, const int32_t* pos,
+                      const float* rope_cos, const float* rope_sin, int npos, hipStream_t st) {
+    SKIMI_CHECK_ARG(block && qn_w && pos && rope_cos && rope_sin && npos > 0, "qprep_fill: bad arguments");
+    hipLaunchKernelGGL(qprep_fill_kernel, dim3(1), dim3(64), 0, st, block, qn_w, qn_b, eps, q_scale, pos, rope_cos, rope_sin, npos);
+    SKIMI_LAUNCH_CHECK();
+    return SKIMI_OK;
+}
+
 __global__ __launch_bounds__(256) void vp3d_im2col_kernel(const float* __restrict__ x, float* __restrict__ a0,
                                                           int B, int L, int Cin, int k, int Kpad) {
     const int Lout = L - k + 1;
diff --git a/skiing_analysis_pytorch_amd/csrc/vggt.hip b/skiing_analysis_pytorch_amd/csrc/vggt.hip
--- a/skiing_analysis_pytorch_amd/csrc/vggt.hip
+++ b/skiing_analysis_pytorch_amd/csrc/vggt.hip
@@ -88,6 +88,7 @@
     float *rope_cos = nullptr, *rope_sin = nullptr;
     int rope_npos = 0;
     const float* dino_pos = nullptr;
+    QPrep* qprep = nullptr;
     std::vector<UvTab> uv;
     std::vector<void*> owned;
     ~ShapeTabs() {
@@ -411,8 +412,8 @@
 
 struct BlockBufs { void* xn; void* qkv; void* ao; void* hid; void* q8 = nullptr; void* q8s = nullptr; };
 
-void run_block(Ctx& c, const BlockW& w, float* x, int batch, int seq, int C, int heads, float eps, bool rope,
-               const BlockBufs& b) {
+void run_block(Ctx& c, const BlockW& w, const float* x_in, float* x, float* x_out, int batch, int seq, int C, int heads, float eps, bool rope,
+               const BlockBufs& b, const QPrep* qprep = nullptr) {
     const int M = batch * seq;
     const int prec = w.qkv.prec;
     const int adt = Ctx::act_dt(prec);
@@ -435,9 +436,9 @@
         if ((rec_qkv = gemm_x3dma_eligible(&q))) d_qkv = q;
     }
     if (ln_mx) {
-        if (!c.rc && !c.dry()) c.rc = layernorm_mx_launch(x, C, M, C, w.n1.g, w.n1.b, eps, b.q8, b.q8s, c.st);
+        if (!c.rc && !c.dry()) c.rc = layernorm_mx_launch(x_in, C, M, C, w.n1.g, w.n1.b, eps, b.q8, b.q8s, c.st);
     } else {
-        c.ln(x, nullptr, C, M, C, w.n1, eps, b.xn, rec_qkv ? SKIMI_BF16X3_REC : adt);
+        c.ln(x_in, nullptr, C, M, C, w.n1, eps, b.xn, rec_qkv ? SKIMI_BF16X3_REC : adt);
     }
     if (fp8) {
         if (!ln_mx && !c.rc && !c.dry()) c.rc = quant_mx_launch(b.xn, SKIMI_BF16, C, M, C, b.q8, b.q8s, c.st);
@@ -448,14 +449,17 @@
         c.gemm(d_qkv);
     }
     int q_scaled = 0;
+    int k_only = qprep != nullptr && rope && !fp8 && attention_qprep_ok(qdt, C / heads);
     if (!c.rc && !c.dry() && (w.qn_w || rope)) {
         const float q_scale = (1.0f / sqrtf((float)(C / heads))) * 1.44269504088896340736f;
         c.rc = qknorm_rope_launch(b.qkv, qdt, M, heads, w.qn_w, w.qn_b, w.kn_w, w.kn_b, 1e-5f, rope ? c.tabs->pos : nullptr,
                                   c.tabs->rope_cos, c.tabs->rope_sin, c.tabs->rope_npos, c.st, q_scale,
-                                  qdt == SKIMI_BF16 && C / heads == 64 ? &q_scaled : nullptr);
+                                  qdt == SKIMI_BF16 && C / heads == 64 ? &q_scaled : nullptr, &k_only);
+    } else {
+        k_only = 0;
     }
     auto d_proj = c.desc(w.proj, b.ao, adt, C, M, x, SKIMI_F32, C);
-    d_proj.gamma = w.ls1; d_proj.resid = x; d_proj.ldr = C;
+    d_proj.gamma = w.ls1; d_proj.resid = x_in; d_proj.ldr = C;
     int ao_rec = 0;
     if (x3 && C / heads == 64) {
         const auto q = as_records(d_proj, b.ao, (size_t)M * C * 4);
@@ -464,19 +468,19 @@
     if (!c.rc && !c.dry())
         c.rc = attention_launch(b.qkv, b.ao, qdt, batch, seq, heads, C / heads, c.st, q_scaled, adt == SKIMI_F32 ? b.hid : nullptr,
                                 adt == SKIMI_F32 ? (size_t)M * hidden * 4 : 0, &ao_rec, adt == SKIMI_F16,
-                                ao_mx ? b.q8 : nullptr, ao_mx ? b.q8s : nullptr);
+                                ao_mx ? b.q8 : nullptr, ao_mx ? b.q8s : nullptr, k_only ? qprep : nullptr);
     if (ao_rec && !c.dry()) d_proj = as_records(d_proj, b.ao, (size_t)M * C * 4);
     if (fp8 && w.proj.wq) {
         if (!ao_mx && !c.rc && !c.dry()) c.rc = quant_mx_launch(b.ao, SKIMI_BF16, C, M, C, b.q8, b.q8s, c.st);
         if (!c.rc && !c.dry())
-            c.rc = gemm_fp8_launch(b.q8, b.q8s, w.proj.wq, w.proj.wq_scales, M, C, C, w.proj.b, SKIMI_ACT_NONE, w.ls1, x, C, x,
+            c.rc = gemm_fp8_launch(b.q8, b.q8s, w.proj.wq, w.proj.wq_scales, M, C, C, w.proj.b, SKIMI_ACT_NONE, w.ls1, x_in, C, x,
                                    SKIMI_F32, C, c.st);
     } else {
         c.gemm(d_proj);
     }
     auto d_fc1 = c.desc(w.fc1, b.xn, adt, C, M, b.hid, adt, hidden);
     d_fc1.act = SKIMI_ACT_GELU;
-    auto d_fc2 = c.desc(w.fc2, b.hid, adt, hidden, M, x, SKIMI_F32, C);
+    auto d_fc2 = c.desc(w.fc2, b.hid, adt, hidden, M, x_out, SKIMI_F32, C);
     d_fc2.gamma = w.ls2; d_fc2.resid = x; d_fc2.ldr = C;
     bool rec_fc1 = false;
     if (x3) {
@@ -511,7 +515,7 @@
             hs = (unsigned char*)b.q8s;
         }
         if (!c.rc && !c.dry())
-            c.rc = gemm_fp8_launch(hq, hs, w.fc2.wq, w.fc2.wq_scales, M, C, hidden, w.fc2.b, SKIMI_ACT_NONE, w.ls2, x, C, x,
+            c.rc = gemm_fp8_launch(hq, hs, w.fc2.wq, w.fc2.wq_scales, M, C, hidden, w.fc2.b, SKIMI_ACT_NONE, w.ls2, x, C, x_out,
                                    SKIMI_F32, C, c.st);
         return;
     }
@@ -807,7 +811,7 @@
         }
         c.ln(pose_tokens, nullptr, D, R, D, none, 1e-6f, xn, SKIMI_F32);
         if (!c.rc && !c.dry()) c.rc = adaln_launch(xn, pose_tokens, mod, xc, R, D, c.st);
-        for (const BlockW& b : w.trunk) run_block(c, b, xc, B, S, D, cfg.cam_heads, 1e-5f, false, bb);
+        for (const BlockW& b : w.trunk) run_block(c, b, xc, xc, xc, B, S, D, cfg.cam_heads, 1e-5f, false, bb);
         c.ln(xc, nullptr, D, R, D, w.trunk_norm, 1e-5f, xn, SKIMI_F32);
         {
             auto d = c.desc(w.fc1, xn, SKIMI_F32, D, R, t2, SKIMI_F32, D / 2);
@@ -863,9 +867,29 @@
                 pos[i + 1] = x + 1;
             }
     if ((rc = up(pos.data(), pos.size() * 4, (void**)&t_->pos))) return rc;
+    auto add_qprep = [&]() -> int {
+        const int hd = cfg.embed_dim / cfg.num_heads;
+        if (hd != 64) return SKIMI_OK;
+        const size_t n = (size_t)2 * cfg.depth;
+        SKIMI_HIP(hipMalloc((void**)&t_->qprep, n * sizeof(QPrep)));
+        t_->owned.push_back(t_->qprep);
+        SKIMI_HIP(hipMemset(t_->qprep, 0, n * sizeof(QPrep)));
+        const float q_scale = (1.0f / sqrtf((float)hd)) * 1.44269504088896340736f;
+        for (int i = 0; i < cfg.depth; ++i)
+            for (int g = 0; g < 2; ++g) {
+                const BlockW& w = g ? h->global[i] : h->frame[i];
+                if (!w.qn_w) continue;
+                const int r = qprep_fill_launch(t_->qprep + 2 * i + g, w.qn_w, w.qn_b, 1e-5f, q_scale, t_->pos, t_->rope_cos,
+                                                t_->rope_sin, t_->rope_npos, nullptr);
+                if (r) return r;
+            }
+        SKIMI_HIP(hipStreamSynchronize(nullptr));
+        return SKIMI_OK;
+    };
     if (first) {
         t_->rope_cos = first->rope_cos; t_->rope_sin = first->rope_sin; t_->rope_npos = first->rope_npos;
         t_->uv = first->uv;
+        if ((rc = add_qprep())) return rc;
         *out = t_;
         entries.push_back(std::move(tabs));
         return SKIMI_OK;
@@ -884,6 +908,7 @@
     if ((rc = up(cs.data(), cs.size() * 4, (void**)&t_->rope_cos))) return rc;
     if ((rc = up(sn.data(), sn.size() * 4, (void**)&t_->rope_sin))) return rc;
     t_->rope_npos = npos;
+    if ((rc = add_qprep())) return rc;
     auto add_uv = [&](int w, int hh, int C) -> int {
         if (find_uv(t_, w, hh, C)) return SKIMI_OK;
         const double aspect = (double)W / (double)H;
@@ -977,15 +1002,32 @@
         }
         if (cfg.use_dino) {
             if (!c.rc && !c.dry()) c.rc = special_tokens_launch(x, h->dino_special, F, S, P, nsp, C, c.st);
-            for (const BlockW& b : h->dino) run_block(c, b, x, F, P, C, cfg.dino_heads, 1e-6f, false, bb);
+            for (const BlockW& b : h->dino) run_block(c, b, x, x, x, F, P, C, cfg.dino_heads, 1e-6f, false, bb);
             c.ln(x, nullptr, C, M, C, h->dino_norm, 1e-6f, x, SKIMI_F32);
         }
         if (!c.rc && !c.dry()) c.rc = special_tokens_launch(x, h->agg_special, F, S, P, nsp, C, c.st);
+        static const bool dyn = getenv("SKIMI_ENV_DYNAMIC") && atoi(getenv("SKIMI_ENV_DYNAMIC"));
+        static int kept_env = -1;
+        if (kept_env < 0 || dyn) kept_env = getenv("SKIMI_KEPT_INPLACE") ? atoi(getenv("SKIMI_KEPT_INPLACE")) : 1;
+        const bool kept_inplace = kept_env != 0;
+        const float* cur = x;
+        auto qp = [&](int i, int g) -> const QPrep* {
+            const BlockW& w = g ? h->global[i] : h->frame[i];
+            return c.tabs && c.tabs->qprep && w.qn_w ? c.tabs->qprep + 2 * i + g : nullptr;
+        };
         for (int i = 0; i < cfg.depth && !c.rc; ++i) {
-            run_block(c, h->frame[i], x, F, P, C, cfg.num_heads, 1e-5f, true, bb);
             auto it = saved.find(i);
+            if (it != saved.end() && kept_inplace) {
+                run_block(c, h->frame[i], cur, x, it->second.first, F, P, C, cfg.num_heads, 1e-5f, true, bb, qp(i, 0));
+                run_block(c, h->global[i], it->second.first, x, it->second.second, B, S * P, C, cfg.num_heads, 1e-5f, true, bb,
+                          qp(i, 1));
+                cur = it->second.second;
+                continue;
+            }
+            run_block(c, h->frame[i], cur, x, x, F, P, C, cfg.num_heads, 1e-5f, true, bb, qp(i, 0));
+            cur = x;
             if (it != saved.end()) c.copy(it->second.first, x, (size_t)M * C * 4);
-            run_block(c, h->global[i], x, B, S * P, C, cfg.num_heads, 1e-5f, true, bb);
+            run_block(c, h->global[i], x, x, x, B, S * P, C, cfg.num_heads, 1e-5f, true, bb, qp(i, 1));
             if (it != saved.end()) c.copy(it->second.second, x, (size_t)M * C * 4);
         }
         c.ar.release(mk);
diff --git a/skiing_analysis_pytorch_amd/ops.py b/skiing_analysis_pytorch_amd/ops.py
--- a/skiing_analysis_pytorch_amd/ops.py
+++ b/skiing_analysis_pytorch_amd/ops.py
@@ -190,6 +190,20 @@
     return out
 
 
+def qknorm_rope_attention_(qkv, batch, seq, heads, qn_w, qn_b, kn_w, kn_b, eps, pos, rope_cos, rope_sin, *, q_scale,
+                           out_dtype=None):
+    _require_cuda(qkv, pos, rope_cos, rope_sin, qn_w, kn_w)
+    assert qkv.dtype == torch.bfloat16
+    out = torch.empty((batch * seq, heads * 64), dtype=out_dtype or qkv.dtype, device=qkv.device)
+    blk = torch.empty(int(lib().skimi_attention_qprep_bytes()), dtype=torch.uint8, device=qkv.device)
+    flag = C.c_int32(0)
+    check(lib().skimi_qknorm_rope_attention(ptr(qkv), ptr(out), _dt(out), batch, seq, heads, ptr(qn_w), ptr(qn_b), ptr(kn_w),
+                                            ptr(kn_b), eps, ptr(pos), ptr(rope_cos), ptr(rope_sin), rope_cos.shape[0],
+                                            q_scale, ptr(blk), C.byref(flag), _lib.current_stream()),
+          "skimi_qknorm_rope_attention")
+    return out, bool(flag.value)
+
+
 def _attention_ex(qkv, batch, seq, heads, head_dim, out_dtype, q_prescaled, x3_scratch, out_records, out):
     _require_cuda(x3_scratch, out)
     rows, Cc = batch * seq, heads * head_dim
```

Result: no change. 17.73 (-1.0%).
